# nalinbhardwaj/curdleproofs.pie

Hardware: AMD Instinct MI355X
Metric: BLS12-381 G1 scalar-muls/sec at MSM size 2^20 (higher is better)
Workload: dtype u32

## Files before the change

curdleproofs_pie_amd/build.py:

```python
from __future__ import annotations

import os
import shutil
import subprocess
import sys

HERE = os.path.dirname(os.path.abspath(__file__))
CSRC = os.path.join(HERE, "csrc")
LIB = os.path.join(HERE, "libcurdle_g1.so")
SOURCES = [os.path.join(CSRC, "msm_gpu.hip"), os.path.join(CSRC, "host_g1.cpp"), os.path.join(CSRC, "merlin.cpp"), os.path.join(CSRC, "shuffle_verify.cpp"), os.path.join(CSRC, "comm.cpp"), os.path.join(CSRC, "lazy_host.cpp")]
DEPS = SOURCES + [os.path.join(CSRC, f) for f in ("kernels_opening.h", "kernels_generator.h", "kernels_fixed.h", "fixed_digits.h", "capi_fixed.h", "kernels_light.h", "light_digits.h", "capi_light.h", "kernels_ipa.h", "ipa_rounds.h", "capi_ipa.h", "kernels_same_msm.h", "same_msm_rounds.h", "capi_same_msm.h", "fp28.h", "g1_xyzz.h", "g1_quad.h", "host_g1.h", "fe_mul_x86.h", "fr.h", "merlin_group.h", "bls_consts.h", "kernels_records.h", "kernels_prepare_digits.h",
                                                    "kernels_sort.h", "kernels_accumulate.h", "kernels_reduce.h", "kernels_small.h", "kernels_batch.h", "kernels_rows.h", "kernels_merlin.h", "kernels_frontend.h", "pool.h", "lazy_host.h", "fp_row.h", "glv.h", "host_context.h", "host_chains.h", "capi_core_msm.h", "capi_vec_batched.h", "capi_lincomb.h",
                                                    "capi_timing_batchmul.h", "capi_codec_transcripts.h", "capi_frontend.h", "capi_rows_probes.h")] + [
    os.path.join(HERE, "..", "include", "curdle_g1.h")
]


def _source_hash() -> str:
    import hashlib

    h = hashlib.sha256()
    for d in sorted(DEPS):
        if os.path.exists(d):
            h.update(os.path.basename(d).encode())
            with open(d, "rb") as f:
                h.update(f.read())
    h.update(os.environ.get("CURDLE_G1_PIPELINE", "staged").encode())
    with open(os.path.abspath(__file__), "rb") as f:
        h.update(f.read())
    return h.hexdigest()


HASH_FILE = LIB + ".srchash"
HOST_ONLY = ("host_g1.cpp", "merlin.cpp", "shuffle_verify.cpp", "comm.cpp", "lazy_host.cpp", "merlin_group.h", "fe_mul_x86.h")


def _hip_unit_hash(extra_flags=()) -> str:
    import hashlib

    h = hashlib.sha256()
    for d in sorted(DEPS):
        if os.path.basename(d) in HOST_ONLY or not os.path.exists(d):
            continue
        h.update(os.path.basename(d).encode())
        with open(d, "rb") as f:
            h.update(f.read())
    h.update(repr(tuple(extra_flags)).encode())
    with open(os.path.abspath(__file__), "rb") as f:
        h.update(f.read())
    return h.hexdigest()[:24]


def needs_build() -> bool:
    if not os.path.exists(LIB) or not os.path.exists(HASH_FILE):
        return True
    try:
        return open(HASH_FILE).read().strip() != _source_hash()
    except OSError:
        return True


LLVM_BIN = "/opt/rocm/lib/llvm/bin"
INFO_FILE = LIB + ".buildinfo"
DROPPED_PASSES = ("reassociate",)


def default_pipeline() -> str:
    p = os.environ.get("CURDLE_G1_PIPELINE", "staged")
    if p not in ("staged", "plain"):
        raise ValueError(f"CURDLE_G1_PIPELINE must be 'staged' or 'plain', not {p!r}")
    return p


def _run(cmd, verbose, **kw):
    if verbose:
        print("[curdleproofs_pie_amd.build]", " ".join(a if len(a) < 160 else a[:157] + "..." for a in cmd), flush=True)
    return subprocess.run(cmd, check=True, **kw)


def _device_pipeline(raw_bc: str, verbose: bool) -> str:
    import re

    tool = lambda t: os.path.join(LLVM_BIN, t)
    out = _run([tool("opt"), "-mtriple=amdgcn-amd-amdhsa", "-mcpu=gfx950", "-amdgpu-internalize-symbols", "-passes=default<O3>", "-print-pipeline-passes",
                "-disable-output", raw_bc], verbose, capture_output=True, text=True).stdout.strip()
    pipe = out.replace(",BitcodeWriterPass", "")
    for dropped in DROPPED_PASSES:
        if f"{dropped}," not in pipe:
            raise RuntimeError(f"pass {dropped!r} not found in the O3 pipeline: the toolchain changed, re-check DESIGN.md section 9")
        pipe = pipe.replace(f"{dropped},", "")
    ll = _run([tool("llvm-dis"), raw_bc, "-o", "-"], False, capture_output=True, text=True).stdout
    keep = re.findall(r"^define [^@\n]*amdgpu_kernel [^@\n]*@([\w.$]+)\(", ll, re.M)
    keep += re.findall(r"^@([\w.$]+) = (?!internal|private)", ll, re.M)
    if not keep or pipe.count(",internalize,") != 1:
# ... 165 lines not shown
```

curdleproofs_pie_amd/csrc/capi_core_msm.h:

```cpp
#pragma once

using cg1::Ctx;
struct cg1_ctx : public cg1::Ctx {};

namespace cg1 {
static Ctx* child_of(Ctx* ctx) { return static_cast<Ctx*>(ctx->child); }

static int ensure_child(Ctx* ctx) {
  if (!ctx->child) {
    cg1_ctx* made = ctx->cu_mask.empty() ? cg1_ctx_create(ctx->device) : cg1_ctx_create_cu_mask(ctx->device, ctx->cu_mask.data(), ctx->cu_mask.size());
    if (!made) { snprintf(ctx->err, sizeof ctx->err, "could not create the second launch chain's context"); return CG1_ERR_HIP; }
    made->split = 0;
    made->batched_split = 0;
    ctx->child = made;
  }
  if (!ctx->ev_prep) HIPCHK(hipEventCreateWithFlags(&ctx->ev_prep, hipEventDisableTiming));
  if (!ctx->ev_acc) HIPCHK(hipEventCreateWithFlags(&ctx->ev_acc, hipEventDisableTiming));
  return CG1_OK;
}

static int msm_begin_split(Ctx* ctx, const PtSrc& src, const void* d_scalars32, size_t n, const WinPlan& plan, int rank, int world) {
  HIPCHK(hipSetDevice(ctx->device));
  { int crc = ensure_child(ctx); if (crc) return crc; }
  Ctx* ch = child_of(ctx);
// ... 191 lines not shown
int cg1_h2d_async(cg1_ctx* ctx, void* dst, const void* src, size_t bytes) {
  if (!ctx) return CG1_ERR_HIP;
  if (bytes == 0) return CG1_OK;
  HIPCHK(hipSetDevice(ctx->device));
  std::call_once(ctx->copy_once, [ctx]() { hipStream_t s = nullptr; if (hipStreamCreateWithFlags(&s, hipStreamNonBlocking) == hipSuccess) ctx->copy_stream.store(s); });
  hipStream_t cs = ctx->copy_stream.load();
  if (!cs) { snprintf(ctx->err, sizeof ctx->err, "could not create the copy stream"); return CG1_ERR_HIP; }
  HIPCHK(hipMemcpyAsync(dst, src, bytes, hipMemcpyHostToDevice, cs));
  return CG1_OK;
}
int cg1_stream_sync(cg1_ctx* ctx) {
  if (!ctx) return CG1_ERR_HIP;
  HIPCHK(hipSetDevice(ctx->device));
  return cg1::wait_stream(ctx);
}
int cg1_copy_fence(cg1_ctx* ctx) {
  if (!ctx) return CG1_ERR_HIP;
  HIPCHK(hipSetDevice(ctx->device));
  hipStream_t cs = ctx->copy_stream.load();
  if (!cs) return CG1_OK;
  HIPCHK(hipEventRecord(ctx->copy_ev, cs));
  HIPCHK(hipStreamWaitEvent(ctx->stream, ctx->copy_ev, 0));
  return CG1_OK;
}
void* cg1_host_alloc(cg1_ctx* ctx, size_t bytes) {
  if (!ctx) return nullptr;
  void* p = nullptr;
  if (hipSetDevice(ctx->device) != hipSuccess) return nullptr;
  if (hipHostMalloc(&p, bytes ? bytes : 1) != hipSuccess) return nullptr;
  return p;
}
void cg1_host_free(cg1_ctx* ctx, void* p) {
  if (!ctx || !p) return;
  (void)hipSetDevice(ctx->device);
  (void)hipHostFree(p);
}
int cg1_d2h_2d(cg1_ctx* ctx, void* dst, size_t dst_pitch, const void* src, size_t src_pitch, size_t width, size_t rows) {
  if (!ctx) return CG1_ERR_HIP;
  if (rows == 0 || width == 0) return CG1_OK;
  if (width > dst_pitch || width > src_pitch) return CG1_ERR_ARG;
  HIPCHK(hipSetDevice(ctx->device));
  HIPCHK(hipMemcpy2D(dst, dst_pitch, src, src_pitch, width, rows, hipMemcpyDeviceToHost));
  return CG1_OK;
}
int cg1_ctx_sync(cg1_ctx* ctx) {
  if (!ctx) return CG1_ERR_HIP;
  HIPCHK(hipSetDevice(ctx->device));
  HIPCHK(hipDeviceSynchronize());
  return CG1_OK;
}
int cg1_merlin_last_passes(const cg1_ctx* ctx) { return ctx ? (int)ctx->merlin_passes : -1; }
int cg1_merlin_last_kernel(const cg1_ctx* ctx) { return ctx ? ctx->merlin_last_kernel : -1; }
int cg1_ctx_device(const cg1_ctx* ctx) { return ctx ? ctx->device : -1; }
void* cg1_ctx_stream(cg1_ctx* ctx) { return ctx ? (void*)ctx->stream : nullptr; }
int cg1_ctx_set_param(cg1_ctx* ctx, const char* name, int value) {
  if (!ctx || !name) return CG1_ERR_ARG;
  if (!strcmp(name, "chunk_rule")) { ctx->chunk_rule = value != 0; return CG1_OK; }
  if (!strcmp(name, "chunk_len")) { if (value < 1 || value > 65536) return CG1_ERR_ARG; ctx->L0 = (uint32_t)value; cg1::free_bufs(ctx); return CG1_OK; }
  if (!strcmp(name, "stage_sort")) { ctx->stage_sort = value ? 1 : 0; return CG1_OK; }
  if (!strcmp(name, "quad")) { ctx->quad = value ? 1 : 0; return CG1_OK; }
  if (!strcmp(name, "glv")) { if (value < 0 || value > 2) return CG1_ERR_ARG; ctx->glv = value; return CG1_OK; }
  if (!strcmp(name, "glv_max_n")) { if (value < 0) return CG1_ERR_ARG; ctx->glv_max_n = value; return CG1_OK; }
  if (!strcmp(name, "batched_split")) { ctx->batched_split = value ? 1 : 0; return CG1_OK; }
  if (!strcmp(name, "batched_split_min_m")) { if (value < 2) return CG1_ERR_ARG; ctx->batched_split_min_m = value; return CG1_OK; }
  if (!strcmp(name, "lincomb_zero_copy")) { ctx->lincomb_zero_copy = value ? 1 : 0; return CG1_OK; }
  if (!strcmp(name, "fold_quad")) { ctx->fold_quad = value ? 1 : 0; return CG1_OK; }
  if (!strcmp(name, "rowcol_row")) { ctx->rowcol_row = value ? 1 : 0; return CG1_OK; }
  if (!strcmp(name, "tree_row")) { ctx->tree_row = value ? 1 : 0; return CG1_OK; }
  if (!strcmp(name, "horner_row")) { ctx->horner_row = value ? 1 : 0; return CG1_OK; }
  if (!strcmp(name, "batch_mul_row")) { ctx->batch_mul_row = value ? 1 : 0; return CG1_OK; }
  if (!strcmp(name, "small_msm")) { ctx->small_msm = value ? 1 : 0; return CG1_OK; }
  if (!strcmp(name, "fixed_slice")) { if (value < 0 || value > 128) return CG1_ERR_ARG; ctx->fixed_slice = value; return CG1_OK; }
  if (!strcmp(name, "fixed_waves")) { if (value != 0 && value != 4 && value != 8 && value != 16) return CG1_ERR_ARG; ctx->fixed_waves = value; return CG1_OK; }
  if (!strcmp(name, "ipa_inv")) { if (value != 0 && value != 1) return CG1_ERR_ARG; ctx->ipa_inv = value; return CG1_OK; }
  if (!strcmp(name, "small_row_tail")) { ctx->small_row_tail = value ? 1 : 0; return CG1_OK; }
  if (!strcmp(name, "split")) { ctx->split = value ? 1 : 0; return CG1_OK; }
  if (!strcmp(name, "split_min_log2n")) { if (value < 10 || value > 31) return CG1_ERR_ARG; ctx->split_min_n = (size_t)1 << value; return CG1_OK; }
  if (!strcmp(name, "reduce_2d")) { ctx->reduce_2d = value ? 1 : 0; return CG1_OK; }
  if (!strcmp(name, "partition_sort")) { ctx->use_partition_sort = value ? 1 : 0; cg1::free_bufs(ctx); return CG1_OK; }
  if (!strcmp(name, "blocking_sync")) { ctx->blocking_sync = value != 0; return CG1_OK; }
  if (!strcmp(name, "big_bins")) { ctx->big_bins = value != 0; return CG1_OK; }
  if (!strcmp(name, "host_split")) { ctx->host_split = value != 0; return CG1_OK; }
  if (!strcmp(name, "arm_helpers")) { ctx->arm_helpers = value != 0; return CG1_OK; }
  if (!strcmp(name, "horner_threads")) { if (value != 1 && value != 2 && value != 4) return CG1_ERR_ARG; ctx->horner_threads = value; return CG1_OK; }
  if (!strcmp(name, "zero_copy")) { ctx->zero_copy = value != 0; return CG1_OK; }
  if (!strcmp(name, "auto_plan")) { ctx->auto_plan = value != 0; return CG1_OK; }
  if (!strcmp(name, "rowcol_quad")) { ctx->rowcol_quad = value != 0; return CG1_OK; }
  if (!strcmp(name, "rowcol_quad_max")) { if (value < 0) return CG1_ERR_ARG; ctx->rowcol_quad_max = value; return CG1_OK; }
  if (!strcmp(name, "fold_pass")) { ctx->fold_pass = value != 0; return CG1_OK; }
  if (!strcmp(name, "scan_one")) { ctx->scan_one = value != 0; return CG1_OK; }
  if (!strcmp(name, "batched_host_horner_max")) { if (value < 0) return CG1_ERR_ARG; ctx->batched_host_horner_max = value; return CG1_OK; }
  if (!strcmp(name, "tree_shift")) { if (value < -1 || value > 4) return CG1_ERR_ARG; ctx->tree_shift = value; return CG1_OK; }
  if (!strcmp(name, "rowcol_lgq")) { if (value != 0 && (value < 2 || value > 4)) return CG1_ERR_ARG; ctx->rowcol_lgq = value; return CG1_OK; }
  if (!strcmp(name, "sort_sub_bits")) { if (value != 0 && (value < 4 || value > 8)) return CG1_ERR_ARG; ctx->sort_sub_bits = value; return CG1_OK; }
  if (!strcmp(name, "batch_mul_host_max")) { if (value < -1) return CG1_ERR_ARG; ctx->batch_mul_host_max = value; return CG1_OK; }
  if (!strcmp(name, "batch_mul_quad_max")) { if (value < 0) return CG1_ERR_ARG; ctx->batch_mul_quad_max = value; return CG1_OK; }
  if (!strcmp(name, "merlin_sync")) { ctx->merlin_sync = value != 0; return CG1_OK; }
  if (!strcmp(name, "fe_timed")) { ctx->fe_timed = value != 0; return CG1_OK; }
  if (!strcmp(name, "fe_rows")) { ctx->fe_rows = value != 0; return CG1_OK; }
  if (!strcmp(name, "fe_prio")) { if (value < 0 || value > 3) return CG1_ERR_ARG; ctx->fe_prio = value; return CG1_OK; }
  if (!strcmp(name, "decompress_waves")) { if (value != 2 && value != 3) return CG1_ERR_ARG; ctx->decompress_waves = value; return CG1_OK; }
  if (!strcmp(name, "merlin_rows")) { ctx->merlin_rows = value != 0; return CG1_OK; }
  if (!strcmp(name, "merlin_lanes")) { if (value < 1 || value > 64) return CG1_ERR_ARG; ctx->merlin_lanes = value; return CG1_OK; }
  if (!strcmp(name, "tree_half")) { ctx->tree_half = value != 0; return CG1_OK; }
  if (!strcmp(name, "wave_agg")) {
    int v = value ? 1 : 0;
    HIPCHK(hipSetDevice(ctx->device));
    HIPCHK(hipMemcpyToSymbol(HIP_SYMBOL(cg1::g_wave_agg), &v, sizeof v));
    return CG1_OK;
  }
  if (!strcmp(name, "profile")) { if (value < 0 || value > 2) return CG1_ERR_ARG; ctx->profile = value; return CG1_OK; }
  if (!strcmp(name, "seg_m")) { if (value != 1 && value != 2 && value != 4 && value != 8 && value != 16) return CG1_ERR_ARG; ctx->seg_m = (uint32_t)value; return CG1_OK; }
  return CG1_ERR_ARG;
}

int cg1_msm_device(cg1_ctx* ctx, const void* d_points, const void* d_scalars, size_t n, int window_c, int shard_rank,
                   int shard_world, uint8_t* out) {
  if (!ctx) return CG1_ERR_HIP;
  cg1h::jac r;
  int rc = cg1::msm_device(ctx, d_points, d_scalars, n, window_c, shard_rank, shard_world, r);
  if (rc == CG1_OK) blob_out(out, r);
  return rc;
}

int cg1_msm_device_begin(cg1_ctx* ctx, const void* d_points, const void* d_scalars, size_t n, int window_c, int shard_rank, int shard_world) {
  if (!ctx) return CG1_ERR_HIP;
  return cg1::msm_begin(ctx, d_points, d_scalars, n, window_c, shard_rank, shard_world);
}
int cg1_msm_device_end(cg1_ctx* ctx, uint8_t* out) {
  if (!ctx) return CG1_ERR_HIP;
  cg1h::jac r;
  int rc = cg1::msm_end(ctx, r);
  if (rc == CG1_OK) blob_out(out, r);
  return rc;
}

int cg1_msm_multi_device(cg1_ctx* const* ctxs, size_t n_ctx, const void* const* d_points, const void* const* d_scalars, const size_t* n,
                         int window_c, uint8_t* out) {
  if (!ctxs || !n_ctx || !d_points || !d_scalars || !n || !out) return CG1_ERR_ARG;
  for (size_t i = 0; i < n_ctx; ++i) {
    if (!ctxs[i]) return CG1_ERR_HIP;
    for (size_t j = 0; j < i; ++j) if (ctxs[j] == ctxs[i]) return CG1_ERR_ARG;
  }
  int rc = CG1_OK;
  size_t begun = 0;
  for (; begun < n_ctx && rc == CG1_OK; ++begun)
    rc = cg1::msm_begin(ctxs[begun], d_points[begun], d_scalars[begun], n[begun], window_c, 0, 1);
  cg1h::jac acc = cg1h::jac_identity();
  for (size_t i = 0; i < begun; ++i) {
    cg1h::jac part;
    int r2 = cg1::msm_end(ctxs[i], part);
    if (rc == CG1_OK) rc = r2;
    if (r2 == CG1_OK) acc = cg1h::jac_add(acc, part);
  }
  if (rc == CG1_OK) blob_out(out, acc);
  return rc;
}

static int ensure_stage(cg1_ctx* ctx, size_t pts_bytes, size_t sc_bytes) {
  if (pts_bytes > ctx->cap_stage_pts) {
    if (ctx->d_stage_pts) (void)hipFree(ctx->d_stage_pts);
    ctx->d_stage_pts = nullptr; ctx->cap_stage_pts = 0;
    const size_t want = pts_bytes + pts_bytes / 4 + 256;
    HIPCHK(hipMalloc(&ctx->d_stage_pts, want));
    ctx->cap_stage_pts = want;
  }
  if (sc_bytes > ctx->cap_stage_sc) {
// ... 73 lines not shown
```

curdleproofs_pie_amd/csrc/host_chains.h:

```cpp
#pragma once

namespace cg1 {

static WinPlan make_plan(int c, bool glv = false) {
  WinPlan pl;
  const int bits = glv ? 127 : 255;
  pl.glv = glv ? 1 : 0;
  if (c > 0) { pl.cmax = c; pl.nwin = bits / c + 1; pl.n_hi = pl.nwin; }
  else {
    const int cm = -c, nw = (bits + 1 + cm - 1) / cm;
    pl.cmax = cm; pl.nwin = nw; pl.n_hi = bits + 1 - nw * (cm - 1);
    if (pl.n_hi < 0) pl.n_hi = 0;
  }
  return pl;
}

static int pick_plan_c(size_t n, int auto_plan) {
  const int c = pick_window(n);
  if (!auto_plan || c != 16) return c;
  if (n <= (1u << 14)) return -12;
  if (n <= (3u << 15)) return -13;
  if (n <= (3u << 16)) return -15;
  return 16;
}
// ... 23 lines not shown
  PtSrc(const void* affine96) : p(affine96) {}
};

static uint32_t blob_points_per_lane(size_t n) {
  size_t K = (n + (1u << 17) - 1) >> 17;
  return (uint32_t)(K < 1 ? 1 : (K > 16 ? 16 : K));
}

static void launch_prepare(hipStream_t st, const PtSrc& src, PreparedPoint* out, uint8_t* flags_out, uint32_t n32, uint32_t* status_words) {
  if (src.kind == PtSrc::AFFINE96) {
    hipLaunchKernelGGL(k_prepare_points, dim3((n32 + 255) / 256), dim3(256), 0, st, (const uint32_t*)src.p, out, flags_out, n32, status_words);
  } else if (src.normalised) {
    hipLaunchKernelGGL((k_prepare_blobs<false>), dim3((n32 + 127) / 128), dim3(128), 0, st, (const uint32_t*)src.p, out, flags_out, n32, 1u, status_words);
  } else {
    const uint32_t K = blob_points_per_lane(n32);
    const uint32_t lanes = (n32 + K - 1) / K;
    hipLaunchKernelGGL((k_prepare_blobs<true>), dim3((lanes + 127) / 128), dim3(128), 0, st, (const uint32_t*)src.p, out, flags_out, n32, K, status_words);
  }
}

struct ChainHooks {
  hipEvent_t before_start = nullptr, after_prepare = nullptr, before_accumulate = nullptr, after_accumulate = nullptr;
};

static int msm_enqueue(Ctx* ctx, const PtSrc& src, const void* d_scalars32, size_t n, const WinPlan& plan, int rank, int world,
                       const ChainHooks& hooks = ChainHooks()) {
  ctx->pend.active = false;
  HIPCHK(hipSetDevice(ctx->device));
  const int c = plan.cmax, nwin = plan.nwin;
  const size_t n_real = n;
  if (plan.glv) n *= 2;
  const int nlw = win_count(nwin, rank, world);
  if (nlw <= 0) return CG1_OK;
  const uint32_t NB = 1u << (c - 1);
  const uint32_t m = std::min<uint32_t>(ctx->seg_m, NB);
  const uint32_t J = NB / m;
  int nbits = 0; while ((1u << nbits) < J) ++nbits;
  const uint32_t bb = (uint32_t)c - 1u, lb2 = (bb + 1u) / 2u, hb2 = bb - lb2;
  const bool use2d = ctx->reduce_2d != 0;
  const uint32_t nitems = use2d ? 1u + hb2 + lb2 : 1u + (uint32_t)nbits;
  const size_t nb_total = (size_t)nlw * NB;
  uint32_t L0 = ctx->L0;
  while (L0 < 65536u && ((uint64_t)n * (uint64_t)nlw >> 18) > (uint64_t)L0) L0 <<= 1;
  if (ctx->chunk_rule && world == 1) {
    const uint64_t entries = (uint64_t)n * (uint64_t)nlw;
    if (entries >= (1ull << 20) && entries < (1ull << 21) && L0 < 10u) L0 = 10u;
    if (entries >= (1ull << 21) && entries < (1ull << 24) && nb_total > (size_t)ctx->rowcol_quad_max) {
      const double mload = (double)n / (double)(1u << bb);
      uint32_t want = (uint32_t)(mload + 8.0 * std::sqrt(mload) + 1.0);
      if (entries < (1ull << 22) && want > 20u) want = 20u;
      if (want > L0) L0 = want;
    }
  }
  int rc = ensure(ctx, n, nb_total, nlw, nitems, L0, src.kind != PtSrc::PREPARED);
  if (rc) return rc;
  hipStream_t st = ctx->stream;
  const uint32_t n32 = (uint32_t)n;
  const uint32_t gn = (n32 + 255) / 256;
  const int profile = ctx->profile;
  auto h0 = std::chrono::steady_clock::now();
  const bool resident = src.kind == PtSrc::PREPARED;
  const PreparedPoint* pts = resident ? static_cast<const PreparedPoint*>(src.p) : ctx->d_pts;
  const uint8_t* flags = resident ? src.flags : ctx->d_flags;
  const size_t nout_words = (size_t)nlw * nitems;
  uint32_t* bad_flag = reinterpret_cast<uint32_t*>(ctx->d_out + nout_words);
  if (hooks.before_start) HIPCHK(hipStreamWaitEvent(st, hooks.before_start, 0));
  if (profile >= 2) HIPCHK(hipEventRecord(ctx->ev[0], st));
  const uint32_t n_real32 = (uint32_t)n_real;
  if (resident) HIPCHK(hipMemsetAsync(bad_flag, 0, 16, st));
  else {
    launch_prepare(st, src, ctx->d_pts, ctx->d_flags, n_real32, bad_flag);
    if (plan.glv) hipLaunchKernelGGL(k_phi_records, dim3((n_real32 + 255) / 256), dim3(256), 0, st, ctx->d_pts, ctx->d_flags, n_real32);
  }
  if (hooks.after_prepare) HIPCHK(hipEventRecord(hooks.after_prepare, st));
  if (profile >= 2) HIPCHK(hipEventRecord(ctx->ev[1], st));
  const uint32_t nblk = (uint32_t)((nb_total + SCAN_ITEMS - 1) / SCAN_ITEMS);
  if (ctx->use_partition_sort && n <= PART_MAX_N) {
    const uint32_t want_sub = ctx->sort_sub_bits ? (uint32_t)ctx->sort_sub_bits : (n <= ((size_t)1 << 16) ? 7u : 8u);
    uint32_t sub_bits = bb < want_sub ? bb : want_sub;
    while (bb - sub_bits > 7u) ++sub_bits;
    const uint32_t nbins = 1u << (bb - sub_bits);
    const uint32_t nslices = (n32 + PART_TILE - 1) / PART_TILE;
    const uint32_t nbc = (uint32_t)nlw * nbins * nslices;
    hipLaunchKernelGGL(k_digits, dim3((n_real32 + 255) / 256), dim3(256), 0, st, (const uint32_t*)d_scalars32, flags, ctx->d_digits, n_real32, plan, rank, world, bad_flag);
    hipLaunchKernelGGL(k_part_count, dim3(nslices, nlw), dim3(256), 0, st, ctx->d_digits, ctx->d_blockcnt, n32, nslices, nbins, sub_bits);
    const uint32_t ublk = (nbc + SCAN_ITEMS - 1) / SCAN_ITEMS;
    if (ctx->scan_one && nbc <= USCAN1_MAX) {
      hipLaunchKernelGGL(k_uscan_one, dim3(1), dim3(1024), 0, st, ctx->d_blockcnt, nbc);
    } else {
      hipLaunchKernelGGL(k_uscan1, dim3(ublk), dim3(256), 0, st, ctx->d_blockcnt, ctx->d_ublocktot, nbc);
      hipLaunchKernelGGL(k_uscan2, dim3(1), dim3(256), 0, st, ctx->d_ublocktot, ublk, ctx->d_blockcnt, nbc);
      hipLaunchKernelGGL(k_uscan3, dim3(ublk), dim3(256), 0, st, ctx->d_ublocktot, ctx->d_blockcnt, nbc);
    }
    if (profile >= 2) HIPCHK(hipEventRecord(ctx->ev[2], st));
    hipLaunchKernelGGL(k_part_scatter, dim3(nslices, nlw), dim3(256), 0, st, ctx->d_digits, ctx->d_blockcnt, ctx->d_part, n32, nslices, nbins, sub_bits, ctx->stage_sort);
    const uint32_t nbt = (uint32_t)nlw * nbins;
    const int big_bins = ctx->big_bins && n32 > 2u * BIN_STAGE;
    hipLaunchKernelGGL(k_slice_plan, dim3(1), dim3(256), 0, st, ctx->d_blockcnt, nbt, nslices, ctx->d_slice_base, ctx->d_bigflag, big_bins);
    hipLaunchKernelGGL(k_bin_sort, dim3(nbt), dim3(256), 0, st, ctx->d_part, ctx->d_blockcnt, ctx->d_hist, ctx->d_sorted, nbt, nslices, sub_bits, ctx->stage_sort, ctx->d_bigflag);
    if (big_bins) {
      const uint32_t max_slices = (uint32_t)(((size_t)n * (size_t)nlw) / SLICE + nbt + 1);
      hipLaunchKernelGGL(k_slice_count, dim3(max_slices), dim3(256), 0, st, ctx->d_part, ctx->d_blockcnt, nbt, nslices, ctx->d_slice_base, ctx->d_slicehist);
      hipLaunchKernelGGL(k_slice_prefix, dim3(nbt), dim3(256), 0, st, ctx->d_blockcnt, nslices, sub_bits, ctx->d_slice_base, ctx->d_bigflag, ctx->d_slicehist, ctx->d_subbase, ctx->d_hist);
      hipLaunchKernelGGL(k_slice_scatter, dim3(max_slices), dim3(256), 0, st, ctx->d_part, ctx->d_blockcnt, nbt, nslices, ctx->d_slice_base, ctx->d_slicehist, ctx->d_subbase, ctx->d_sorted);
    }
    if (profile >= 2) HIPCHK(hipEventRecord(ctx->ev[3], st));
    if (ctx->scan_one && nb_total <= SCAN1_MAX) {
      hipLaunchKernelGGL(k_scan_one, dim3(1), dim3(1024), 0, st, ctx->d_hist, ctx->d_off, ctx->d_choff, (uint32_t)nb_total, L0);
    } else {
      hipLaunchKernelGGL(k_scan1, dim3(nblk), dim3(256), 0, st, ctx->d_hist, ctx->d_off, ctx->d_choff, ctx->d_blocktot, (uint32_t)nb_total, L0);
      hipLaunchKernelGGL(k_scan2, dim3(1), dim3(256), 0, st, ctx->d_blocktot, nblk, ctx->d_off, ctx->d_choff, (uint32_t)nb_total);
      hipLaunchKernelGGL(k_scan3, dim3(nblk), dim3(256), 0, st, ctx->d_blocktot, ctx->d_off, ctx->d_choff, (uint32_t)nb_total);
    }
  } else {
    HIPCHK(hipMemsetAsync(ctx->d_hist, 0, nb_total * 4, st));
    hipLaunchKernelGGL(k_hist, dim3(gn), dim3(256), 0, st, (const uint32_t*)d_scalars32, flags, ctx->d_hist, n32, plan, rank, world, bad_flag);
    if (profile >= 2) HIPCHK(hipEventRecord(ctx->ev[2], st));
    hipLaunchKernelGGL(k_scan1, dim3(nblk), dim3(256), 0, st, ctx->d_hist, ctx->d_off, ctx->d_choff, ctx->d_blocktot, (uint32_t)nb_total, L0);
    hipLaunchKernelGGL(k_scan2, dim3(1), dim3(256), 0, st, ctx->d_blocktot, nblk, ctx->d_off, ctx->d_choff, (uint32_t)nb_total);
    hipLaunchKernelGGL(k_scan3, dim3(nblk), dim3(256), 0, st, ctx->d_blocktot, ctx->d_off, ctx->d_choff, (uint32_t)nb_total);
    if (profile >= 2) HIPCHK(hipEventRecord(ctx->ev[3], st));
    hipLaunchKernelGGL(k_scatter, dim3(gn), dim3(256), 0, st, (const uint32_t*)d_scalars32, flags, ctx->d_hist, ctx->d_off, ctx->d_sorted, n32, plan, rank, world);
  }
  HIPCHK(hipMemsetAsync(ctx->d_zblock, 0, zblock_clear_bytes(ctx), st));
  hipLaunchKernelGGL(k_chunk_desc, dim3((uint32_t)std::min<size_t>(CHUNK_DESC_BLOCKS, (nb_total + 255) / 256)), dim3(256), 0, st, ctx->d_off, ctx->d_choff, ctx->d_desc, ctx->d_lenhist, ctx->d_heavy, (uint32_t)ctx->cap_heavy, (uint32_t)nb_total, L0, ctx->d_any_multi);
  const size_t max_chunks = nb_total + (n * (size_t)nlw) / L0 + 1;
  const uint32_t gchunks = (uint32_t)((max_chunks + 255) / 256);
  hipLaunchKernelGGL(k_len_scan, dim3(1), dim3(256), 0, st, ctx->d_lenhist, ctx->d_lenhist + LEN_BINS, ctx->d_off + nb_total, ctx->d_choff + nb_total, bad_flag);
  hipLaunchKernelGGL(k_order, dim3((gchunks + ORDER_PER - 1) / ORDER_PER), dim3(256), 0, st, ctx->d_desc, ctx->d_choff + nb_total, ctx->d_lenhist + LEN_BINS, ctx->d_order);
  if (hooks.before_accumulate) HIPCHK(hipStreamWaitEvent(st, hooks.before_accumulate, 0));
  if (profile >= 1) HIPCHK(hipEventRecord(ctx->ev[4], st));
  hipLaunchKernelGGL(k_accumulate, dim3(gchunks), dim3(256), 0, st, ctx->d_desc, ctx->d_choff + nb_total, ctx->d_order, ctx->d_sorted, pts, ctx->d_sums);
  if (profile >= 1) HIPCHK(hipEventRecord(ctx->ev[5], st));
  if (hooks.after_accumulate) HIPCHK(hipEventRecord(hooks.after_accumulate, st));
  hipLaunchKernelGGL(k_heavy_combine, dim3(512), dim3(256), 0, st, ctx->d_heavy, (uint32_t)ctx->cap_heavy, ctx->d_choff, ctx->d_sums, ctx->d_combined);
  const bool small_quad = ctx->quad && ctx->rowcol_quad && nb_total <= (size_t)ctx->rowcol_quad_max;
  const bool rows_fold = small_quad && use2d && ctx->rowcol_row && ctx->tree_row && nb_total <= 8192;
  if (rows_fold) {}
  else if (small_quad && ctx->fold_quad)
    hipLaunchKernelGGL(k_bucket_fold_quad, dim3((uint32_t)((nb_total * 4 + 255) / 256)), dim3(256), 0, st, ctx->d_choff, ctx->d_sums, ctx->d_combined, (uint32_t)nb_total, ctx->d_any_multi);
  else if (ctx->fold_pass)
    hipLaunchKernelGGL(k_bucket_fold, dim3((uint32_t)((nb_total + 255) / 256)), dim3(256), 0, st, ctx->d_choff, ctx->d_sums, ctx->d_combined, (uint32_t)nb_total, ctx->d_any_multi);
  bool tree_exports = false;
  if (use2d) {
    const uint32_t R = 1u << hb2, Cn = 1u << lb2;
    const uint32_t lpr = Cn < 32u ? Cn : 32u, lpc = R < 16u ? R : 16u;
    const uint32_t nrow_blocks = ((uint32_t)nlw * R + (256u / lpr) - 1u) / (256u / lpr);
    const uint32_t ncol_blocks = ((uint32_t)nlw * Cn + (256u / lpc) - 1u) / (256u / lpc);
    PointSum* rowsum = ctx->d_segrun;
    PointSum* colsum = ctx->d_segtot;
    if (small_quad) {
      uint32_t lgq = (R == Cn) ? 2u : 3u;
      if (ctx->rowcol_lgq >= 2 && ctx->rowcol_lgq <= 4) lgq = (uint32_t)ctx->rowcol_lgq;
      const uint32_t rc_waves = ((uint32_t)nlw * (R + Cn) + (16u >> lgq) - 1u) / (16u >> lgq);
      if (ctx->rowcol_row && ctx->tree_row)
        hipLaunchKernelGGL(k_rowcol_quad_row, dim3(((uint32_t)nlw * (R + Cn) + 3u) / 4u), dim3(256), 0, st, ctx->d_choff, ctx->d_sums, ctx->d_combined,
                           rowsum, colsum, (uint32_t)nlw, hb2, lb2);
      else
      hipLaunchKernelGGL(k_rowcol_quad, dim3((rc_waves + 3u) / 4u), dim3(256), 0, st, ctx->d_choff, ctx->d_sums,
                         rowsum, colsum, (uint32_t)nlw, hb2, lb2, lgq);
    }
    else
      hipLaunchKernelGGL(k_rowcol, dim3(nrow_blocks + ncol_blocks), dim3(256), 0, st, ctx->d_choff, ctx->d_sums, ctx->d_combined,
                         rowsum, colsum, (uint32_t)nlw, hb2, lb2, nrow_blocks, ctx->quad);
    if (profile >= 2) HIPCHK(hipEventRecord(ctx->ev[6], st));
    const uint32_t tree_threads = std::min<uint32_t>(512u, std::max<uint32_t>(64u, 4u << std::max(hb2, lb2)) >> (ctx->tree_shift >= 0 ? ctx->tree_shift : (ctx->tree_half ? 1 : 0)));
    if (ctx->tree_row) {
      uint32_t W = (1u << std::max(hb2, lb2)) >> 3;
      W = W < 1u ? 1u : (W > 16u ? 16u : W);
      tree_exports = ctx->zero_copy != 0;
      if (tree_exports) ++ctx->seq;
      hipLaunchKernelGGL(k_small_tree_row, dim3(nitems, nlw), dim3(64u * W), 0, st, rowsum, colsum, ctx->d_out, hb2, lb2,
                         tree_exports ? ctx->h_out_dev : (PointWords*)nullptr, bad_flag, ctx->h_flag_dev, ctx->seq);
    }
    else if (ctx->quad) hipLaunchKernelGGL(k_small_tree_quad, dim3(nitems, nlw), dim3(std::max<uint32_t>(64u, tree_threads)), 0, st, rowsum, colsum, ctx->d_out, hb2, lb2);
    else hipLaunchKernelGGL(k_small_tree, dim3(nitems, nlw), dim3(256), 0, st, rowsum, colsum, ctx->d_out, hb2, lb2);
  } else {
    const uint32_t nseg_total = (uint32_t)(nb_total / m);
    hipLaunchKernelGGL(k_seg_reduce, dim3((nseg_total + 255) / 256), dim3(256), 0, st, ctx->d_choff, ctx->d_sums, ctx->d_combined, ctx->d_segrun, ctx->d_segtot, nseg_total, m);
    if (profile >= 2) HIPCHK(hipEventRecord(ctx->ev[6], st));
    uint32_t S = (J + BT_ELEMS - 1) / BT_ELEMS; if (S < 1) S = 1; if (S > 64) S = 64;
    hipLaunchKernelGGL(k_bit_tree, dim3(nitems, nlw, S), dim3(256), 0, st, ctx->d_segrun, ctx->d_segtot, ctx->d_partial, J);
    hipLaunchKernelGGL(k_bit_tree_final, dim3((uint32_t)(nitems * nlw)), dim3(64), 0, st, ctx->d_partial, ctx->d_out, S);
  }
  const bool zc = ctx->zero_copy != 0;
  if (zc && tree_exports) {
  } else if (zc) {
    ++ctx->seq;
    const uint32_t nvec = (uint32_t)((((size_t)nlw * nitems + 1) * sizeof(PointWords)) / 16);
    hipLaunchKernelGGL(k_export_host, dim3(1), dim3(1024), 0, st, reinterpret_cast<const uint4*>(ctx->d_out), reinterpret_cast<uint4*>(ctx->h_out_dev), nvec,
                       ctx->h_flag_dev, ctx->seq);
  } else {
    HIPCHK(hipMemcpyAsync(ctx->h_out, ctx->d_out, ((size_t)nlw * nitems + 1) * sizeof(PointWords), hipMemcpyDeviceToHost, st));
  }
  if (profile >= 2) HIPCHK(hipEventRecord(ctx->ev[7], st));
  auto h1 = std::chrono::steady_clock::now();
  Ctx::Pending& pd = ctx->pend;
  pd.zero_copy = zc; pd.seq = ctx->seq; pd.hout = ctx->h_out;
  pd.active = true; pd.c = c; pd.plan = plan; pd.rank = rank; pd.world = world; pd.nlw = nlw; pd.nbits = nbits; pd.m = m; pd.lb2 = lb2; pd.hb2 = hb2;
  pd.nitems = nitems; pd.use2d = use2d; pd.profile = profile; pd.nout_words = nout_words; pd.h0 = h0; pd.h1 = h1;
  pd.arm_helpers = ctx->arm_helpers && ctx->host_split && ctx->horner_threads > 1 && n <= ((size_t)1 << 18);
  return CG1_OK;
}

static int msm_finish(Ctx* ctx, cg1h::jac& result) {
  result = cg1h::jac_identity();
  if (!ctx->pend.active) return CG1_OK;
  const Ctx::Pending pd = ctx->pend;
  ctx->pend.active = false;
  const int c = pd.c, rank = pd.rank, world = pd.world, nlw = pd.nlw, nbits = pd.nbits;
  (void)c;
  const uint32_t m = pd.m, lb2 = pd.lb2, hb2 = pd.hb2, nitems = pd.nitems;
  const bool use2d = pd.use2d;
  const size_t nout_words = pd.nout_words;
  const auto h0 = pd.h0, h1 = pd.h1;
  HIPCHK(hipSetDevice(ctx->device));
  struct StandDown { Ctx* c; bool on; ~StandDown() { if (on) for (int j = 0; j < 3; ++j) c->helper[j].disarm(); } } stand_down{ctx, false};
  if (pd.zero_copy && !ctx->blocking_sync && pd.profile < 2) {
    if (pd.arm_helpers) for (int j = 0; j < 3 && j + 1 < ctx->horner_threads; ++j) ctx->helper[j].arm();
    stand_down.on = pd.arm_helpers;
    volatile uint32_t* flag = ctx->h_flag;
    for (uint32_t spins = 0; *flag != pd.seq; ++spins) {
      if ((spins & 0x3fffu) == 0x3fffu) {
        hipError_t q = hipStreamQuery(ctx->stream);
        if (q == hipSuccess) { if (*flag != pd.seq) { snprintf(ctx->err, sizeof ctx->err, "the stream drained without the export flag"); return CG1_ERR_HIP; } break; }
        if (q != hipErrorNotReady) { snprintf(ctx->err, sizeof ctx->err, "stream failed: %s", hipGetErrorString(q)); return CG1_ERR_HIP; }
      }
      __builtin_ia32_pause();
    }
    std::atomic_thread_fence(std::memory_order_acquire);
  } else {
    int wrc = wait_stream(ctx); if (wrc) return wrc;
  }
  HIPCHK(hipGetLastError());
  {
    const uint32_t* st_words = reinterpret_cast<const uint32_t*>(pd.hout + nout_words);
    ctx->last_entries = st_words[1]; ctx->last_chunks = st_words[2];
    if (st_words[0]) {
      snprintf(ctx->err, sizeof ctx->err, "a scalar is >= 2^255: scalar32 must be a canonical Fr element (< r)");
      return CG1_ERR_ENCODING;
    }
  }
  auto h2 = std::chrono::steady_clock::now();
  { int erc = read_phase_events(ctx, pd.profile); if (erc) return erc; }
  ctx->last_c = c;

  auto t0 = std::chrono::steady_clock::now();
  ctx->host_ms[0] = std::chrono::duration<float, std::milli>(h1 - h0).count();
  ctx->host_ms[1] = std::chrono::duration<float, std::milli>(h2 - h1).count();
  ctx->host_ms[2] = std::chrono::duration<float, std::milli>(t0 - h2).count();
  int lm = 0; while ((1u << lm) < m) ++lm;
  const WinPlan& plan = pd.plan;
  constexpr int EMAX = 2 * 256 + 64;
  std::vector<std::pair<int, const PointWords*>> items;
  items.reserve((size_t)nlw * nitems);
  int e_top = 0;
  for (int lw = 0; lw < nlw; ++lw) {
    const int w = win_global(lw, rank, world), base = plan.off(w);
    const PointWords* row = pd.hout + (size_t)lw * nitems;
    auto put = [&](int e, const PointWords* p) { if (!p->inf && e >= 0 && e < EMAX) { items.emplace_back(e, p); if (e > e_top) e_top = e; } };
    put(base, &row[0]);
    if (use2d) {
      for (uint32_t k = 0; k < hb2; ++k) put(base + (int)lb2 + (int)k, &row[1 + k]);
      for (uint32_t k = 0; k < lb2; ++k) put(base + (int)k, &row[1 + hb2 + k]);
    } else {
      for (int b2 = 0; b2 < nbits; ++b2) put(base + lm + b2, &row[1 + b2]);
    }
  }
  uint16_t first[EMAX + 1];
  memset(first, 0, sizeof first);
  for (const auto& it : items) ++first[it.first + 1];
  for (int e = 0; e < EMAX; ++e) first[e + 1] = (uint16_t)(first[e + 1] + first[e]);
  std::vector<const PointWords*> byexp(items.size());
  {
    uint16_t cur[EMAX];
    memcpy(cur, first, sizeof cur);
    for (const auto& it : items) byexp[cur[it.first]++] = it.second;
  }
  auto horner = [&](int lo, int hi) {
    cg1h::jac a = cg1h::jac_identity();
    for (int e = hi; e >= lo; --e) {
      a = cg1h::jac_dbl(a);
      for (uint16_t k = first[e]; k < first[e + 1]; ++k) a = cg1h::jac_add(a, jac_from_words(*byexp[k]));
    }
    return a;
  };
  cg1h::jac acc;
  const int nth = (!ctx->host_split || e_top < 96) ? 1 : (ctx->horner_threads >= 4 && e_top >= 112 ? 4 : 2);
  if (nth > 1) {
    cg1h::jac part[4];
    int lo[5];
    {
      constexpr long DBL = 7, ADD = 16;
      auto fill = [&](long C, int* cut) {
        int e = 0;
        for (int j = 0; j < nth; ++j) {
          cut[j] = e;
          long adds = 0;
          while (e <= e_top && DBL * (e + 1) + ADD * (adds + (first[e + 1] - first[e])) <= C) { adds += first[e + 1] - first[e]; ++e; }
        }
        cut[nth] = e_top + 1;
        return e > e_top;
      };
      long lo_c = DBL * (e_top + 1), hi_c = DBL * (e_top + 1) + ADD * (long)items.size();
      int cut[5];
      while (lo_c < hi_c) {
        const long mid = (lo_c + hi_c) / 2;
        if (fill(mid, cut)) hi_c = mid; else lo_c = mid + 1;
      }
      fill(hi_c, cut);
      for (int j = 0; j <= nth; ++j) lo[j] = cut[j];
    }
    auto run_part = [&](int j) {
      cg1h::jac a = horner(lo[j], lo[j + 1] - 1);
      for (int k = 0; k < lo[j]; ++k) a = cg1h::jac_dbl(a);
      part[j] = a;
    };
    for (int j = 0; j + 1 < nth; ++j) ctx->helper[j].run([&, j]() { run_part(j); });
    if (pd.arm_helpers) for (int j = nth - 1 < 0 ? 0 : nth - 1; j < 3; ++j) ctx->helper[j].disarm();
    run_part(nth - 1);
    acc = part[nth - 1];
    for (int j = 0; j + 1 < nth; ++j) { ctx->helper[j].wait(); acc = cg1h::jac_add(acc, part[j]); }
  } else {
    if (pd.arm_helpers) for (int j = 0; j < 3; ++j) ctx->helper[j].disarm();
    acc = horner(0, e_top);
  }
  result = acc;
  ctx->host_tail_ms = std::chrono::duration<float, std::milli>(std::chrono::steady_clock::now() - t0).count();
  ctx->host_ms[3] = ctx->host_tail_ms;
  return CG1_OK;
}

static int pick_small_c(size_t n) {
  if (n <= 24) return 4;
  if (n <= 96) return 6;
  if (n <= 6 * SM_SLICE) return 7;
  return 8;
}

static int msm_enqueue_small(Ctx* ctx, const PtSrc& src, const void* d_scalars32, size_t n, int c, uint32_t M = 1, const uint32_t* d_offs = nullptr, size_t max_n = 0,
                             bool glv = false) {
  ctx->pend.active = false;
  HIPCHK(hipSetDevice(ctx->device));
  const WinPlan plan = make_plan(c, glv);
  const uint32_t nwin = (uint32_t)plan.nwin, bb = (uint32_t)c - 1u, lb2 = (bb + 1u) / 2u, hb2 = bb - lb2, nitems = 1u + hb2 + lb2;
  if (M == 1) max_n = n;
  const uint32_t S = (uint32_t)(((glv ? 2 * max_n : max_n) + SM_SLICE - 1) / SM_SLICE);
  auto h0 = std::chrono::steady_clock::now();
  if (!ctx->h_small_out) {
    HIPCHK(hipHostMalloc((void**)&ctx->h_small_out, ((size_t)SM_MAX_MSMS * 64 * 9 + 1) * sizeof(PointWords), hipHostMallocMapped | hipHostMallocCoherent));
    HIPCHK(hipHostGetDevicePointer((void**)&ctx->h_small_out_dev, ctx->h_small_out, 0));
    HIPCHK(hipMalloc(&ctx->d_small_ctr, (SM_MAX_MSMS * 64 + 8) * 4));
    HIPCHK(hipMemsetAsync(ctx->d_small_ctr, 0, (SM_MAX_MSMS * 64 + 8) * 4, ctx->stream));
  }
  const size_t need_partial = (size_t)M * nwin * S * nitems;
  if (S > 1 && need_partial > ctx->cap_small_partial) {
    if (ctx->d_small_partial) (void)hipFree(ctx->d_small_partial);
    ctx->d_small_partial = nullptr; ctx->cap_small_partial = 0;
    HIPCHK(hipMalloc(&ctx->d_small_partial, need_partial * sizeof(PointSum)));
    ctx->cap_small_partial = need_partial;
  }
  hipStream_t st = ctx->stream;
  SmallArgs a;
  a.src = src.p; a.flags = src.flags; a.scalars = static_cast<const uint32_t*>(d_scalars32); a.offs = d_offs;
  a.n = (uint32_t)n; a.M = M; a.S = S; a.c = (uint32_t)c; a.nwin = nwin; a.hb = hb2; a.lb = lb2; a.nitems = nitems;
  a.partial = ctx->d_small_partial; a.counters = ctx->d_small_ctr;
  a.out_host = ctx->h_small_out_dev; a.flag_host = ctx->h_flag_dev; a.seq = ++ctx->seq;
  a.row_tail = ctx->small_row_tail ? 1u : 0u;
  a.glv = glv ? 1u : 0u;
  int kind = (int)src.kind;
  if (src.kind == PtSrc::BLOBS && !src.normalised) {
    if (n > ctx->cap_small_pts) {
      if (ctx->d_small_pts) (void)hipFree(ctx->d_small_pts);
      if (ctx->d_small_flags) (void)hipFree(ctx->d_small_flags);
      ctx->d_small_pts = nullptr; ctx->d_small_flags = nullptr; ctx->cap_small_pts = 0;
      const size_t cap = n < SM_MAX_N ? SM_MAX_N : n;
      HIPCHK(hipMalloc(&ctx->d_small_pts, cap * sizeof(PreparedPoint)));
      HIPCHK(hipMalloc(&ctx->d_small_flags, cap + 16));
      ctx->cap_small_pts = cap;
    }
    launch_prepare(st, src, ctx->d_small_pts, ctx->d_small_flags, (uint32_t)n, nullptr);
    a.src = ctx->d_small_pts; a.flags = ctx->d_small_flags;
    kind = (int)PtSrc::PREPARED;
  }
  const dim3 grid(nwin, S, M), block(512);
  if (kind == (int)PtSrc::AFFINE96) hipLaunchKernelGGL((k_msm_small<0>), grid, block, 0, st, a);
  else if (kind == (int)PtSrc::BLOBS) hipLaunchKernelGGL((k_msm_small<1>), grid, block, 0, st, a);
  else hipLaunchKernelGGL((k_msm_small<2>), grid, block, 0, st, a);
  auto h1 = std::chrono::steady_clock::now();
  Ctx::Pending& pd = ctx->pend;
  pd.zero_copy = true; pd.seq = ctx->seq; pd.hout = ctx->h_small_out;
  pd.active = true; pd.c = c; pd.plan = plan; pd.rank = 0; pd.world = 1; pd.nlw = (int)nwin; pd.nbits = 0; pd.m = 1; pd.lb2 = lb2; pd.hb2 = hb2;
  pd.nitems = nitems; pd.use2d = true; pd.profile = 0; pd.nout_words = (size_t)M * nwin * nitems; pd.h0 = h0; pd.h1 = h1;
  pd.arm_helpers = ctx->arm_helpers && ctx->host_split && ctx->horner_threads > 1 && M == 1;
  return CG1_OK;
}

static cg1h::jac horner_2d_items(const PointWords* rows, const WinPlan& plan, uint32_t nitems, uint32_t hb2, uint32_t lb2) {
  constexpr int EMAX = 2 * 256 + 64;
  std::vector<std::pair<int, const PointWords*>> items;
  items.reserve((size_t)plan.nwin * nitems);
  int e_top = 0;
  for (int w = 0; w < plan.nwin; ++w) {
    const int base = plan.off(w);
    const PointWords* row = rows + (size_t)w * nitems;
    auto put = [&](int e, const PointWords* p) { if (!p->inf) { items.emplace_back(e, p); if (e > e_top) e_top = e; } };
    put(base, &row[0]);
    for (uint32_t k = 0; k < hb2; ++k) put(base + (int)lb2 + (int)k, &row[1 + k]);
    for (uint32_t k = 0; k < lb2; ++k) put(base + (int)k, &row[1 + hb2 + k]);
  }
  uint16_t first[EMAX + 1];
  memset(first, 0, sizeof first);
  for (const auto& it : items) ++first[it.first + 1];
  for (int e = 0; e < EMAX; ++e) first[e + 1] = (uint16_t)(first[e + 1] + first[e]);
  std::vector<const PointWords*> byexp(items.size());
  {
    uint16_t cur[EMAX];
    memcpy(cur, first, sizeof cur);
    for (const auto& it : items) byexp[cur[it.first]++] = it.second;
  }
  cg1h::jac a = cg1h::jac_identity();
  for (int e = e_top; e >= 0; --e) {
    a = cg1h::jac_dbl(a);
    for (uint16_t k = first[e]; k < first[e + 1]; ++k) a = cg1h::jac_add(a, jac_from_words(*byexp[k]));
  }
  return a;
}

static int msm_small_batched_finish(Ctx* ctx, uint32_t M, std::vector<cg1h::jac>& results) {
  const Ctx::Pending pd = ctx->pend;
  ctx->pend.active = false;
  HIPCHK(hipSetDevice(ctx->device));
  if (!ctx->blocking_sync) {
    volatile uint32_t* flag = ctx->h_flag;
    for (uint32_t spins = 0; *flag != pd.seq; ++spins) {
      if ((spins & 0x3fffu) == 0x3fffu) {
        hipError_t q = hipStreamQuery(ctx->stream);
        if (q == hipSuccess) { if (*flag != pd.seq) { snprintf(ctx->err, sizeof ctx->err, "the stream drained without the export flag"); return CG1_ERR_HIP; } break; }
        if (q != hipErrorNotReady) { snprintf(ctx->err, sizeof ctx->err, "stream failed: %s", hipGetErrorString(q)); return CG1_ERR_HIP; }
      }
      __builtin_ia32_pause();
    }
    std::atomic_thread_fence(std::memory_order_acquire);
  } else {
    int wrc = wait_stream(ctx); if (wrc) return wrc;
  }
  HIPCHK(hipGetLastError());
  const uint32_t* st_words = reinterpret_cast<const uint32_t*>(pd.hout + pd.nout_words);
  ctx->last_entries = st_words[1]; ctx->last_chunks = 0;
  if (st_words[0]) {
    snprintf(ctx->err, sizeof ctx->err, "a scalar is >= 2^255: scalar32 must be a canonical Fr element (< r)");
    return CG1_ERR_ENCODING;
  }
  auto t0 = std::chrono::steady_clock::now();
  const size_t per = (size_t)pd.plan.nwin * pd.nitems;
  auto one = [&](size_t j) { results[j] = horner_2d_items(pd.hout + j * per, pd.plan, pd.nitems, pd.hb2, pd.lb2); };
  if (M <= 4) {
    const size_t nth = std::min<size_t>(4, M);
    for (size_t t = 1; t < nth; ++t) ctx->helper[t - 1].run([&, t]() { for (size_t j = t; j < M; j += nth) one(j); });
    for (size_t j = 0; j < M; j += nth) one(j);
    for (size_t t = 1; t < nth; ++t) ctx->helper[t - 1].wait();
  } else {
    std::atomic<size_t> next{0};
    std::function<void()> work = [&]() { for (;;) { const size_t j = next.fetch_add(1); if (j >= M) return; one(j); } };
    Pool& pool = Pool::get();
    pool.run(work, std::min<size_t>(M, pool.size() + 1));
  }
  auto t1 = std::chrono::steady_clock::now();
  ctx->host_ms[0] = std::chrono::duration<float, std::milli>(pd.h1 - pd.h0).count();
  ctx->host_ms[1] = std::chrono::duration<float, std::milli>(t0 - pd.h1).count();
  ctx->host_ms[2] = 0;
  ctx->host_ms[3] = ctx->host_tail_ms = std::chrono::duration<float, std::milli>(t1 - t0).count();
  for (int i = 0; i < CG1_NPHASE; ++i) ctx->phase_ms[i] = 0.f;
  ctx->last_c = pd.c;
  ctx->last_acc_launches = 0;
  return CG1_OK;
}

static Ctx* child_of(Ctx* ctx);
static int msm_begin_split(Ctx* ctx, const PtSrc& src, const void* d_scalars32, size_t n, const WinPlan& plan, int rank, int world);

int msm_begin(Ctx* ctx, const PtSrc& src, const void* d_scalars32, size_t n, int c, int rank, int world) {
  ctx->pend.active = false;
  ctx->pend_c = 0;
  if (n == 0) return CG1_OK;
  if (n >= (1ull << 31)) { snprintf(ctx->err, sizeof ctx->err, "n too large"); return CG1_ERR_ARG; }
  if (world < 1 || world > 255 || rank < 0 || rank >= world) { snprintf(ctx->err, sizeof ctx->err, "bad window shard %d/%d", rank, world); return CG1_ERR_ARG; }
  for (int pass = (ctx->glv && 2 * n <= SM_MAX_N) ? 1 : 0; pass >= 0; --pass) {
    const bool sglv = pass == 1;
    const size_t nn = sglv ? 2 * n : n;
    const int bits = sglv ? 127 : 255;
    if (ctx->small_msm && nn <= SM_MAX_N && world == 1 && (c == 0 || (c >= 4 && c <= 9 && c != 5)) &&
        (size_t)(bits / (c ? c : pick_small_c(nn)) + 1) * ((nn + SM_SLICE - 1) / SM_SLICE) <= SM_ONE_ROUND) {
      if (c == 0) c = pick_small_c(nn);
      ctx->pend_c = c;
      return msm_enqueue_small(ctx, src, d_scalars32, n, c, 1, nullptr, 0, sglv);
    }
  }
  const bool glv = src.kind != PtSrc::PREPARED && ctx->use_partition_sort && 2 * n <= PART_MAX_N &&
                   (ctx->glv == 2 || (ctx->glv == 1 && n <= (size_t)ctx->glv_max_n));
  if (c == 0) c = pick_plan_c(glv ? 2 * n : n, ctx->auto_plan);
  const int cabs = c < 0 ? -c : c;
  if (cabs < 4 || cabs > 16) { snprintf(ctx->err, sizeof ctx->err, "window width %d out of range [4,16]", c); return CG1_ERR_ARG; }
  const WinPlan plan = make_plan(c, glv);
  ctx->pend_c = c;
  ctx->pend_split = false;
  if (ctx->split && n >= ctx->split_min_n && win_count(plan.nwin, rank, world) >= 2) return msm_begin_split(ctx, src, d_scalars32, n, plan, rank, world);
  return msm_enqueue(ctx, src, d_scalars32, n, plan, rank, world);
}
// ... 16 lines not shown
    ctx->last_entries = e_hi + ch->last_entries; ctx->last_chunks = c_hi + ch->last_chunks;
    ctx->host_ms[0] = enq + ch->host_ms[0]; ctx->host_ms[1] = wait_hi + ch->host_ms[1]; ctx->host_ms[3] = tail_hi + ch->host_ms[3];
    ctx->host_tail_ms = ch->host_ms[3];
  }
  if (ctx->pend_c) ctx->last_c = ctx->pend_c;
  return rc;
}
int msm_device(Ctx* ctx, const PtSrc& src, const void* d_scalars32, size_t n, int c, int rank, int world, cg1h::jac& result) {
  result = cg1h::jac_identity();
  int rc = msm_begin(ctx, src, d_scalars32, n, c, rank, world);
  if (rc) return rc;
  return msm_end(ctx, result);
}


int pick_window_batched(size_t n_avg, bool glv) {
  const int bits = glv ? 127 : 255;
  if (glv) n_avg *= 2;
  int best = 4; double best_cost = 1e300;
  for (int c = 4; c <= 9; ++c) {
    if (bits % c == 0) continue;
    int nwin = bits / c + 1;
    double NB = (double)(1u << (c - 1));
    double cost = (double)nwin * ((double)n_avg + 1.4 * (2.0 * NB + 3.0 * NB / 8.0)) + 1.4 * (double)bits;
    if (cost < best_cost) { best_cost = cost; best = c; }
  }
  return best;
}
int pick_window_batched(size_t n_avg) { return pick_window_batched(n_avg, false); }

static int ensure_child(Ctx* ctx);

struct BatchedChain {
  size_t M = 0; int c = 0; uint32_t nwin = 0; bool host_horner = false;
  std::chrono::steady_clock::time_point h0, h1;
};
static int batched_chain_enqueue(Ctx* ctx, const void* d_points96, const void* d_scalars32, const uint32_t* h_offsets, size_t M, int c, bool glv,
                                 hipEvent_t wait_before_accumulate, hipEvent_t record_after_accumulate, BatchedChain& bc) {
  const size_t N = h_offsets[M], N_real = N;
  HIPCHK(hipSetDevice(ctx->device));
  const WinPlan bplan = make_plan(c, glv);
  const uint32_t nwin = (uint32_t)bplan.nwin, NB = 1u << (c - 1);
  const size_t G = M * nwin, nb_total = G * NB;
  const size_t Nv = glv ? 2 * N : N;
  if (nb_total >= (1ull << 31) || Nv * nwin >= (1ull << 31)) { snprintf(ctx->err, sizeof ctx->err, "batch too large"); return CG1_ERR_ARG; }
  const uint32_t m = 8 < NB ? 8 : NB;
  uint32_t log2m = 0; while ((1u << log2m) < m) ++log2m;
  const uint32_t J = NB / m;
  uint32_t L0 = ctx->L0;
  while (L0 < 65536u && ((uint64_t)Nv * (uint64_t)nwin >> 18) > (uint64_t)L0) L0 <<= 1;
  int rc = ensure(ctx, Nv, nb_total, nwin, 1, L0);
  if (rc) return rc;
  if ((M + 1) > ctx->cap_boffs) {
    if (ctx->d_boffs) (void)hipFree(ctx->d_boffs);
    HIPCHK(hipMalloc(&ctx->d_boffs, (M + 1) * 4));
    ctx->cap_boffs = M + 1;
  }
  if (G > ctx->cap_gsum) {
    if (ctx->d_gsum) (void)hipFree(ctx->d_gsum);
    HIPCHK(hipMalloc(&ctx->d_gsum, G * sizeof(PointSum)));
    ctx->cap_gsum = G;
  }
  if (M > ctx->cap_bout) {
    if (ctx->d_bout) (void)hipFree(ctx->d_bout);
    if (ctx->h_bout) (void)hipHostFree(ctx->h_bout);
    HIPCHK(hipMalloc(&ctx->d_bout, (M + 1) * sizeof(PointWords)));
    HIPCHK(hipHostMalloc(&ctx->h_bout, (M + 1) * sizeof(PointWords)));
    ctx->cap_bout = M;
  }
  if (Nv * nwin > ctx->cap_digits) {
    if (ctx->d_digits) (void)hipFree(ctx->d_digits);
    HIPCHK(hipMalloc(&ctx->d_digits, Nv * nwin * 2 + 16));
    ctx->cap_digits = Nv * nwin;
  }
  hipStream_t st = ctx->stream;
  const uint32_t N32 = (uint32_t)N_real, gn = (N32 + 255) / 256, Nv32 = (uint32_t)Nv, split = glv ? N32 : 0u;
  auto h0 = std::chrono::steady_clock::now();
  HIPCHK(hipMemcpyAsync(ctx->d_boffs, h_offsets, (M + 1) * 4, hipMemcpyHostToDevice, st));
  if (ctx->profile >= 2) HIPCHK(hipEventRecord(ctx->ev[0], st));
  uint32_t* bad_flag = reinterpret_cast<uint32_t*>(ctx->d_bout + M);
  hipLaunchKernelGGL(k_prepare_points, dim3(gn), dim3(256), 0, st, (const uint32_t*)d_points96, ctx->d_pts, ctx->d_flags, N32, bad_flag);
  if (glv) hipLaunchKernelGGL(k_phi_records, dim3(gn), dim3(256), 0, st, ctx->d_pts, ctx->d_flags, N32);
  if (ctx->profile >= 2) HIPCHK(hipEventRecord(ctx->ev[1], st));
  hipLaunchKernelGGL(k_digits, dim3(gn), dim3(256), 0, st, (const uint32_t*)d_scalars32, ctx->d_flags, ctx->d_digits, N32, bplan, 0, 1, bad_flag);
  hipLaunchKernelGGL(k_group_count, dim3((uint32_t)M, nwin), dim3(256), 0, st, ctx->d_digits, ctx->d_boffs, ctx->d_hist, Nv32, NB, nwin, split);
  if (ctx->profile >= 2) HIPCHK(hipEventRecord(ctx->ev[2], st));
  const uint32_t nblk = (uint32_t)((nb_total + SCAN_ITEMS - 1) / SCAN_ITEMS);
  hipLaunchKernelGGL(k_scan1, dim3(nblk), dim3(256), 0, st, ctx->d_hist, ctx->d_off, ctx->d_choff, ctx->d_blocktot, (uint32_t)nb_total, L0);
  hipLaunchKernelGGL(k_scan2, dim3(1), dim3(256), 0, st, ctx->d_blocktot, nblk, ctx->d_off, ctx->d_choff, (uint32_t)nb_total);
  hipLaunchKernelGGL(k_scan3, dim3(nblk), dim3(256), 0, st, ctx->d_blocktot, ctx->d_off, ctx->d_choff, (uint32_t)nb_total);
  hipLaunchKernelGGL(k_group_scatter, dim3((uint32_t)M, nwin), dim3(256), 0, st, ctx->d_digits, ctx->d_boffs, ctx->d_off, ctx->d_sorted, Nv32, NB, nwin, split);
  if (ctx->profile >= 2) HIPCHK(hipEventRecord(ctx->ev[3], st));
  HIPCHK(hipMemsetAsync(ctx->d_zblock, 0, zblock_clear_bytes(ctx), st));
  hipLaunchKernelGGL(k_chunk_desc, dim3((uint32_t)std::min<size_t>(CHUNK_DESC_BLOCKS, (nb_total + 255) / 256)), dim3(256), 0, st, ctx->d_off, ctx->d_choff, ctx->d_desc, ctx->d_lenhist, ctx->d_heavy, (uint32_t)ctx->cap_heavy, (uint32_t)nb_total, L0, ctx->d_any_multi);
  const size_t max_chunks = nb_total + (Nv * (size_t)nwin) / L0 + 1;
  const uint32_t gchunks = (uint32_t)((max_chunks + 255) / 256);
  hipLaunchKernelGGL(k_len_scan, dim3(1), dim3(256), 0, st, ctx->d_lenhist, ctx->d_lenhist + LEN_BINS, ctx->d_off + nb_total, ctx->d_choff + nb_total, bad_flag);
  hipLaunchKernelGGL(k_order, dim3((gchunks + ORDER_PER - 1) / ORDER_PER), dim3(256), 0, st, ctx->d_desc, ctx->d_choff + nb_total, ctx->d_lenhist + LEN_BINS, ctx->d_order);
  if (wait_before_accumulate) HIPCHK(hipStreamWaitEvent(st, wait_before_accumulate, 0));
  if (ctx->profile >= 1) HIPCHK(hipEventRecord(ctx->ev[4], st));
  hipLaunchKernelGGL(k_accumulate, dim3(gchunks), dim3(256), 0, st, ctx->d_desc, ctx->d_choff + nb_total, ctx->d_order, ctx->d_sorted, ctx->d_pts, ctx->d_sums);
  if (ctx->profile >= 1) HIPCHK(hipEventRecord(ctx->ev[5], st));
  if (record_after_accumulate) HIPCHK(hipEventRecord(record_after_accumulate, st));
  const uint32_t nseg_total = (uint32_t)(nb_total / m);
  hipLaunchKernelGGL(k_heavy_combine, dim3(512), dim3(256), 0, st, ctx->d_heavy, (uint32_t)ctx->cap_heavy, ctx->d_choff, ctx->d_sums, ctx->d_combined);
  hipLaunchKernelGGL(k_seg_reduce, dim3((nseg_total + 255) / 256), dim3(256), 0, st, ctx->d_choff, ctx->d_sums, ctx->d_combined, ctx->d_segrun, ctx->d_segtot, nseg_total, m);
  hipLaunchKernelGGL(k_group_reduce, dim3((uint32_t)((G + 255) / 256)), dim3(256), 0, st, ctx->d_segrun, ctx->d_segtot, ctx->d_gsum, (uint32_t)G, J, log2m);
  if (ctx->profile >= 2) HIPCHK(hipEventRecord(ctx->ev[6], st));
  const bool host_horner = M <= (size_t)ctx->batched_host_horner_max;
  if (host_horner) {
    if (G > ctx->cap_gout) {
      if (ctx->d_gout) (void)hipFree(ctx->d_gout);
      if (ctx->h_gout) (void)hipHostFree(ctx->h_gout);
      ctx->d_gout = nullptr; ctx->h_gout = nullptr; ctx->cap_gout = 0;
      HIPCHK(hipMalloc(&ctx->d_gout, G * sizeof(PointWords)));
      HIPCHK(hipHostMalloc(&ctx->h_gout, G * sizeof(PointWords)));
      ctx->cap_gout = G;
    }
    hipLaunchKernelGGL(k_export_sums, dim3((uint32_t)((G + 63) / 64)), dim3(64), 0, st, ctx->d_gsum, ctx->d_gout, (uint32_t)G);
    HIPCHK(hipMemcpyAsync(ctx->h_gout, ctx->d_gout, G * sizeof(PointWords), hipMemcpyDeviceToHost, st));
    HIPCHK(hipMemcpyAsync(ctx->h_bout + M, ctx->d_bout + M, sizeof(PointWords), hipMemcpyDeviceToHost, st));
  } else {
    if (ctx->horner_row && M <= 2048) hipLaunchKernelGGL(k_msm_horner_row, dim3((uint32_t)M), dim3(64), 0, st, ctx->d_gsum, ctx->d_bout, (uint32_t)M, nwin, (uint32_t)c);
    else if (ctx->quad) hipLaunchKernelGGL(k_msm_horner_quad, dim3((uint32_t)((M * 4 + 63) / 64)), dim3(64), 0, st, ctx->d_gsum, ctx->d_bout, (uint32_t)M, nwin, (uint32_t)c);
    else hipLaunchKernelGGL(k_msm_horner, dim3((uint32_t)((M + 63) / 64)), dim3(64), 0, st, ctx->d_gsum, ctx->d_bout, (uint32_t)M, nwin, (uint32_t)c);
    HIPCHK(hipMemcpyAsync(ctx->h_bout, ctx->d_bout, (M + 1) * sizeof(PointWords), hipMemcpyDeviceToHost, st));
  }
  if (ctx->profile >= 2) HIPCHK(hipEventRecord(ctx->ev[7], st));
  bc.M = M; bc.c = c; bc.nwin = nwin; bc.host_horner = host_horner; bc.h0 = h0; bc.h1 = std::chrono::steady_clock::now();
  return CG1_OK;
}

static int batched_chain_finish(Ctx* ctx, const BatchedChain& bc, cg1h::jac* results) {
  const size_t M = bc.M; const int c = bc.c; const uint32_t nwin = bc.nwin; const bool host_horner = bc.host_horner;
  const auto h0 = bc.h0, h1 = bc.h1;
  HIPCHK(hipSetDevice(ctx->device));
  { int wrc = wait_stream(ctx); if (wrc) return wrc; }
  HIPCHK(hipGetLastError());
  {
    const uint32_t* st_words = reinterpret_cast<const uint32_t*>(ctx->h_bout + M);
    ctx->last_entries = st_words[1]; ctx->last_chunks = st_words[2];
    if (st_words[0]) {
      snprintf(ctx->err, sizeof ctx->err, "a scalar is >= 2^255: scalar32 must be a canonical Fr element (< r)");
      return CG1_ERR_ENCODING;
    }
  }
  auto h2 = std::chrono::steady_clock::now();
  { int erc = read_phase_events(ctx, ctx->profile); if (erc) return erc; }
  ctx->last_c = c;
  if (host_horner) {
    auto one = [&](size_t j) {
      cg1h::jac a = cg1h::jac_identity();
      for (int w = (int)nwin - 1; w >= 0; --w) {
        for (int k = 0; k < c; ++k) a = cg1h::jac_dbl(a);
        a = cg1h::jac_add(a, jac_from_words(ctx->h_gout[j * nwin + (size_t)w]));
      }
      results[j] = a;
    };
    const size_t nth = std::min<size_t>(4, M);
    for (size_t t = 1; t < nth; ++t) ctx->helper[t - 1].run([&, t]() { for (size_t j = t; j < M; j += nth) one(j); });
    for (size_t j = 0; j < M; j += nth) one(j);
    for (size_t t = 1; t < nth; ++t) ctx->helper[t - 1].wait();
  } else {
    for (size_t j = 0; j < M; ++j) results[j] = jac_from_words(ctx->h_bout[j]);
  }
  auto h3 = std::chrono::steady_clock::now();
  ctx->host_ms[0] = std::chrono::duration<float, std::milli>(h1 - h0).count();
  ctx->host_ms[1] = std::chrono::duration<float, std::milli>(h2 - h1).count();
  ctx->host_ms[2] = 0;
  ctx->host_ms[3] = ctx->host_tail_ms = std::chrono::duration<float, std::milli>(h3 - h2).count();
  return CG1_OK;
}

static int msm_batched_small_end(Ctx* ctx, size_t M, std::vector<cg1h::jac>& results) {
  if (M == 1) { cg1h::jac r; int rc = msm_finish(ctx, r); ctx->last_acc_launches = 0; if (rc == CG1_OK) results[0] = r; return rc; }
  return msm_small_batched_finish(ctx, (uint32_t)M, results);
}
int msm_batched_device(Ctx* ctx, const void* d_points96, const void* d_scalars32, const uint32_t* h_offsets, size_t M,
                       int c, std::vector<cg1h::jac>& results, bool* async_small = nullptr, const uint32_t* d_offsets_ready = nullptr) {
  if (async_small) *async_small = false;
  results.assign(M, cg1h::jac_identity());
  if (M == 0) return CG1_OK;
  const size_t N = h_offsets[M];
  for (size_t j = 0; j < M; ++j) if (h_offsets[j] > h_offsets[j + 1]) { snprintf(ctx->err, sizeof ctx->err, "offsets not monotone"); return CG1_ERR_ARG; }
  if (h_offsets[0] != 0) { snprintf(ctx->err, sizeof ctx->err, "offsets[0] must be 0"); return CG1_ERR_ARG; }
  if (N == 0) return CG1_OK;
  if (N >= (1ull << 31) || M > 65535) { snprintf(ctx->err, sizeof ctx->err, "batch too large"); return CG1_ERR_ARG; }
  {
// ... 62 lines not shown
```

curdleproofs_pie_amd/csrc/host_context.h:

```cpp
#pragma once

namespace cg1 {

#define HIPCHK(x) do { hipError_t e_ = (x); if (e_ != hipSuccess) { \
  snprintf(ctx->err, sizeof ctx->err, "%s failed: %s (%s:%d)", #x, hipGetErrorString(e_), __FILE__, __LINE__); return CG1_ERR_HIP; } } while (0)

struct Helper {
  std::thread th;
  std::mutex mu;
  std::condition_variable cv;
  std::function<void()> job;
  bool has = false, done = true, quit = false, armed = false;
  std::atomic<bool> posted{false};
  std::atomic<bool> stand_down{false};
  void start_locked() { if (!th.joinable()) th = std::thread([this]() { loop(); }); }
  void run(std::function<void()> f) {
    std::unique_lock<std::mutex> lk(mu);
    start_locked();
    job = std::move(f); has = true; done = false;
    posted.store(true, std::memory_order_release);
    cv.notify_all();
  }
  void arm() {
    std::unique_lock<std::mutex> lk(mu);
    start_locked();
    if (!has && done) { stand_down.store(false, std::memory_order_relaxed); armed = true; cv.notify_all(); }
  }
  void disarm() { stand_down.store(true, std::memory_order_release); }
  void wait() {
    std::unique_lock<std::mutex> lk(mu);
    cv.wait(lk, [this]() { return done; });
  }
  void loop() {
    std::unique_lock<std::mutex> lk(mu);
    for (;;) {
      cv.wait(lk, [this]() { return has || quit || armed; });
      if (quit) return;
      if (!has) {
        armed = false;
        lk.unlock();
        const auto until = std::chrono::steady_clock::now() + std::chrono::milliseconds(2);
        for (uint32_t k = 0; !posted.load(std::memory_order_acquire); ++k) {
          if (stand_down.load(std::memory_order_acquire)) break;
          if ((k & 0xffu) == 0xffu && std::chrono::steady_clock::now() > until) break;
          __builtin_ia32_pause();
        }
        lk.lock();
        if (!has) continue;
      }
      armed = false;
      std::function<void()> f = std::move(job);
      has = false;
      posted.store(false, std::memory_order_relaxed);
      lk.unlock();
      f();
      lk.lock();
      done = true;
      cv.notify_all();
    }
  }
  ~Helper() {
    { std::unique_lock<std::mutex> lk(mu); quit = true; cv.notify_all(); }
    if (th.joinable()) th.join();
  }
};

struct Ctx {
  int device = 0;
  Helper helper[3];
  hipStream_t stream = nullptr;
  std::atomic<hipStream_t> copy_stream{nullptr};
  std::once_flag copy_once;
  hipEvent_t copy_ev = nullptr;
  std::vector<uint32_t> cu_mask;
  hipStream_t side_stream = nullptr;
  hipEvent_t side_ev = nullptr;
  hipEvent_t sync_ev = nullptr;
  int blocking_sync = 0;
  char err[256] = {0};
  size_t cap_n = 0, cap_nb = 0, cap_chunks = 0, cap_entries = 0, cap_out = 0;
  PreparedPoint* d_pts = nullptr;
  uint8_t* d_flags = nullptr;
  uint32_t *d_hist = nullptr, *d_off = nullptr, *d_choff = nullptr, *d_sorted = nullptr;
  uint2 *d_blocktot = nullptr, *d_desc = nullptr;
  uint32_t *d_order = nullptr, *d_lenhist = nullptr;
  uint32_t* d_zblock = nullptr; size_t cap_zblock = 0;
  uint32_t* d_any_multi = nullptr;
  PointSum* d_partial = nullptr; size_t cap_partial = 0;
  uint16_t* d_digits = nullptr; uint32_t* d_part = nullptr; uint32_t* d_blockcnt = nullptr; uint32_t* d_ublocktot = nullptr;
  size_t cap_digits = 0, cap_part = 0, cap_blockcnt = 0;
  uint32_t *d_slice_base = nullptr, *d_slicehist = nullptr, *d_subbase = nullptr; uint8_t* d_bigflag = nullptr;
  size_t cap_bigflag = 0, cap_slices = 0;
  int big_bins = 1;
  int use_partition_sort = 1;
  int stage_sort = 1;
  int host_split = 1;
  int rowcol_quad = 1;
  int rowcol_lgq = 0;
  int rowcol_quad_max = 1 << 18;
  int tree_shift = 2;
  int tree_half = 1;
  int merlin_sync = 1;
  uint32_t merlin_clk[2] = {0, 0};
  int fe_timed = 0;
  int fe_rows = 1;
  int fe_prio = 0;
  int decompress_waves = 3;
  void* d_opening = nullptr; size_t cap_opening = 0;
  void* d_prover = nullptr; size_t cap_prover = 0;
  PreparedPoint* d_gen_tab = nullptr;
  int fixed_slice = 0;
  int fixed_waves = 0;
  int ipa_inv = 0;
  int merlin_last_kernel = 0;
  int merlin_rows = 1;
  void* d_merlin_rows = nullptr; size_t merlin_rows_cap = 0;
  int merlin_lanes = 64;
  uint32_t merlin_passes = 0;
  int sort_sub_bits = 0;
  int batch_mul_host_max = -1;
  int last_batch_mul_on_host = 0;
  int batch_mul_quad_max = 8192;
  int scan_one = 1;
  int fold_pass = 1;
  int auto_plan = 1;
  struct Pending {
    bool active = false;
    int c = 0, rank = 0, world = 1, nlw = 0, nbits = 0;
    WinPlan plan;
    uint32_t m = 1, lb2 = 0, hb2 = 0, nitems = 0;
    bool use2d = true;
    int profile = 0;
    bool zero_copy = false; uint32_t seq = 0;
    bool arm_helpers = false;
    size_t nout_words = 0;
    const PointWords* hout = nullptr;
    std::chrono::steady_clock::time_point h0, h1;
  } pend;
  int split = 0;
  size_t split_min_n = (size_t)1 << 17;
  cg1_ctx* child = nullptr;
  hipEvent_t ev_prep = nullptr, ev_acc = nullptr;
  bool pend_split = false;
  int last_acc_launches = 0;
  int small_row_tail = 1;
  int small_msm = 1;
  PointSum* d_small_partial = nullptr; size_t cap_small_partial = 0;
  uint32_t* d_small_ctr = nullptr;
  PreparedPoint* d_small_pts = nullptr; uint8_t* d_small_flags = nullptr; size_t cap_small_pts = 0;
  PointWords* h_small_out = nullptr; PointWords* h_small_out_dev = nullptr;
  int quad = 1;
  int reduce_2d = 1;
  uint32_t* d_heavy = nullptr; size_t cap_heavy = 0;
  uint8_t* d_combined = nullptr; size_t cap_combined = 0;
  uint32_t* d_boffs = nullptr; size_t cap_boffs = 0;
  PointSum* d_gsum = nullptr; size_t cap_gsum = 0;
  PointWords* d_bout = nullptr; PointWords* h_bout = nullptr; size_t cap_bout = 0;
  PointWords* d_gout = nullptr; PointWords* h_gout = nullptr; size_t cap_gout = 0;
  int glv = 0;
  int glv_max_n = 1 << 14;
  int lincomb_zero_copy = 1;
  int fold_quad = 1;
  int rowcol_row = 1;
  int tree_row = 1;
  int horner_row = 1;
  int batch_mul_row = 1;
  int batched_split = 0;
  int batched_split_min_m = 256;
  int batched_host_horner_max = 24;
  PointSum *d_sums = nullptr, *d_segrun = nullptr, *d_segtot = nullptr;
  PointWords* d_out = nullptr;
  PointWords* h_out = nullptr;
  PointWords* h_out_dev = nullptr;
  uint32_t* h_flag = nullptr;
  uint32_t* h_flag_dev = nullptr;
  uint32_t seq = 0;
  int zero_copy = 1;
  int arm_helpers = 1;
  int horner_threads = 4;
  void* d_stage_pts = nullptr; void* d_stage_sc = nullptr; size_t cap_stage_pts = 0, cap_stage_sc = 0;
  uint8_t* h_lin = nullptr; uint8_t* h_lin_dev = nullptr; size_t cap_h_lin = 0;
  hipEvent_t ev[CG1_NPHASE + 1];
  float phase_ms[CG1_NPHASE] = {0};
  float host_tail_ms = 0;
  float host_ms[4] = {0, 0, 0, 0};
  int profile = 1;
  uint32_t last_chunks = 0, last_entries = 0;
  hipEvent_t tm_ev[2] = {nullptr, nullptr};
  int last_c = 0, pend_c = 0;
  int chunk_rule = 1;
  uint32_t L0 = 8;
  uint32_t seg_m = 4;
};

static void free_bufs(Ctx* c) {
  auto F = [](auto*& p) { if (p) { (void)hipFree(p); p = nullptr; } };
  F(c->d_pts); F(c->d_flags); F(c->d_hist); F(c->d_off); F(c->d_choff); F(c->d_sorted); F(c->d_blocktot); F(c->d_desc);
  F(c->d_sums); F(c->d_segrun); F(c->d_segtot); F(c->d_out); F(c->d_order); F(c->d_zblock); F(c->d_partial);
  c->d_lenhist = c->d_heavy = c->d_any_multi = nullptr; c->d_combined = nullptr; c->cap_zblock = 0; c->cap_heavy = 0; c->cap_combined = 0;
  c->cap_partial = 0;
  F(c->d_digits); F(c->d_part); F(c->d_blockcnt); F(c->d_ublocktot); F(c->d_boffs); F(c->d_gsum); F(c->d_bout);
  F(c->d_slice_base); F(c->d_slicehist); F(c->d_subbase); F(c->d_bigflag); c->cap_bigflag = 0; c->cap_slices = 0;
  if (c->h_bout) { (void)hipHostFree(c->h_bout); c->h_bout = nullptr; }
  if (c->h_lin) { (void)hipHostFree(c->h_lin); c->h_lin = nullptr; c->h_lin_dev = nullptr; c->cap_h_lin = 0; }
  if (c->d_gout) { (void)hipFree(c->d_gout); c->d_gout = nullptr; }
  if (c->h_gout) { (void)hipHostFree(c->h_gout); c->h_gout = nullptr; }
  c->cap_gout = 0;
  c->cap_boffs = c->cap_gsum = c->cap_bout = 0;
  c->cap_digits = c->cap_part = c->cap_blockcnt = 0;
  if (c->h_out) { (void)hipHostFree(c->h_out); c->h_out = nullptr; }
  c->cap_n = c->cap_nb = c->cap_chunks = c->cap_entries = c->cap_out = 0;
}

static int ensure(Ctx* ctx, size_t n, size_t nb_total, size_t nlw, size_t nitems, uint32_t L, bool need_points = true) {
  size_t entries = n * nlw;
  size_t chunks = nb_total + entries / L + 1;
  if (need_points && n > ctx->cap_n) {
    if (ctx->d_pts) (void)hipFree(ctx->d_pts);
    if (ctx->d_flags) (void)hipFree(ctx->d_flags);
    HIPCHK(hipMalloc(&ctx->d_pts, n * sizeof(PreparedPoint)));
    HIPCHK(hipMalloc(&ctx->d_flags, n + 16));
    ctx->cap_n = n;
  }
  if (nb_total > ctx->cap_nb) {
    auto F = [](auto*& p) { if (p) { (void)hipFree(p); p = nullptr; } };
    F(ctx->d_hist); F(ctx->d_off); F(ctx->d_choff); F(ctx->d_blocktot); F(ctx->d_segrun); F(ctx->d_segtot);
    HIPCHK(hipMalloc(&ctx->d_hist, nb_total * 4));
    HIPCHK(hipMalloc(&ctx->d_off, (nb_total + 1) * 4));
    HIPCHK(hipMalloc(&ctx->d_choff, (nb_total + 1) * 4));
    HIPCHK(hipMalloc(&ctx->d_blocktot, (nb_total / SCAN_ITEMS + 2) * sizeof(uint2)));
    HIPCHK(hipMalloc(&ctx->d_segrun, nb_total * sizeof(PointSum)));
    HIPCHK(hipMalloc(&ctx->d_segtot, nb_total * sizeof(PointSum)));
    ctx->cap_nb = nb_total;
  }
  if (entries > ctx->cap_entries) {
    if (ctx->d_sorted) (void)hipFree(ctx->d_sorted);
    HIPCHK(hipMalloc(&ctx->d_sorted, (entries + 1) * 4));
    ctx->cap_entries = entries;
  }
  if (chunks > ctx->cap_chunks) {
    if (ctx->d_desc) (void)hipFree(ctx->d_desc);
    if (ctx->d_sums) (void)hipFree(ctx->d_sums);
    if (ctx->d_order) (void)hipFree(ctx->d_order);
    HIPCHK(hipMalloc(&ctx->d_order, chunks * 4));
    HIPCHK(hipMalloc(&ctx->d_desc, chunks * sizeof(uint2)));
    HIPCHK(hipMalloc(&ctx->d_sums, chunks * sizeof(PointSum)));
    ctx->cap_chunks = chunks;
  }
  {
    const size_t hcap = entries / ((size_t)L * (HEAVY_MIN_CHUNKS - 1)) + 2;
    const size_t z0 = 2 * LEN_BINS + 1, h0 = z0 + (nb_total + 3) / 4, words = h0 + 1 + hcap + 64;
    if (words > ctx->cap_zblock) {
      if (ctx->d_zblock) (void)hipFree(ctx->d_zblock);
      ctx->d_zblock = nullptr; ctx->cap_zblock = 0;
      HIPCHK(hipMalloc(&ctx->d_zblock, words * 4));
      ctx->cap_zblock = words;
    }
    ctx->d_lenhist = ctx->d_zblock;
    ctx->d_any_multi = ctx->d_zblock + 2 * LEN_BINS;
    ctx->d_combined = reinterpret_cast<uint8_t*>(ctx->d_zblock + z0);
    ctx->d_heavy = ctx->d_zblock + h0;
    ctx->cap_heavy = hcap;
    ctx->cap_combined = nb_total;
  }
  if (ctx->use_partition_sort && n <= PART_MAX_N) {
    const size_t nslices = (n + PART_TILE - 1) / PART_TILE;
    const size_t nbc = nlw * 128 * nslices + 1;
    if (entries > ctx->cap_digits) {
      if (ctx->d_digits) (void)hipFree(ctx->d_digits);
      HIPCHK(hipMalloc(&ctx->d_digits, entries * 2 + 16));
      ctx->cap_digits = entries;
    }
    if (entries > ctx->cap_part) {
      if (ctx->d_part) (void)hipFree(ctx->d_part);
      HIPCHK(hipMalloc(&ctx->d_part, (entries + 1) * 4));
      ctx->cap_part = entries;
    }
    if (nlw * 128 > ctx->cap_bigflag) {
      auto F = [](auto*& p) { if (p) { (void)hipFree(p); p = nullptr; } };
      F(ctx->d_bigflag); F(ctx->d_slice_base); F(ctx->d_subbase);
      HIPCHK(hipMalloc(&ctx->d_bigflag, nlw * 128 + 16));
      HIPCHK(hipMalloc(&ctx->d_slice_base, (nlw * 128 + 1) * 4));
      HIPCHK(hipMalloc(&ctx->d_subbase, nlw * 128 * 256 * 4));
      ctx->cap_bigflag = nlw * 128;
    }
    {
      const size_t max_slices = entries / SLICE + nlw * 128 + 1;
      if (max_slices > ctx->cap_slices) {
        if (ctx->d_slicehist) (void)hipFree(ctx->d_slicehist);
        HIPCHK(hipMalloc(&ctx->d_slicehist, max_slices * 256 * 4));
        ctx->cap_slices = max_slices;
      }
    }
    if (nbc > ctx->cap_blockcnt) {
      if (ctx->d_blockcnt) (void)hipFree(ctx->d_blockcnt);
      if (ctx->d_ublocktot) (void)hipFree(ctx->d_ublocktot);
      HIPCHK(hipMalloc(&ctx->d_blockcnt, nbc * 4));
      HIPCHK(hipMalloc(&ctx->d_ublocktot, (nbc / SCAN_ITEMS + 2) * 4));
      ctx->cap_blockcnt = nbc;
    }
  }
  size_t nout = nlw * nitems;
  if (nout * 64 > ctx->cap_partial) {
    if (ctx->d_partial) (void)hipFree(ctx->d_partial);
    HIPCHK(hipMalloc(&ctx->d_partial, nout * 64 * sizeof(PointSum)));
    ctx->cap_partial = nout * 64;
  }
  if (nout > ctx->cap_out) {
    if (ctx->d_out) (void)hipFree(ctx->d_out);
    if (ctx->h_out) (void)hipHostFree(ctx->h_out);
    HIPCHK(hipMalloc(&ctx->d_out, (nout + 1) * sizeof(PointWords)));
    HIPCHK(hipHostMalloc(&ctx->h_out, (nout + 1) * sizeof(PointWords), hipHostMallocMapped | hipHostMallocCoherent));
    HIPCHK(hipHostGetDevicePointer((void**)&ctx->h_out_dev, ctx->h_out, 0));
    ctx->cap_out = nout;
  }
  return CG1_OK;
}

static size_t zblock_clear_bytes(const Ctx* ctx) {
  size_t bytes = (size_t)((ctx->d_heavy + 1) - ctx->d_zblock) * 4;
  bytes = (bytes + 255) & ~(size_t)255;
  const size_t cap = ctx->cap_zblock * 4;
  return bytes < cap ? bytes : cap;
}

static int read_phase_events(Ctx* ctx, int profile) {
  for (int i = 0; i < CG1_NPHASE; ++i) ctx->phase_ms[i] = 0.f;
  if (profile >= 2) {
    for (int i = 0; i < CG1_NPHASE; ++i) HIPCHK(hipEventElapsedTime(&ctx->phase_ms[i], ctx->ev[i], ctx->ev[i + 1]));
  } else if (profile == 1) {
    HIPCHK(hipEventElapsedTime(&ctx->phase_ms[4], ctx->ev[4], ctx->ev[5]));
  }
  return CG1_OK;
}

static cg1h::fe fe_from_words12(const uint32_t w[12]) {
  cg1h::fe r;
  for (int i = 0; i < 6; ++i) r.l[i] = (uint64_t)w[2 * i] | ((uint64_t)w[2 * i + 1] << 32);
  return r;
}
static cg1h::jac jac_from_words(const PointWords& p) {
  if (p.inf) return cg1h::jac_identity();
  return cg1h::jac_from_xyzz(fe_from_words12(p.w[0]), fe_from_words12(p.w[1]), fe_from_words12(p.w[2]), fe_from_words12(p.w[3]));
}

}
```

curdleproofs_pie_amd/csrc/host_g1.cpp:

```cpp
#include "host_g1.h"
#include "bls_consts.h"
#include "fe_mul_x86.h"
#include <cstring>
#include <vector>

namespace cg1h {

typedef unsigned __int128 u128;
using cg1::H_P; using cg1::H_PINV; using cg1::H_R1; using cg1::H_R2;

static inline fe mk(const uint64_t* w) { fe r; for (int i = 0; i < 6; ++i) r.l[i] = w[i]; return r; }

fe fe_zero() { fe r; memset(&r, 0, sizeof r); return r; }
fe fe_one() { return mk(H_R1); }
bool fe_is_zero(const fe& a) { uint64_t o = 0; for (int i = 0; i < 6; ++i) o |= a.l[i]; return o == 0; }
bool fe_eq(const fe& a, const fe& b) { uint64_t o = 0; for (int i = 0; i < 6; ++i) o |= a.l[i] ^ b.l[i]; return o == 0; }

static inline bool geq_p(const uint64_t* a) {
  for (int i = 5; i >= 0; --i) { if (a[i] > H_P[i]) return true; if (a[i] < H_P[i]) return false; }
  return true;
}
static inline void sub_p(uint64_t* a) {
  u128 br = 0;
  for (int i = 0; i < 6; ++i) { u128 t = (u128)a[i] - H_P[i] - br; a[i] = (uint64_t)t; br = (t >> 64) & 1; }
}

bool fe_is_canonical(const fe& a) { return !geq_p(a.l); }

fe fe_add(const fe& a, const fe& b) {
  fe r; u128 c = 0;
  for (int i = 0; i < 6; ++i) { c += (u128)a.l[i] + b.l[i]; r.l[i] = (uint64_t)c; c >>= 64; }
  if (geq_p(r.l)) sub_p(r.l);
  return r;
}
fe fe_sub(const fe& a, const fe& b) {
  fe r; u128 br = 0;
  for (int i = 0; i < 6; ++i) { u128 t = (u128)a.l[i] - b.l[i] - br; r.l[i] = (uint64_t)t; br = (t >> 64) & 1; }
  if (br) { u128 c = 0; for (int i = 0; i < 6; ++i) { c += (u128)r.l[i] + H_P[i]; r.l[i] = (uint64_t)c; c >>= 64; } }
  return r;
}
fe fe_neg(const fe& a) { return fe_is_zero(a) ? a : fe_sub(fe_zero(), a); }

#if defined(__x86_64__)
static const bool g_has_adx = __builtin_cpu_supports("bmi2") && __builtin_cpu_supports("adx");
#endif

fe fe_mul(const fe& a, const fe& b) {
#if defined(__x86_64__)
  if (g_has_adx) {
    fe r;
    fe_mul_adx(r.l, a.l, b.l, H_P, H_PINV);
    if (geq_p(r.l)) sub_p(r.l);
    return r;
  }
#endif
  uint64_t t0 = 0, t1 = 0, t2 = 0, t3 = 0, t4 = 0, t5 = 0;
#pragma GCC unroll 6
  for (int i = 0; i < 6; ++i) {
    const uint64_t bi = b.l[i];
    u128 c = (u128)a.l[0] * bi + t0;
    const uint64_t m = (uint64_t)c * H_PINV;
    u128 d = (u128)m * H_P[0] + (uint64_t)c;
    c >>= 64; d >>= 64;
    c += (u128)a.l[1] * bi + t1; d += (u128)m * H_P[1] + (uint64_t)c; t0 = (uint64_t)d; c >>= 64; d >>= 64;
    c += (u128)a.l[2] * bi + t2; d += (u128)m * H_P[2] + (uint64_t)c; t1 = (uint64_t)d; c >>= 64; d >>= 64;
    c += (u128)a.l[3] * bi + t3; d += (u128)m * H_P[3] + (uint64_t)c; t2 = (uint64_t)d; c >>= 64; d >>= 64;
    c += (u128)a.l[4] * bi + t4; d += (u128)m * H_P[4] + (uint64_t)c; t3 = (uint64_t)d; c >>= 64; d >>= 64;
    c += (u128)a.l[5] * bi + t5; d += (u128)m * H_P[5] + (uint64_t)c; t4 = (uint64_t)d; c >>= 64; d >>= 64;
    t5 = (uint64_t)c + (uint64_t)d;
  }
  fe r; r.l[0] = t0; r.l[1] = t1; r.l[2] = t2; r.l[3] = t3; r.l[4] = t4; r.l[5] = t5;
  if (geq_p(r.l)) sub_p(r.l);
  return r;
}
fe fe_sqr(const fe& a) {
#if defined(__x86_64__)
  if (g_has_adx) {
    fe r;
    fe_sqr_adx(r.l, a.l, H_P, H_PINV);
    if (geq_p(r.l)) sub_p(r.l);
    return r;
  }
#endif
  return fe_mul(a, a);
}

static fe fe_pow(const fe& a, const uint64_t e[6]) {
  fe tab[16];
  tab[1] = a;
  for (int i = 2; i < 16; ++i) tab[i] = (i & 1) ? fe_mul(tab[i - 1], a) : fe_sqr(tab[i / 2]);
  fe r = fe_one();
  bool started = false;
  for (int nib = 95; nib >= 0; --nib) {
    const unsigned d = (unsigned)(e[nib >> 4] >> ((nib & 15) * 4)) & 15u;
    if (started) { r = fe_sqr(r); r = fe_sqr(r); r = fe_sqr(r); r = fe_sqr(r); }
    if (d) { r = started ? fe_mul(r, tab[d]) : tab[d]; started = true; }
  }
  return started ? r : fe_one();
}
fe fe_inv(const fe& a) { return fe_pow(a, cg1::H_INV_EXP); }
bool fe_sqrt(const fe& a, fe& out) {
  fe s = fe_pow(a, cg1::H_SQRT_EXP);
  if (!fe_eq(fe_sqr(s), a)) return false;
  out = s;
  return true;
}

fe fe_from_std(const uint64_t w[6]) { return fe_mul(mk(w), mk(H_R2)); }
void fe_to_std(const fe& a, uint64_t w[6]) {
  fe one = fe_zero(); one.l[0] = 1;
  fe r = fe_mul(a, one);
  for (int i = 0; i < 6; ++i) w[i] = r.l[i];
}
bool fe_from_le48(const uint8_t* b, fe& out) {
  uint64_t w[6];
  for (int i = 0; i < 6; ++i) { uint64_t v = 0; for (int j = 7; j >= 0; --j) v = (v << 8) | b[8 * i + j]; w[i] = v; }
  if (geq_p(w)) return false;
  out = fe_from_std(w);
  return true;
}
void fe_to_le48(const fe& a, uint8_t* b) {
  uint64_t w[6]; fe_to_std(a, w);
  for (int i = 0; i < 6; ++i) for (int j = 0; j < 8; ++j) b[8 * i + j] = (uint8_t)(w[i] >> (8 * j));
}
bool fe_from_be48(const uint8_t* b, fe& out) {
  uint8_t le[48];
  for (int i = 0; i < 48; ++i) le[i] = b[47 - i];
// ... 199 lines not shown
```

curdleproofs_pie_amd/csrc/kernels_accumulate.h:

```cpp
#pragma once

__global__ void __launch_bounds__(256) k_accumulate(const uint2* __restrict__ desc, const uint32_t* __restrict__ total_chunks,
                                                    const uint32_t* __restrict__ order, const uint32_t* __restrict__ sorted,
                                                    const PreparedPoint* __restrict__ pts, PointSum* __restrict__ sums) {
  uint32_t g = blockIdx.x * 256 + threadIdx.x;
  if (g >= *total_chunks) return;
  const uint32_t t = order[g];
  const uint2 d = desc[t];
  const uint32_t* ent = sorted + d.x;
  if (d.y == 0u) { store_sum(sums + t, xyzz_identity()); return; }
  uint32_t e = ent[0];
  fp x, y; uint32_t flags;
  load_affine(pts + (e & 0x7fffffffu), x, y, flags);
  xyzz acc;
  uint32_t j = 1;
  if (e >> 31) y = fp_neg<3>(y);
  if (d.y >= 2u) {
    const uint32_t e1 = ent[1];
    fp x1, y1;
    load_affine(pts + (e1 & 0x7fffffffu), x1, y1, flags);
    if (e1 >> 31) y1 = fp_neg<3>(y1);
    e = ent[d.y > 2u ? 2 : 1];
    fp xn, yn;
    load_affine(pts + (e & 0x7fffffffu), xn, yn, flags);
    acc = xyzz_mmadd(x, y, x1, y1);
    x = xn; y = yn;
    j = 2;
  } else {
    acc = xyzz_from_affine(x, y);
  }
  for (; j < d.y; ++j) {
    const uint32_t en = ent[(j + 1 < d.y) ? j + 1 : j];
    fp xn, yn;
    load_affine(pts + (en & 0x7fffffffu), xn, yn, flags);
    if (e >> 31) y = fp_neg<3>(y);
    if (!xyzz_madd_fast(acc, x, y)) break;
    e = en; x = xn; y = yn;
  }
  for (; j < d.y; ++j) {
    acc = xyzz_madd(acc, x, y);
    if (j + 1 < d.y) {
      e = ent[j + 1];
      load_affine(pts + (e & 0x7fffffffu), x, y, flags);
      if (e >> 31) y = fp_neg<3>(y);
    }
  }
  store_sum(sums + t, acc);
}

__global__ void __launch_bounds__(256) k_heavy_combine(const uint32_t* __restrict__ heavy, uint32_t heavy_cap,
                                                       const uint32_t* __restrict__ choff, PointSum* __restrict__ sums,
                                                       uint8_t* __restrict__ combined) {
  __shared__ PointSum sh[4];
  uint32_t nheavy = heavy[0];
  if (nheavy > heavy_cap) nheavy = heavy_cap;
  for (uint32_t h = blockIdx.x; h < nheavy; h += gridDim.x) {
    const uint32_t b = heavy[1 + h];
    const uint32_t c0 = choff[b], c1 = choff[b + 1];
    xyzz acc = xyzz_identity();
    for (uint32_t k = c0 + threadIdx.x; k < c1; k += 256) acc = xyzz_add(acc, load_sum(sums + k));
    __syncthreads();
    for (int delta = 32; delta >= 1; delta >>= 1) {
      xyzz o = shfl_down_xyzz(acc, delta);
      if ((threadIdx.x & 63) < (uint32_t)delta) acc = xyzz_add(acc, o);
    }
    if ((threadIdx.x & 63) == 0) store_sum(&sh[threadIdx.x >> 6], acc);
    __syncthreads();
    if (threadIdx.x == 0) {
      for (int k = 1; k < 4; ++k) acc = xyzz_add(acc, load_sum(&sh[k]));
      store_sum(sums + c0, acc);
      combined[b] = 1;
    }
    __syncthreads();
  }
}

__global__ void __launch_bounds__(256) k_bucket_fold(const uint32_t* __restrict__ choff, PointSum* __restrict__ sums,
                                                     uint8_t* __restrict__ combined, uint32_t nb_total, const uint32_t* __restrict__ any_multi = nullptr) {
  if (any_multi && *any_multi == 0u) return;
  uint32_t b = blockIdx.x * 256 + threadIdx.x;
  if (b >= nb_total) return;
  const uint32_t c0 = choff[b], c1 = choff[b + 1];
  if (c1 - c0 < 2u || c1 - c0 >= HEAVY_MIN_CHUNKS) return;
  xyzz acc = load_sum(sums + c0);
  for (uint32_t k = c0 + 1; k < c1; ++k) acc = xyzz_add(acc, load_sum(sums + k));
  store_sum(sums + c0, acc);
  combined[b] = 1;
}
```

curdleproofs_pie_amd/csrc/kernels_prepare_digits.h:

```cpp
#pragma once

__global__ void __launch_bounds__(256) k_prepare_points(const uint32_t* __restrict__ raw, PreparedPoint* __restrict__ out,
                                                        uint8_t* __restrict__ inf_flag, uint32_t n, uint32_t* __restrict__ status_words = nullptr) {
  if (status_words && blockIdx.x == 0 && threadIdx.x < 4) status_words[threadIdx.x] = 0;
  __shared__ uint4 stage[256 * 8];
  const uint32_t base = blockIdx.x * 256u, t = threadIdx.x;
  const uint32_t cnt = (n - base < 256u) ? n - base : 256u;
  const uint4* src = reinterpret_cast<const uint4*>(raw + 24ull * base);
  for (uint32_t j = t; j < cnt * 6u; j += 256u) stage[j] = src[j];
  __syncthreads();
  uint32_t o[32];
  if (t < cnt) {
    uint32_t w[24];
#pragma unroll
    for (int k = 0; k < 6; ++k) { uint4 v = stage[t * 6u + k]; w[4 * k] = v.x; w[4 * k + 1] = v.y; w[4 * k + 2] = v.z; w[4 * k + 3] = v.w; }
    uint32_t any = 0;
#pragma unroll
    for (int k = 0; k < 24; ++k) any |= w[k];
    fp x = fp_to_mont(fp_from_words(w));
    fp y = fp_to_mont(fp_from_words(w + 12));
#pragma unroll
    for (int k = 0; k < NL; ++k) { o[k] = x.l[k]; o[NL + k] = y.l[k]; }
    o[28] = any ? 0u : 1u;
    inf_flag[base + t] = any ? 0 : 1;
// ... 93 lines not shown
    store_fp14(o, x);
    store_fp14(o + NL, y);
    reinterpret_cast<uint4*>(o)[7] = make_uint4(0u, 0u, 0u, 0u);
  }
}

struct WinPlan {
  int nwin, cmax, n_hi;
  int glv;
  CG1_HD int width(int w) const { return w < n_hi ? cmax : cmax - 1; }
  CG1_HD int off(int w) const { return w < n_hi ? w * cmax : n_hi * cmax + (w - n_hi) * (cmax - 1); }
};
CG1_HD int win_local(int w, int rank, int sel) {
  const int world = sel & 0xff, lw0 = (sel >> 8) & 0xff, cnt = (sel >> 16) & 0xff;
  if ((w % world) != rank) return -1;
  const int lw = w / world - lw0;
  return (lw >= 0 && (cnt == 0 || lw < cnt)) ? lw : -1;
}
CG1_HD int win_global(int lw, int rank, int sel) { return rank + (lw + ((sel >> 8) & 0xff)) * (sel & 0xff); }
CG1_HD int win_count(int nwin, int rank, int sel) {
  const int world = sel & 0xff, lw0 = (sel >> 8) & 0xff, cnt = (sel >> 16) & 0xff;
  return cnt ? cnt : (nwin - rank + world - 1) / world - lw0;
}
CG1_HD int win_sel(int world, int lw0, int cnt) { return world | (lw0 << 8) | (cnt << 16); }
struct WinWalk {
  int own, lw, world, cnt;
  CG1_HD WinWalk(int rank, int sel) : own(rank), lw(-((sel >> 8) & 0xff)), world(sel & 0xff), cnt((sel >> 16) & 0xff) {}
  CG1_HD int step(int w) {
    if (w != own) return -1;
    const int l = lw;
    own += world; ++lw;
    return (l >= 0 && (cnt == 0 || l < cnt)) ? l : -1;
  }
};

struct DigitIter {
  uint32_t s[8];
  uint32_t carry;
  uint32_t flip;
  __device__ __forceinline__ int next(const WinPlan& pl, int w) {
    const int c = pl.width(w);
    const uint32_t raw = s[0] & ((1u << c) - 1u);
#pragma unroll
    for (int k = 0; k < 7; ++k) s[k] = __builtin_amdgcn_alignbit(s[k + 1], s[k], (uint32_t)c);
    s[7] >>= c;
    uint32_t d = raw + carry;
    int r;
    if (d > (1u << (c - 1)) - flip) { carry = 1; r = (int)d - (1 << c); }
    else { carry = 0; r = (int)d; }
    return flip ? -r : r;
  }
};
__device__ __forceinline__ void load_scalar(const uint32_t* scalars, uint32_t i, DigitIter& it) {
  const uint4* q = reinterpret_cast<const uint4*>(scalars + 8ull * i);
  uint4 a = q[0], b = q[1];
  it.s[0] = a.x; it.s[1] = a.y; it.s[2] = a.z; it.s[3] = a.w;
  it.s[4] = b.x; it.s[5] = b.y; it.s[6] = b.z; it.s[7] = b.w;
  it.carry = 0; it.flip = 0;
}
__device__ __forceinline__ void load_half(const uint32_t (&mag)[4], uint32_t neg, DigitIter& it) {
  it.s[0] = mag[0]; it.s[1] = mag[1]; it.s[2] = mag[2]; it.s[3] = mag[3];
  it.s[4] = it.s[5] = it.s[6] = it.s[7] = 0;
  it.carry = 0; it.flip = neg;
}

__global__ void __launch_bounds__(256) k_phi_records(PreparedPoint* __restrict__ pts, uint8_t* __restrict__ inf_flag, uint32_t n) {
  const uint32_t i = blockIdx.x * 256 + threadIdx.x;
  if (i >= n) return;
  constexpr uint32_t bt[NL] = {D_BETA[0], D_BETA[1], D_BETA[2], D_BETA[3], D_BETA[4], D_BETA[5], D_BETA[6], D_BETA[7], D_BETA[8], D_BETA[9], D_BETA[10], D_BETA[11], D_BETA[12], D_BETA[13]};
  fp beta; for (int k = 0; k < NL; ++k) beta.l[k] = bt[k];
  const uint4* src = reinterpret_cast<const uint4*>(pts + i);
  uint32_t w[32];
#pragma unroll
  for (int k = 0; k < 8; ++k) { const uint4 v = src[k]; w[4 * k] = v.x; w[4 * k + 1] = v.y; w[4 * k + 2] = v.z; w[4 * k + 3] = v.w; }
  fp x; for (int k = 0; k < NL; ++k) x.l[k] = w[k];
  const fp bx = fp_norm(fp_mul(x, beta));
  for (int k = 0; k < NL; ++k) w[k] = bx.l[k];
  uint4* dst = reinterpret_cast<uint4*>(pts + n + i);
#pragma unroll
  for (int k = 0; k < 8; ++k) dst[k] = make_uint4(w[4 * k], w[4 * k + 1], w[4 * k + 2], w[4 * k + 3]);
  inf_flag[n + i] = inf_flag[i];
}

__global__ void __launch_bounds__(256) k_hist(const uint32_t* __restrict__ scalars, const uint8_t* __restrict__ inf_flag,
                                              uint32_t* __restrict__ hist, uint32_t n, WinPlan pl, int rank, int world,
                                              uint32_t* __restrict__ bad_flag) {
  uint32_t i = blockIdx.x * 256 + threadIdx.x;
  if (i >= n) return;
  if (inf_flag[i]) return;
  DigitIter it;
  load_scalar(scalars, i, it);
  if (it.s[7] >> 31) *bad_flag = 1u;
  const uint32_t NB = 1u << (pl.cmax - 1);
  WinWalk ww(rank, world);
  for (int w = 0; w < pl.nwin; ++w) {
    int d = it.next(pl, w);
    const int lw = ww.step(w);
    if (d == 0 || lw < 0) continue;
    uint32_t b = (uint32_t)(d < 0 ? -d : d) - 1u;
    atomicAdd(&hist[(uint32_t)lw * NB + b], 1u);
  }
}

__global__ void __launch_bounds__(256) k_scatter(const uint32_t* __restrict__ scalars, const uint8_t* __restrict__ inf_flag,
                                                 uint32_t* __restrict__ cursor, const uint32_t* __restrict__ off,
                                                 uint32_t* __restrict__ sorted, uint32_t n, WinPlan pl, int rank, int world) {
  uint32_t i = blockIdx.x * 256 + threadIdx.x;
  if (i >= n) return;
  if (inf_flag[i]) return;
  DigitIter it;
  load_scalar(scalars, i, it);
  const uint32_t NB = 1u << (pl.cmax - 1);
  WinWalk ww(rank, world);
  for (int w = 0; w < pl.nwin; ++w) {
    int d = it.next(pl, w);
    const int lw = ww.step(w);
    if (d == 0 || lw < 0) continue;
    uint32_t key = (uint32_t)lw * NB + (uint32_t)(d < 0 ? -d : d) - 1u;
    uint32_t slot = atomicSub(&cursor[key], 1u) - 1u;
    sorted[off[key] + slot] = i | (d < 0 ? 0x80000000u : 0u);
  }
}

constexpr int SCAN_ITEMS = 1024;
```

curdleproofs_pie_amd/csrc/kernels_records.h:

```cpp
#pragma once

struct alignas(16) PreparedPoint {
  uint32_t x[NL];
  uint32_t y[NL];
  uint32_t flags;
  uint32_t pad[3];
};
static_assert(sizeof(PreparedPoint) == 128, "one cache line per point");

struct alignas(16) PointSum {
  uint32_t c[4][NL];
  uint32_t inf;
  uint32_t pad[7];
};
static_assert(sizeof(PointSum) == 256, "");

struct alignas(16) PointWords {
  uint32_t w[4][12];
  uint32_t inf;
  uint32_t pad[3];
};
static_assert(sizeof(PointWords) == 208, "");

__device__ __forceinline__ void load_affine(const PreparedPoint* p, fp& x, fp& y, uint32_t& flags) {
  const uint4* q = reinterpret_cast<const uint4*>(p);
  uint4 v[8];
#pragma unroll
  for (int i = 0; i < 8; ++i) v[i] = q[i];
  const uint32_t* w = reinterpret_cast<const uint32_t*>(v);
#pragma unroll
  for (int i = 0; i < NL; ++i) { x.l[i] = w[i]; y.l[i] = w[NL + i]; }
  flags = w[2 * NL];
}

__device__ __forceinline__ void store_sum(PointSum* dst, const xyzz& a) {
  uint32_t w[64];
#pragma unroll
  for (int i = 0; i < NL; ++i) { w[i] = a.X.l[i]; w[NL + i] = a.Y.l[i]; w[2 * NL + i] = a.ZZ.l[i]; w[3 * NL + i] = a.ZZZ.l[i]; }
  w[4 * NL] = a.inf;
#pragma unroll
  for (int i = 4 * NL + 1; i < 64; ++i) w[i] = 0;
  uint4* q = reinterpret_cast<uint4*>(dst);
#pragma unroll
  for (int i = 0; i < 16; ++i) q[i] = make_uint4(w[4 * i], w[4 * i + 1], w[4 * i + 2], w[4 * i + 3]);
}

__device__ __forceinline__ xyzz load_sum(const PointSum* src) {
  const uint4* q = reinterpret_cast<const uint4*>(src);
  uint32_t w[60];
#pragma unroll
  for (int i = 0; i < 15; ++i) { uint4 v = q[i]; w[4 * i] = v.x; w[4 * i + 1] = v.y; w[4 * i + 2] = v.z; w[4 * i + 3] = v.w; }
  xyzz a;
#pragma unroll
  for (int i = 0; i < NL; ++i) { a.X.l[i] = w[i]; a.Y.l[i] = w[NL + i]; a.ZZ.l[i] = w[2 * NL + i]; a.ZZZ.l[i] = w[3 * NL + i]; }
  a.inf = w[4 * NL];
  return a;
}


__device__ __forceinline__ xyzz shfl_xyzz(const xyzz& a, int src_lane) {
  xyzz r;
#pragma unroll
  for (int i = 0; i < NL; ++i) {
    r.X.l[i] = __shfl(a.X.l[i], src_lane, 64);
    r.Y.l[i] = __shfl(a.Y.l[i], src_lane, 64);
    r.ZZ.l[i] = __shfl(a.ZZ.l[i], src_lane, 64);
    r.ZZZ.l[i] = __shfl(a.ZZZ.l[i], src_lane, 64);
  }
  r.inf = __shfl(a.inf, src_lane, 64);
  return r;
}

__device__ __forceinline__ xyzz shfl_down_xyzz(const xyzz& a, int delta) {
  xyzz r;
#pragma unroll
  for (int i = 0; i < NL; ++i) {
    r.X.l[i] = __shfl_down(a.X.l[i], delta, 64);
    r.Y.l[i] = __shfl_down(a.Y.l[i], delta, 64);
    r.ZZ.l[i] = __shfl_down(a.ZZ.l[i], delta, 64);
    r.ZZZ.l[i] = __shfl_down(a.ZZZ.l[i], delta, 64);
  }
  r.inf = __shfl_down(a.inf, delta, 64);
  return r;
}
```

curdleproofs_pie_amd/csrc/kernels_sort.h:

```cpp
#pragma once

constexpr uint32_t PART_TILE = 4096;
constexpr uint32_t PART_MAX_N = 1u << 23;

__device__ __forceinline__ uint32_t digit_mag(uint32_t e, uint32_t& neg) {
  if (e == 0x8000u) { neg = 0; return 0x8000u; }
  int d = (int)(int16_t)(uint16_t)e;
  neg = d < 0;
  return (uint32_t)(d < 0 ? -d : d);
}

__device__ int g_wave_agg = 1;
__device__ __forceinline__ uint32_t lds_ranked_inc(uint32_t* ctr, uint32_t key, bool active) {
  if (!g_wave_agg) return active ? atomicAdd(&ctr[key], 1u) : 0u;
  const unsigned long long amask = __ballot(active);
  if (amask == 0ull) return 0u;
  const int leader = __ffsll((long long)amask) - 1;
  const uint32_t k0 = __shfl(key, leader, 64);
  if (__ballot(active && key != k0) == 0ull) {
    const uint32_t lane = threadIdx.x & 63u;
    uint32_t base = 0;
    if ((int)lane == leader) base = atomicAdd(&ctr[k0], (uint32_t)__popcll(amask));
    base = __shfl(base, leader, 64);
    return base + (uint32_t)__popcll(amask & ((1ull << lane) - 1ull));
  }
  return active ? atomicAdd(&ctr[key], 1u) : 0u;
}

__global__ void __launch_bounds__(256) k_digits(const uint32_t* __restrict__ scalars, const uint8_t* __restrict__ inf_flag,
                                                uint16_t* __restrict__ digits, uint32_t n, WinPlan pl, int rank, int world,
                                                uint32_t* __restrict__ bad_flag) {
  uint32_t i = blockIdx.x * 256 + threadIdx.x;
  if (i >= n) return;
  const bool inf = inf_flag[i] != 0;
  DigitIter it;
  load_scalar(scalars, i, it);
  if (it.s[7] >> 31) *bad_flag = 1u;
  if (pl.glv) {
    GlvParts g;
    glv_split(it.s, g);
    DigitIter a, b;
    load_half(g.k1, g.neg1, a);
    load_half(g.k2, g.neg2, b);
    const size_t nv = 2 * (size_t)n;
    WinWalk ww(rank, world);
    for (int w = 0; w < pl.nwin; ++w) {
      const int d1 = a.next(pl, w), d2 = b.next(pl, w);
      const int lw = ww.step(w);
      if (lw < 0) continue;
      digits[(size_t)lw * nv + i] = inf ? (uint16_t)0 : (uint16_t)(d1 & 0xFFFF);
      digits[(size_t)lw * nv + n + i] = inf ? (uint16_t)0 : (uint16_t)(d2 & 0xFFFF);
    }
    return;
  }
  WinWalk ww(rank, world);
  for (int w = 0; w < pl.nwin; ++w) {
    int d = it.next(pl, w);
    const int lw = ww.step(w);
    if (lw < 0) continue;
    digits[(size_t)lw * n + i] = inf ? (uint16_t)0 : (uint16_t)(d & 0xFFFF);
  }
}

__global__ void __launch_bounds__(256) k_part_count(const uint16_t* __restrict__ digits, uint32_t* __restrict__ block_counts,
                                                    uint32_t n, uint32_t nslices, uint32_t nbins, uint32_t sub_bits) {
  __shared__ uint32_t cnt[128];
  if (threadIdx.x < 128) cnt[threadIdx.x] = 0;
  __syncthreads();
  const uint32_t slice = blockIdx.x, lw = blockIdx.y;
  const uint16_t* dg = digits + (size_t)lw * n;
  for (uint32_t k = 0; k < PART_TILE / 256; ++k) {
    uint32_t i = slice * PART_TILE + k * 256 + threadIdx.x;
    uint32_t e = (i < n) ? (uint32_t)dg[i] : 0u;
    uint32_t neg, key = e ? ((digit_mag(e, neg) - 1u) >> sub_bits) : 0u;
    lds_ranked_inc(cnt, key, e != 0u);
  }
  __syncthreads();
  if (threadIdx.x < nbins) block_counts[((size_t)lw * nbins + threadIdx.x) * nslices + slice] = cnt[threadIdx.x];
}

__global__ void __launch_bounds__(256) k_part_scatter(const uint16_t* __restrict__ digits, const uint32_t* __restrict__ block_base,
                                                      uint32_t* __restrict__ part, uint32_t n, uint32_t nslices, uint32_t nbins,
                                                      uint32_t sub_bits, int use_stage) {
  __shared__ uint32_t cur[128];
  __shared__ uint32_t gbase[128];
  __shared__ uint32_t lbase[128];
  __shared__ uint32_t stage[PART_TILE];
  __shared__ uint32_t gpos[PART_TILE];
  const uint32_t slice = blockIdx.x, lw = blockIdx.y;
  uint32_t mycnt = 0;
  if (threadIdx.x < nbins) {
    const size_t idx = ((size_t)lw * nbins + threadIdx.x) * nslices + slice;
    gbase[threadIdx.x] = block_base[idx];
    mycnt = block_base[idx + 1] - block_base[idx];
    lbase[threadIdx.x] = mycnt;
  } else if (threadIdx.x < 128) {
    lbase[threadIdx.x] = 0;
  }
  __syncthreads();
  if (use_stage) {
    for (int d = 1; d < 128; d <<= 1) {
      uint32_t u = (threadIdx.x < 128 && (int)threadIdx.x >= d) ? lbase[threadIdx.x - d] : 0u;
      __syncthreads();
      if (threadIdx.x < 128) lbase[threadIdx.x] += u;
      __syncthreads();
    }
    if (threadIdx.x < 128) { lbase[threadIdx.x] -= mycnt; cur[threadIdx.x] = lbase[threadIdx.x]; }
  } else if (threadIdx.x < nbins) {
    cur[threadIdx.x] = gbase[threadIdx.x];
  }
  __syncthreads();
  const uint16_t* dg = digits + (size_t)lw * n;
  const uint32_t sub_mask = (1u << sub_bits) - 1u;
  for (uint32_t k = 0; k < PART_TILE / 256; ++k) {
    uint32_t i = slice * PART_TILE + k * 256 + threadIdx.x;
    uint32_t e = (i < n) ? (uint32_t)dg[i] : 0u;
    uint32_t neg = 0, b = e ? (digit_mag(e, neg) - 1u) : 0u;
    const uint32_t bin = b >> sub_bits;
    uint32_t pos = lds_ranked_inc(cur, bin, e != 0u);
    const uint32_t val = i | (neg << 23) | ((b & sub_mask) << 24);
    if (e) {
      if (use_stage) { stage[pos] = val; gpos[pos] = gbase[bin] + (pos - lbase[bin]); }
      else part[pos] = val;
    }
  }
  if (use_stage) {
    __syncthreads();
    const uint32_t total = lbase[nbins - 1] + (block_base[((size_t)lw * nbins + nbins - 1) * nslices + slice + 1] - gbase[nbins - 1]);
    for (uint32_t o = threadIdx.x; o < total; o += 256) part[gpos[o]] = stage[o];
  }
}
constexpr uint32_t BIN_STAGE = 12288;
__global__ void __launch_bounds__(256) k_bin_sort(const uint32_t* __restrict__ part, const uint32_t* __restrict__ block_base,
                                                  uint32_t* __restrict__ hist, uint32_t* __restrict__ sorted,
                                                  uint32_t nbins_total, uint32_t nslices, uint32_t sub_bits, int use_stage,
                                                  const uint8_t* __restrict__ bigflag) {
  __shared__ uint32_t cnt[256];
  __shared__ uint32_t cur[256];
  __shared__ uint32_t stage[BIN_STAGE];
  const uint32_t g = blockIdx.x;
  if (bigflag[g]) return;
  const uint32_t start = block_base[(size_t)g * nslices];
  const uint32_t end = block_base[(size_t)(g + 1) * nslices];
  cnt[threadIdx.x] = 0;
  __syncthreads();
  const uint32_t span = ((end - start + 255u) / 256u) * 256u;
  for (uint32_t o = threadIdx.x; o < span; o += 256) {
    const bool live = start + o < end;
    lds_ranked_inc(cnt, live ? (part[start + o] >> 24) : 0u, live);
  }
  __syncthreads();
  const uint32_t mine = cnt[threadIdx.x];
  cur[threadIdx.x] = mine;
  __syncthreads();
  for (int d = 1; d < 256; d <<= 1) {
    uint32_t u = ((int)threadIdx.x >= d) ? cur[threadIdx.x - d] : 0u;
    __syncthreads();
    cur[threadIdx.x] += u;
    __syncthreads();
  }
  const uint32_t excl = cur[threadIdx.x] - mine;
  __syncthreads();
  const bool staged = use_stage && (end - start) <= BIN_STAGE;
  cur[threadIdx.x] = (staged ? 0u : start) + excl;
  if (threadIdx.x < (1u << sub_bits)) hist[((size_t)g << sub_bits) + threadIdx.x] = mine;
  __syncthreads();
  for (uint32_t o = threadIdx.x; o < span; o += 256) {
    const bool live = start + o < end;
    const uint32_t v = live ? part[start + o] : 0u;
    const uint32_t pos = lds_ranked_inc(cur, v >> 24, live);
    const uint32_t val = (v & 0x7fffffu) | ((v >> 23 & 1u) << 31);
    if (live) { if (staged) stage[pos] = val; else sorted[pos] = val; }
  }
  if (staged) {
    __syncthreads();
    for (uint32_t o = threadIdx.x; start + o < end; o += 256) sorted[start + o] = stage[o];
  }
}

constexpr uint32_t SLICE = BIN_STAGE;

__global__ void __launch_bounds__(256) k_slice_plan(const uint32_t* __restrict__ block_base, uint32_t nbins_total, uint32_t nslices,
                                                    uint32_t* __restrict__ slice_base ,
                                                    uint8_t* __restrict__ bigflag, int enable) {
  __shared__ uint32_t part_sum[256];
  const uint32_t per = (nbins_total + 255u) / 256u, g0 = threadIdx.x * per;
  uint32_t mine = 0;
  for (uint32_t g = g0; g < g0 + per && g < nbins_total; ++g) {
    const uint32_t size = block_base[(size_t)(g + 1) * nslices] - block_base[(size_t)g * nslices];
    mine += (enable && size > BIN_STAGE) ? (size + SLICE - 1u) / SLICE : 0u;
  }
  part_sum[threadIdx.x] = mine;
  __syncthreads();
  for (int d = 1; d < 256; d <<= 1) {
    uint32_t u = ((int)threadIdx.x >= d) ? part_sum[threadIdx.x - d] : 0u;
    __syncthreads();
    part_sum[threadIdx.x] += u;
    __syncthreads();
  }
  uint32_t run = part_sum[threadIdx.x] - mine;
  for (uint32_t g = g0; g < g0 + per && g < nbins_total; ++g) {
    const uint32_t size = block_base[(size_t)(g + 1) * nslices] - block_base[(size_t)g * nslices];
    const uint32_t ns = (enable && size > BIN_STAGE) ? (size + SLICE - 1u) / SLICE : 0u;
    slice_base[g] = run;
    bigflag[g] = ns ? 1 : 0;
    run += ns;
  }
  if (threadIdx.x == 255) slice_base[nbins_total] = part_sum[255];
}

__device__ __forceinline__ bool slice_of_block(const uint32_t* __restrict__ slice_base, uint32_t nbins_total, uint32_t b,
                                               uint32_t& g, uint32_t& s) {
  if (b >= slice_base[nbins_total]) return false;
  uint32_t lo = 0, hi = nbins_total;
  while (hi - lo > 1) {
    const uint32_t mid = (lo + hi) >> 1;
    if (slice_base[mid] <= b) lo = mid; else hi = mid;
  }
  g = lo;
  s = b - slice_base[lo];
  return true;
}

__global__ void __launch_bounds__(256) k_slice_count(const uint32_t* __restrict__ part, const uint32_t* __restrict__ block_base,
                                                     uint32_t nbins_total, uint32_t nslices, const uint32_t* __restrict__ slice_base,
                                                     uint32_t* __restrict__ slicehist) {
  __shared__ uint32_t cnt[256];
  uint32_t g, s;
  if (!slice_of_block(slice_base, nbins_total, blockIdx.x, g, s)) return;
  const uint32_t start = block_base[(size_t)g * nslices], end = block_base[(size_t)(g + 1) * nslices];
  const uint32_t lo = start + s * SLICE, hi = (lo + SLICE < end) ? lo + SLICE : end;
  cnt[threadIdx.x] = 0;
  __syncthreads();
  const uint32_t span = ((hi - lo + 255u) / 256u) * 256u;
  for (uint32_t o = threadIdx.x; o < span; o += 256) {
    const bool live = lo + o < hi;
    lds_ranked_inc(cnt, live ? (part[lo + o] >> 24) : 0u, live);
  }
  __syncthreads();
  slicehist[(size_t)blockIdx.x * 256u + threadIdx.x] = cnt[threadIdx.x];
}

__global__ void __launch_bounds__(256) k_slice_prefix(const uint32_t* __restrict__ block_base, uint32_t nslices, uint32_t sub_bits,
                                                      const uint32_t* __restrict__ slice_base, const uint8_t* __restrict__ bigflag,
                                                      uint32_t* __restrict__ slicehist, uint32_t* __restrict__ subbase,
                                                      uint32_t* __restrict__ hist) {
  __shared__ uint32_t tot[256];
  const uint32_t g = blockIdx.x;
  if (!bigflag[g]) return;
  const uint32_t b0 = slice_base[g], b1 = slice_base[g + 1];
  uint32_t run = 0;
  for (uint32_t b = b0; b < b1; ++b) {
    const size_t idx = (size_t)b * 256u + threadIdx.x;
    const uint32_t v = slicehist[idx];
    slicehist[idx] = run;
    run += v;
  }
  tot[threadIdx.x] = run;
  __syncthreads();
  for (int d = 1; d < 256; d <<= 1) {
    uint32_t u = ((int)threadIdx.x >= d) ? tot[threadIdx.x - d] : 0u;
    __syncthreads();
    tot[threadIdx.x] += u;
    __syncthreads();
  }
  subbase[(size_t)g * 256u + threadIdx.x] = block_base[(size_t)g * nslices] + tot[threadIdx.x] - run;
  if (threadIdx.x < (1u << sub_bits)) hist[((size_t)g << sub_bits) + threadIdx.x] = run;
}

__global__ void __launch_bounds__(256) k_slice_scatter(const uint32_t* __restrict__ part, const uint32_t* __restrict__ block_base,
                                                       uint32_t nbins_total, uint32_t nslices, const uint32_t* __restrict__ slice_base,
                                                       const uint32_t* __restrict__ slicehist, const uint32_t* __restrict__ subbase,
                                                       uint32_t* __restrict__ sorted) {
  __shared__ uint32_t cnt[256];
  __shared__ uint32_t cur[256];
  __shared__ uint32_t gdst[256];
  __shared__ uint32_t stage[SLICE];
  uint32_t g, s;
  if (!slice_of_block(slice_base, nbins_total, blockIdx.x, g, s)) return;
  const uint32_t start = block_base[(size_t)g * nslices], end = block_base[(size_t)(g + 1) * nslices];
  const uint32_t lo = start + s * SLICE, hi = (lo + SLICE < end) ? lo + SLICE : end;
  cnt[threadIdx.x] = 0;
  __syncthreads();
  const uint32_t span = ((hi - lo + 255u) / 256u) * 256u;
  for (uint32_t o = threadIdx.x; o < span; o += 256) {
    const bool live = lo + o < hi;
    lds_ranked_inc(cnt, live ? (part[lo + o] >> 24) : 0u, live);
  }
  __syncthreads();
  const uint32_t mine = cnt[threadIdx.x];
  __syncthreads();
  for (int d = 1; d < 256; d <<= 1) {
    uint32_t u = ((int)threadIdx.x >= d) ? cnt[threadIdx.x - d] : 0u;
    __syncthreads();
    cnt[threadIdx.x] += u;
    __syncthreads();
  }
  const uint32_t lbase = cnt[threadIdx.x] - mine;
  __syncthreads();
  cnt[threadIdx.x] = lbase;
  cur[threadIdx.x] = lbase;
  gdst[threadIdx.x] = subbase[(size_t)g * 256u + threadIdx.x] + slicehist[(size_t)blockIdx.x * 256u + threadIdx.x];
  __syncthreads();
  for (uint32_t o = threadIdx.x; o < span; o += 256) {
    const bool live = lo + o < hi;
    const uint32_t v = live ? part[lo + o] : 0u;
    const uint32_t pos = lds_ranked_inc(cur, v >> 24, live);
    if (live) stage[pos] = v;
  }
  __syncthreads();
  for (uint32_t o = threadIdx.x; o < hi - lo; o += 256) {
    const uint32_t v = stage[o], k = v >> 24;
    sorted[gdst[k] + (o - cnt[k])] = (v & 0x7fffffu) | ((v >> 23 & 1u) << 31);
  }
}

__global__ void __launch_bounds__(256) k_uscan1(uint32_t* __restrict__ a, uint32_t* __restrict__ block_tot, uint32_t n) {
  __shared__ uint32_t sh[256];
  uint32_t base = blockIdx.x * SCAN_ITEMS + threadIdx.x * 4;
  uint32_t v[4], local = 0;
#pragma unroll
  for (int k = 0; k < 4; ++k) { v[k] = (base + k < n) ? a[base + k] : 0u; local += v[k]; }
  sh[threadIdx.x] = local;
  __syncthreads();
  for (int d = 1; d < 256; d <<= 1) {
    uint32_t u = ((int)threadIdx.x >= d) ? sh[threadIdx.x - d] : 0u;
    __syncthreads();
    sh[threadIdx.x] += u;
    __syncthreads();
  }
  uint32_t excl = sh[threadIdx.x] - local;
#pragma unroll
  for (int k = 0; k < 4; ++k) { if (base + k < n) a[base + k] = excl; excl += v[k]; }
  if (threadIdx.x == 255) block_tot[blockIdx.x] = sh[255];
}
__global__ void __launch_bounds__(256) k_uscan2(uint32_t* __restrict__ block_tot, uint32_t nblocks, uint32_t* __restrict__ a, uint32_t n) {
  __shared__ uint32_t sh[256];
  uint32_t carry = 0;
  for (uint32_t tile = 0; tile < nblocks; tile += 256) {
    uint32_t i = tile + threadIdx.x;
    uint32_t v = (i < nblocks) ? block_tot[i] : 0u;
    sh[threadIdx.x] = v;
    __syncthreads();
    for (int d = 1; d < 256; d <<= 1) {
      uint32_t u = ((int)threadIdx.x >= d) ? sh[threadIdx.x - d] : 0u;
      __syncthreads();
      sh[threadIdx.x] += u;
      __syncthreads();
    }
    if (i < nblocks) block_tot[i] = carry + sh[threadIdx.x] - v;
    uint32_t tot = sh[255];
    __syncthreads();
    carry += tot;
  }
  if (threadIdx.x == 0) a[n] = carry;
}
__global__ void __launch_bounds__(256) k_uscan3(const uint32_t* __restrict__ block_tot, uint32_t* __restrict__ a, uint32_t n) {
  uint32_t base = blockIdx.x * SCAN_ITEMS + threadIdx.x * 4;
  uint32_t p = block_tot[blockIdx.x];
#pragma unroll
  for (int k = 0; k < 4; ++k) if (base + k < n) a[base + k] += p;
}

constexpr uint32_t USCAN1_MAX = 1u << 15;
__global__ void __launch_bounds__(1024) k_uscan_one(uint32_t* __restrict__ a, uint32_t n) {
  __shared__ uint32_t sh[1024];
  const uint32_t per = (n + 1023u) / 1024u, lo = threadIdx.x * per, hi = (lo + per < n) ? lo + per : n;
  uint32_t local = 0;
  for (uint32_t i = lo; i < hi; ++i) local += a[i];
  sh[threadIdx.x] = local;
  __syncthreads();
  for (int d = 1; d < 1024; d <<= 1) {
    uint32_t u = ((int)threadIdx.x >= d) ? sh[threadIdx.x - d] : 0u;
    __syncthreads();
    sh[threadIdx.x] += u;
    __syncthreads();
  }
  uint32_t excl = sh[threadIdx.x] - local;
  for (uint32_t i = lo; i < hi; ++i) { const uint32_t v = a[i]; a[i] = excl; excl += v; }
  if (threadIdx.x == 1023) a[n] = sh[1023];
}

__global__ void __launch_bounds__(256) k_group_count(const uint16_t* __restrict__ digits, const uint32_t* __restrict__ offs,
                                                     uint32_t* __restrict__ hist, uint32_t N, uint32_t NB, uint32_t nwin, uint32_t split) {
  __shared__ uint32_t cnt[256];
  cnt[threadIdx.x] = 0;
  __syncthreads();
  const uint32_t j = blockIdx.x, w = blockIdx.y;
  const uint32_t o0 = offs[j], o1 = offs[j + 1];
  const uint32_t span = ((o1 - o0 + 255u) / 256u) * 256u;
  for (uint32_t half = 0; half < (split ? 2u : 1u); ++half) {
    const uint16_t* dg = digits + (size_t)w * N + (size_t)half * split;
    for (uint32_t o = threadIdx.x; o < span; o += 256) {
      const uint32_t e = (o0 + o < o1) ? (uint32_t)dg[o0 + o] : 0u;
      uint32_t neg;
      lds_ranked_inc(cnt, e ? digit_mag(e, neg) - 1u : 0u, e != 0u);
    }
  }
  __syncthreads();
  if (threadIdx.x < NB) hist[((size_t)j * nwin + w) * NB + threadIdx.x] = cnt[threadIdx.x];
}

__global__ void __launch_bounds__(256) k_group_scatter(const uint16_t* __restrict__ digits, const uint32_t* __restrict__ offs,
                                                       const uint32_t* __restrict__ off, uint32_t* __restrict__ sorted,
                                                       uint32_t N, uint32_t NB, uint32_t nwin, uint32_t split) {
  __shared__ uint32_t cur[256];
  const uint32_t j = blockIdx.x, w = blockIdx.y;
  if (threadIdx.x < NB) cur[threadIdx.x] = off[((size_t)j * nwin + w) * NB + threadIdx.x];
  __syncthreads();
  const uint32_t o0 = offs[j], o1 = offs[j + 1];
  const uint16_t* dg = digits + (size_t)w * N;
  const uint32_t span = ((o1 - o0 + 255u) / 256u) * 256u;
  for (uint32_t half = 0; half < (split ? 2u : 1u); ++half) {
    for (uint32_t o = threadIdx.x; o < span; o += 256) {
      const uint32_t i = half * split + o0 + o;
      const uint32_t e = (o0 + o < o1) ? (uint32_t)dg[i] : 0u;
      uint32_t neg = 0;
      const uint32_t b = e ? digit_mag(e, neg) - 1u : 0u;
      const uint32_t pos = lds_ranked_inc(cur, b, e != 0u);
      if (e) sorted[pos] = i | (neg << 31);
    }
  }
}

__global__ void __launch_bounds__(256) k_group_reduce(const PointSum* __restrict__ seg_run, const PointSum* __restrict__ seg_tot,
                                                      PointSum* __restrict__ group_sum, uint32_t ngroups, uint32_t J, uint32_t log2m) {
  uint32_t g = blockIdx.x * 256 + threadIdx.x;
  if (g >= ngroups) return;
  const PointSum* run = seg_run + (size_t)g * J;
  const PointSum* tot = seg_tot + (size_t)g * J;
  xyzz r = xyzz_identity(), t = xyzz_identity();
  for (uint32_t s = J - 1; s >= 1; --s) { r = xyzz_add(r, load_sum(run + s)); t = xyzz_add(t, r); }
  for (uint32_t k = 0; k < log2m; ++k) t = xyzz_dbl(t);
  for (uint32_t s = 0; s < J; ++s) t = xyzz_add(t, load_sum(tot + s));
  store_sum(group_sum + g, t);
}

__global__ void __launch_bounds__(64) k_msm_horner(const PointSum* __restrict__ group_sum, PointWords* __restrict__ out,
                                                   uint32_t M, uint32_t nwin, uint32_t c) {
  uint32_t j = blockIdx.x * 64 + threadIdx.x;
  if (j >= M) return;
  xyzz acc = xyzz_identity();
  for (int w = (int)nwin - 1; w >= 0; --w) {
    for (uint32_t k = 0; k < c; ++k) acc = xyzz_dbl(acc);
    acc = xyzz_add(acc, load_sum(group_sum + (size_t)j * nwin + w));
  }
  xyzz_words o;
  xyzz_export(acc, o);
  PointWords* dst = out + j;
  for (int cidx = 0; cidx < 4; ++cidx) for (int k = 0; k < 12; ++k) dst->w[cidx][k] = o.w[cidx][k];
  dst->inf = o.inf;
}

constexpr uint32_t MAX_CHUNKS_PER_BUCKET = 4096;
constexpr uint32_t HEAVY_MIN_CHUNKS = 17;
__device__ __forceinline__ uint32_t chunk_len(uint32_t cnt, uint32_t L0) {
  uint32_t s = (cnt + MAX_CHUNKS_PER_BUCKET - 1) / MAX_CHUNKS_PER_BUCKET;
  return s > L0 ? s : L0;
}
__device__ __forceinline__ uint32_t chunk_count(uint32_t cnt, uint32_t L0) {
  if (cnt == 0) return 0;
  uint32_t L = chunk_len(cnt, L0);
  return (cnt + L - 1) / L;
}

__global__ void __launch_bounds__(256) k_scan1(const uint32_t* __restrict__ hist, uint32_t* __restrict__ off, uint32_t* __restrict__ choff,
                                               uint2* __restrict__ block_tot, uint32_t nb_total, uint32_t L0) {
  __shared__ uint2 sh[256];
  uint32_t base = blockIdx.x * SCAN_ITEMS + threadIdx.x * 4;
  uint32_t cnt[4], ch[4];
  uint2 local = make_uint2(0, 0);
#pragma unroll
  for (int k = 0; k < 4; ++k) {
    cnt[k] = (base + k < nb_total) ? hist[base + k] : 0u;
    ch[k] = chunk_count(cnt[k], L0);
    local.x += cnt[k]; local.y += ch[k];
  }
  sh[threadIdx.x] = local;
  __syncthreads();
  for (int d = 1; d < 256; d <<= 1) {
    uint2 v = make_uint2(0, 0);
    if ((int)threadIdx.x >= d) v = sh[threadIdx.x - d];
    __syncthreads();
    sh[threadIdx.x].x += v.x; sh[threadIdx.x].y += v.y;
    __syncthreads();
  }
  uint2 excl = make_uint2(sh[threadIdx.x].x - local.x, sh[threadIdx.x].y - local.y);
#pragma unroll
  for (int k = 0; k < 4; ++k) {
    if (base + k < nb_total) { off[base + k] = excl.x; choff[base + k] = excl.y; }
    excl.x += cnt[k]; excl.y += ch[k];
  }
  if (threadIdx.x == 255) block_tot[blockIdx.x] = sh[255];
}
__global__ void __launch_bounds__(256) k_scan2(uint2* __restrict__ block_tot, uint32_t nblocks, uint32_t* __restrict__ off,
                                               uint32_t* __restrict__ choff, uint32_t nb_total) {
  __shared__ uint2 sh[256];
  uint2 carry = make_uint2(0, 0);
  for (uint32_t tile = 0; tile < nblocks; tile += 256) {
    uint32_t i = tile + threadIdx.x;
    uint2 v = (i < nblocks) ? block_tot[i] : make_uint2(0, 0);
    sh[threadIdx.x] = v;
    __syncthreads();
    for (int d = 1; d < 256; d <<= 1) {
      uint2 u = make_uint2(0, 0);
      if ((int)threadIdx.x >= d) u = sh[threadIdx.x - d];
      __syncthreads();
      sh[threadIdx.x].x += u.x; sh[threadIdx.x].y += u.y;
      __syncthreads();
    }
    if (i < nblocks) block_tot[i] = make_uint2(carry.x + sh[threadIdx.x].x - v.x, carry.y + sh[threadIdx.x].y - v.y);
    uint2 tot = sh[255];
    __syncthreads();
    carry.x += tot.x; carry.y += tot.y;
  }
  if (threadIdx.x == 0) { off[nb_total] = carry.x; choff[nb_total] = carry.y; }
}
__global__ void __launch_bounds__(256) k_scan3(const uint2* __restrict__ block_tot, uint32_t* __restrict__ off,
                                               uint32_t* __restrict__ choff, uint32_t nb_total) {
  uint32_t base = blockIdx.x * SCAN_ITEMS + threadIdx.x * 4;
  uint2 p = block_tot[blockIdx.x];
#pragma unroll
  for (int k = 0; k < 4; ++k) if (base + k < nb_total) { off[base + k] += p.x; choff[base + k] += p.y; }
}

constexpr uint32_t LEN_BINS = 256;
__device__ __forceinline__ uint32_t len_key(uint32_t len) { return len < LEN_BINS - 1 ? len : LEN_BINS - 1; }

constexpr uint32_t SCAN1_MAX = 1u << 13;
__global__ void __launch_bounds__(1024) k_scan_one(const uint32_t* __restrict__ hist, uint32_t* __restrict__ off, uint32_t* __restrict__ choff,
                                                    uint32_t nb_total, uint32_t L0) {
  __shared__ uint2 sh[1024];
  const uint32_t per = (nb_total + 1023u) / 1024u, lo = threadIdx.x * per, hi = (lo + per < nb_total) ? lo + per : nb_total;
  uint2 local = make_uint2(0, 0);
  for (uint32_t i = lo; i < hi; ++i) { const uint32_t c = hist[i]; local.x += c; local.y += chunk_count(c, L0); }
  sh[threadIdx.x] = local;
  __syncthreads();
  for (int d = 1; d < 1024; d <<= 1) {
    uint2 v = make_uint2(0, 0);
    if ((int)threadIdx.x >= d) v = sh[threadIdx.x - d];
    __syncthreads();
    sh[threadIdx.x].x += v.x; sh[threadIdx.x].y += v.y;
    __syncthreads();
  }
  uint2 excl = make_uint2(sh[threadIdx.x].x - local.x, sh[threadIdx.x].y - local.y);
  for (uint32_t i = lo; i < hi; ++i) {
    const uint32_t c = hist[i];
    off[i] = excl.x; choff[i] = excl.y;
    excl.x += c; excl.y += chunk_count(c, L0);
  }
  if (threadIdx.x == 1023) { off[nb_total] = sh[1023].x; choff[nb_total] = sh[1023].y; }
}

constexpr uint32_t CHUNK_DESC_BLOCKS = 320;
__global__ void __launch_bounds__(256) k_chunk_desc(const uint32_t* __restrict__ off, const uint32_t* __restrict__ choff,
                                                    uint2* __restrict__ desc, uint32_t* __restrict__ len_hist,
                                                    uint32_t* __restrict__ heavy ,
                                                    uint32_t heavy_cap, uint32_t nb_total, uint32_t L0, uint32_t* __restrict__ any_multi = nullptr) {
  __shared__ uint32_t sh[LEN_BINS];
  sh[threadIdx.x] = 0;
  __syncthreads();
#pragma unroll 1
  for (uint32_t b = blockIdx.x * 256 + threadIdx.x; b - threadIdx.x < nb_total; b += gridDim.x * 256) {
  if (b < nb_total) {
    uint32_t start = off[b], cnt = off[b + 1] - start;
    if (cnt) {
      uint32_t L = chunk_len(cnt, L0), nch = (cnt + L - 1) / L, o = choff[b];
      for (uint32_t k = 0; k < nch; ++k) {
        uint32_t s = k * L, len = (cnt - s < L) ? (cnt - s) : L;
        desc[o + k] = make_uint2(start + s, len);
      }
      if (nch > 1u) atomicAdd(&sh[len_key(L)], nch - 1u);
      atomicAdd(&sh[len_key(cnt - (nch - 1u) * L)], 1u);
      if (nch >= HEAVY_MIN_CHUNKS) {
        uint32_t slot = atomicAdd(&heavy[0], 1u);
        if (slot < heavy_cap) heavy[1 + slot] = b;
      } else if (nch >= 2u && any_multi) {
        *any_multi = 1u;
      }
    }
  }
  }
  __syncthreads();
  uint32_t v = sh[threadIdx.x];
  if (v) atomicAdd(&len_hist[threadIdx.x], v);
}

__global__ void __launch_bounds__(256) k_len_scan(const uint32_t* __restrict__ len_hist, uint32_t* __restrict__ len_cursor,
                                                  const uint32_t* __restrict__ total_entries, const uint32_t* __restrict__ total_chunks,
                                                  uint32_t* __restrict__ stats) {
  __shared__ uint32_t sh[LEN_BINS];
  if (threadIdx.x == 0) { stats[1] = *total_entries; stats[2] = *total_chunks; }
  uint32_t rev = LEN_BINS - 1 - threadIdx.x;
  uint32_t v = len_hist[rev];
  sh[threadIdx.x] = v;
  __syncthreads();
  for (int d = 1; d < 256; d <<= 1) {
    uint32_t u = ((int)threadIdx.x >= d) ? sh[threadIdx.x - d] : 0u;
    __syncthreads();
    sh[threadIdx.x] += u;
    __syncthreads();
  }
  len_cursor[rev] = sh[threadIdx.x] - v;
}

constexpr uint32_t ORDER_PER = 8;
__global__ void __launch_bounds__(256) k_order(const uint2* __restrict__ desc, const uint32_t* __restrict__ total_chunks,
                                               uint32_t* __restrict__ len_cursor, uint32_t* __restrict__ order) {
  __shared__ uint32_t cnt[LEN_BINS];
  __shared__ uint32_t base[LEN_BINS];
  cnt[threadIdx.x] = 0;
  __syncthreads();
  const uint32_t total = *total_chunks;
  uint32_t key[ORDER_PER], local[ORDER_PER];
#pragma unroll
  for (uint32_t rep = 0; rep < ORDER_PER; ++rep) {
    const uint32_t t = (blockIdx.x * ORDER_PER + rep) * 256 + threadIdx.x;
    const bool live = t < total;
    key[rep] = live ? len_key(desc[t].y) : 0u;
    local[rep] = 0;
    const unsigned long long amask = __ballot(live);
    if (amask) {
      const int leader = __ffsll((long long)amask) - 1;
      const uint32_t k0 = __shfl(key[rep], leader, 64);
      const unsigned long long same = __ballot(live && key[rep] == k0);
      const uint32_t lane = threadIdx.x & 63u;
      uint32_t b0 = 0;
      if ((int)lane == leader) b0 = atomicAdd(&cnt[k0], (uint32_t)__popcll(same));
      b0 = __shfl(b0, leader, 64);
      if (live) local[rep] = (key[rep] == k0) ? b0 + (uint32_t)__popcll(same & ((1ull << lane) - 1ull)) : atomicAdd(&cnt[key[rep]], 1u);
    }
  }
  __syncthreads();
  const uint32_t c = cnt[threadIdx.x];
  if (c) base[threadIdx.x] = atomicAdd(&len_cursor[threadIdx.x], c);
  __syncthreads();
#pragma unroll
  for (uint32_t rep = 0; rep < ORDER_PER; ++rep) {
    const uint32_t t = (blockIdx.x * ORDER_PER + rep) * 256 + threadIdx.x;
    if (t < total) order[base[key[rep]] + local[rep]] = t;
  }
}
```

curdleproofs_pie_amd/csrc/msm_gpu.hip:

```cpp
#include <hip/hip_runtime.h>
#include <cstdint>
#include <cstdio>
#include <cstring>
#include <cmath>
#include <vector>
#include <string>
#include <algorithm>
#include <atomic>
#include <chrono>
#include <condition_variable>
#include <functional>
#include <mutex>
#include <thread>
#include "g1_xyzz.h"
#include "g1_quad.h"
#include "host_g1.h"
#include "lazy_host.h"
#include "pool.h"
#include "../../include/curdle_g1.h"

namespace cg1 {

int pick_window(size_t n);

#include "kernels_records.h"
#include "fp_row.h"
#include "glv.h"
#include "kernels_prepare_digits.h"
#include "kernels_sort.h"
#include "kernels_accumulate.h"
#include "kernels_reduce.h"
#include "kernels_small.h"
#include "kernels_batch.h"
#include "kernels_generator.h"
#include "fixed_digits.h"
#include "kernels_fixed.h"
#include "light_digits.h"
#include "kernels_light.h"
}
#include "kernels_rows.h"
#include "kernels_merlin.h"
#include "kernels_frontend.h"
#include "kernels_opening.h"
#include "kernels_ipa.h"
#include "kernels_same_msm.h"
#include "host_context.h"
#include "host_chains.h"
#include "capi_core_msm.h"
#include "capi_vec_batched.h"
#include "capi_lincomb.h"
#include "capi_timing_batchmul.h"
#include "capi_codec_transcripts.h"
#include "capi_frontend.h"
#include "capi_rows_probes.h"
#include "capi_fixed.h"
#include "capi_ipa.h"
#include "capi_light.h"
#include "capi_same_msm.h"
```

Measured before the change: 371.2 million.

## Fuse MSM sort-pipeline kernels and widen host Horner split to eight threads

Several small launches in the bucket-sort pipeline are folded away. The scan second pass moves into a last-block-ticket tail of the first pass, the length histogram and its scan move into the scan kernels, k_order is merged into k_chunk_desc, slice planning moves into part_scatter, zblock clearing moves into the digit kernel, and heavy combine is joined with the bucket fold. The aim is to cut kernel-launch and serialization overhead on the critical path. The host Horner tail is factored into a shared helper that can use up to eight threads. The trade-offs are the extra atomics and ticket synchronization the fusions need, and possible ordering subtleties.

```diff
diff --git a/curdleproofs_pie_amd/build.py b/curdleproofs_pie_amd/build.py
--- a/curdleproofs_pie_amd/build.py
+++ b/curdleproofs_pie_amd/build.py
@@ -9,7 +9,7 @@
 CSRC = os.path.join(HERE, "csrc")
 LIB = os.path.join(HERE, "libcurdle_g1.so")
 SOURCES = [os.path.join(CSRC, "msm_gpu.hip"), os.path.join(CSRC, "host_g1.cpp"), os.path.join(CSRC, "merlin.cpp"), os.path.join(CSRC, "shuffle_verify.cpp"), os.path.join(CSRC, "comm.cpp"), os.path.join(CSRC, "lazy_host.cpp")]
-DEPS = SOURCES + [os.path.join(CSRC, f) for f in ("kernels_opening.h", "kernels_generator.h", "kernels_fixed.h", "fixed_digits.h", "capi_fixed.h", "kernels_light.h", "light_digits.h", "capi_light.h", "kernels_ipa.h", "ipa_rounds.h", "capi_ipa.h", "kernels_same_msm.h", "same_msm_rounds.h", "capi_same_msm.h", "fp28.h", "g1_xyzz.h", "g1_quad.h", "host_g1.h", "fe_mul_x86.h", "fr.h", "merlin_group.h", "bls_consts.h", "kernels_records.h", "kernels_prepare_digits.h",
+DEPS = SOURCES + [os.path.join(CSRC, f) for f in ("kernels_opening.h", "kernels_generator.h", "kernels_fixed.h", "fixed_digits.h", "capi_fixed.h", "kernels_light.h", "light_digits.h", "capi_light.h", "kernels_ipa.h", "ipa_rounds.h", "capi_ipa.h", "kernels_same_msm.h", "same_msm_rounds.h", "capi_same_msm.h", "fp28.h", "g1_xyzz.h", "g1_quad.h", "host_g1.h", "host_horner.h", "fe_mul_x86.h", "fr.h", "merlin_group.h", "bls_consts.h", "kernels_records.h", "kernels_prepare_digits.h",
                                                     "kernels_sort.h", "kernels_accumulate.h", "kernels_reduce.h", "kernels_small.h", "kernels_batch.h", "kernels_rows.h", "kernels_merlin.h", "kernels_frontend.h", "pool.h", "lazy_host.h", "fp_row.h", "glv.h", "host_context.h", "host_chains.h", "capi_core_msm.h", "capi_vec_batched.h", "capi_lincomb.h",
                                                     "capi_timing_batchmul.h", "capi_codec_transcripts.h", "capi_frontend.h", "capi_rows_probes.h")] + [
     os.path.join(HERE, "..", "include", "curdle_g1.h")
diff --git a/curdleproofs_pie_amd/csrc/capi_core_msm.h b/curdleproofs_pie_amd/csrc/capi_core_msm.h
--- a/curdleproofs_pie_amd/csrc/capi_core_msm.h
+++ b/curdleproofs_pie_amd/csrc/capi_core_msm.h
@@ -297,7 +297,7 @@
   if (!strcmp(name, "big_bins")) { ctx->big_bins = value != 0; return CG1_OK; }
   if (!strcmp(name, "host_split")) { ctx->host_split = value != 0; return CG1_OK; }
   if (!strcmp(name, "arm_helpers")) { ctx->arm_helpers = value != 0; return CG1_OK; }
-  if (!strcmp(name, "horner_threads")) { if (value != 1 && value != 2 && value != 4) return CG1_ERR_ARG; ctx->horner_threads = value; return CG1_OK; }
+  if (!strcmp(name, "horner_threads")) { if (value != 1 && value != 2 && value != 4 && value != 8) return CG1_ERR_ARG; ctx->horner_threads = value; return CG1_OK; }
   if (!strcmp(name, "zero_copy")) { ctx->zero_copy = value != 0; return CG1_OK; }
   if (!strcmp(name, "auto_plan")) { ctx->auto_plan = value != 0; return CG1_OK; }
   if (!strcmp(name, "rowcol_quad")) { ctx->rowcol_quad = value != 0; return CG1_OK; }
diff --git a/curdleproofs_pie_amd/csrc/host_chains.h b/curdleproofs_pie_amd/csrc/host_chains.h
--- a/curdleproofs_pie_amd/csrc/host_chains.h
+++ b/curdleproofs_pie_amd/csrc/host_chains.h
@@ -129,21 +129,20 @@
     const uint32_t nbins = 1u << (bb - sub_bits);
     const uint32_t nslices = (n32 + PART_TILE - 1) / PART_TILE;
     const uint32_t nbc = (uint32_t)nlw * nbins * nslices;
-    hipLaunchKernelGGL(k_digits, dim3((n_real32 + 255) / 256), dim3(256), 0, st, (const uint32_t*)d_scalars32, flags, ctx->d_digits, n_real32, plan, rank, world, bad_flag);
+    hipLaunchKernelGGL(k_digits, dim3((n_real32 + 255) / 256), dim3(256), 0, st, (const uint32_t*)d_scalars32, flags, ctx->d_digits, n_real32, plan, rank, world, bad_flag, ctx->d_zblock, zblock_clear_words(ctx));
     hipLaunchKernelGGL(k_part_count, dim3(nslices, nlw), dim3(256), 0, st, ctx->d_digits, ctx->d_blockcnt, n32, nslices, nbins, sub_bits);
     const uint32_t ublk = (nbc + SCAN_ITEMS - 1) / SCAN_ITEMS;
     if (ctx->scan_one && nbc <= USCAN1_MAX) {
       hipLaunchKernelGGL(k_uscan_one, dim3(1), dim3(1024), 0, st, ctx->d_blockcnt, nbc);
     } else {
-      hipLaunchKernelGGL(k_uscan1, dim3(ublk), dim3(256), 0, st, ctx->d_blockcnt, ctx->d_ublocktot, nbc);
-      hipLaunchKernelGGL(k_uscan2, dim3(1), dim3(256), 0, st, ctx->d_ublocktot, ublk, ctx->d_blockcnt, nbc);
+      hipLaunchKernelGGL(k_uscan1, dim3(ublk), dim3(256), 0, st, ctx->d_blockcnt, ctx->d_ublocktot, nbc, ctx->d_ticket);
       hipLaunchKernelGGL(k_uscan3, dim3(ublk), dim3(256), 0, st, ctx->d_ublocktot, ctx->d_blockcnt, nbc);
     }
     if (profile >= 2) HIPCHK(hipEventRecord(ctx->ev[2], st));
-    hipLaunchKernelGGL(k_part_scatter, dim3(nslices, nlw), dim3(256), 0, st, ctx->d_digits, ctx->d_blockcnt, ctx->d_part, n32, nslices, nbins, sub_bits, ctx->stage_sort);
     const uint32_t nbt = (uint32_t)nlw * nbins;
     const int big_bins = ctx->big_bins && n32 > 2u * BIN_STAGE;
-    hipLaunchKernelGGL(k_slice_plan, dim3(1), dim3(256), 0, st, ctx->d_blockcnt, nbt, nslices, ctx->d_slice_base, ctx->d_bigflag, big_bins);
+    hipLaunchKernelGGL(k_part_scatter, dim3(nslices, nlw), dim3(256), 0, st, ctx->d_digits, ctx->d_blockcnt, ctx->d_part, n32, nslices, nbins, sub_bits, ctx->stage_sort,
+                       ctx->d_slice_base, ctx->d_bigflag, big_bins);
     hipLaunchKernelGGL(k_bin_sort, dim3(nbt), dim3(256), 0, st, ctx->d_part, ctx->d_blockcnt, ctx->d_hist, ctx->d_sorted, nbt, nslices, sub_bits, ctx->stage_sort, ctx->d_bigflag);
     if (big_bins) {
       const uint32_t max_slices = (uint32_t)(((size_t)n * (size_t)nlw) / SLICE + nbt + 1);
@@ -153,41 +152,39 @@
     }
     if (profile >= 2) HIPCHK(hipEventRecord(ctx->ev[3], st));
     if (ctx->scan_one && nb_total <= SCAN1_MAX) {
-      hipLaunchKernelGGL(k_scan_one, dim3(1), dim3(1024), 0, st, ctx->d_hist, ctx->d_off, ctx->d_choff, (uint32_t)nb_total, L0);
+      hipLaunchKernelGGL(k_scan_one, dim3(1), dim3(1024), 0, st, ctx->d_hist, ctx->d_off, ctx->d_choff, (uint32_t)nb_total, L0, ctx->d_lenhist + LEN_BINS, bad_flag);
     } else {
-      hipLaunchKernelGGL(k_scan1, dim3(nblk), dim3(256), 0, st, ctx->d_hist, ctx->d_off, ctx->d_choff, ctx->d_blocktot, (uint32_t)nb_total, L0);
-      hipLaunchKernelGGL(k_scan2, dim3(1), dim3(256), 0, st, ctx->d_blocktot, nblk, ctx->d_off, ctx->d_choff, (uint32_t)nb_total);
+      hipLaunchKernelGGL(k_scan1, dim3(nblk), dim3(256), 0, st, ctx->d_hist, ctx->d_off, ctx->d_choff, ctx->d_blocktot, (uint32_t)nb_total, L0,
+                         ctx->d_lenhist, ctx->d_lenhist + LEN_BINS, ctx->d_ticket + 1, bad_flag);
       hipLaunchKernelGGL(k_scan3, dim3(nblk), dim3(256), 0, st, ctx->d_blocktot, ctx->d_off, ctx->d_choff, (uint32_t)nb_total);
     }
   } else {
     HIPCHK(hipMemsetAsync(ctx->d_hist, 0, nb_total * 4, st));
-    hipLaunchKernelGGL(k_hist, dim3(gn), dim3(256), 0, st, (const uint32_t*)d_scalars32, flags, ctx->d_hist, n32, plan, rank, world, bad_flag);
+    hipLaunchKernelGGL(k_hist, dim3(gn), dim3(256), 0, st, (const uint32_t*)d_scalars32, flags, ctx->d_hist, n32, plan, rank, world, bad_flag, ctx->d_zblock, zblock_clear_words(ctx));
     if (profile >= 2) HIPCHK(hipEventRecord(ctx->ev[2], st));
-    hipLaunchKernelGGL(k_scan1, dim3(nblk), dim3(256), 0, st, ctx->d_hist, ctx->d_off, ctx->d_choff, ctx->d_blocktot, (uint32_t)nb_total, L0);
-    hipLaunchKernelGGL(k_scan2, dim3(1), dim3(256), 0, st, ctx->d_blocktot, nblk, ctx->d_off, ctx->d_choff, (uint32_t)nb_total);
+    hipLaunchKernelGGL(k_scan1, dim3(nblk), dim3(256), 0, st, ctx->d_hist, ctx->d_off, ctx->d_choff, ctx->d_blocktot, (uint32_t)nb_total, L0,
+                       ctx->d_lenhist, ctx->d_lenhist + LEN_BINS, ctx->d_ticket + 1, bad_flag);
     hipLaunchKernelGGL(k_scan3, dim3(nblk), dim3(256), 0, st, ctx->d_blocktot, ctx->d_off, ctx->d_choff, (uint32_t)nb_total);
     if (profile >= 2) HIPCHK(hipEventRecord(ctx->ev[3], st));
     hipLaunchKernelGGL(k_scatter, dim3(gn), dim3(256), 0, st, (const uint32_t*)d_scalars32, flags, ctx->d_hist, ctx->d_off, ctx->d_sorted, n32, plan, rank, world);
   }
-  HIPCHK(hipMemsetAsync(ctx->d_zblock, 0, zblock_clear_bytes(ctx), st));
-  hipLaunchKernelGGL(k_chunk_desc, dim3((uint32_t)std::min<size_t>(CHUNK_DESC_BLOCKS, (nb_total + 255) / 256)), dim3(256), 0, st, ctx->d_off, ctx->d_choff, ctx->d_desc, ctx->d_lenhist, ctx->d_heavy, (uint32_t)ctx->cap_heavy, (uint32_t)nb_total, L0, ctx->d_any_multi);
+  hipLaunchKernelGGL(k_chunk_desc, dim3((uint32_t)std::min<size_t>(CHUNK_DESC_BLOCKS, (nb_total + 255) / 256)), dim3(256), 0, st, ctx->d_off, ctx->d_choff, ctx->d_desc,
+                     ctx->d_lenhist + LEN_BINS, ctx->d_order, ctx->d_heavy, (uint32_t)ctx->cap_heavy, (uint32_t)nb_total, L0, ctx->d_any_multi);
   const size_t max_chunks = nb_total + (n * (size_t)nlw) / L0 + 1;
   const uint32_t gchunks = (uint32_t)((max_chunks + 255) / 256);
-  hipLaunchKernelGGL(k_len_scan, dim3(1), dim3(256), 0, st, ctx->d_lenhist, ctx->d_lenhist + LEN_BINS, ctx->d_off + nb_total, ctx->d_choff + nb_total, bad_flag);
-  hipLaunchKernelGGL(k_order, dim3((gchunks + ORDER_PER - 1) / ORDER_PER), dim3(256), 0, st, ctx->d_desc, ctx->d_choff + nb_total, ctx->d_lenhist + LEN_BINS, ctx->d_order);
   if (hooks.before_accumulate) HIPCHK(hipStreamWaitEvent(st, hooks.before_accumulate, 0));
   if (profile >= 1) HIPCHK(hipEventRecord(ctx->ev[4], st));
   hipLaunchKernelGGL(k_accumulate, dim3(gchunks), dim3(256), 0, st, ctx->d_desc, ctx->d_choff + nb_total, ctx->d_order, ctx->d_sorted, pts, ctx->d_sums);
   if (profile >= 1) HIPCHK(hipEventRecord(ctx->ev[5], st));
   if (hooks.after_accumulate) HIPCHK(hipEventRecord(hooks.after_accumulate, st));
-  hipLaunchKernelGGL(k_heavy_combine, dim3(512), dim3(256), 0, st, ctx->d_heavy, (uint32_t)ctx->cap_heavy, ctx->d_choff, ctx->d_sums, ctx->d_combined);
   const bool small_quad = ctx->quad && ctx->rowcol_quad && nb_total <= (size_t)ctx->rowcol_quad_max;
   const bool rows_fold = small_quad && use2d && ctx->rowcol_row && ctx->tree_row && nb_total <= 8192;
-  if (rows_fold) {}
-  else if (small_quad && ctx->fold_quad)
+  const bool quad_fold = !rows_fold && small_quad && ctx->fold_quad;
+  const int lane_fold = (!rows_fold && !quad_fold && ctx->fold_pass) ? 1 : 0;
+  hipLaunchKernelGGL(k_chunk_join, dim3(lane_fold ? std::max<uint32_t>(512u, (uint32_t)((nb_total + 255) / 256)) : 512u), dim3(256), 0, st, ctx->d_heavy, (uint32_t)ctx->cap_heavy,
+                     ctx->d_choff, ctx->d_sums, ctx->d_combined, (uint32_t)nb_total, ctx->d_any_multi, lane_fold);
+  if (quad_fold)
     hipLaunchKernelGGL(k_bucket_fold_quad, dim3((uint32_t)((nb_total * 4 + 255) / 256)), dim3(256), 0, st, ctx->d_choff, ctx->d_sums, ctx->d_combined, (uint32_t)nb_total, ctx->d_any_multi);
-  else if (ctx->fold_pass)
-    hipLaunchKernelGGL(k_bucket_fold, dim3((uint32_t)((nb_total + 255) / 256)), dim3(256), 0, st, ctx->d_choff, ctx->d_sums, ctx->d_combined, (uint32_t)nb_total, ctx->d_any_multi);
   bool tree_exports = false;
   if (use2d) {
     const uint32_t R = 1u << hb2, Cn = 1u << lb2;
@@ -262,9 +259,9 @@
   const size_t nout_words = pd.nout_words;
   const auto h0 = pd.h0, h1 = pd.h1;
   HIPCHK(hipSetDevice(ctx->device));
-  struct StandDown { Ctx* c; bool on; ~StandDown() { if (on) for (int j = 0; j < 3; ++j) c->helper[j].disarm(); } } stand_down{ctx, false};
+  struct StandDown { Ctx* c; bool on; ~StandDown() { if (on) for (int j = 0; j < HORNER_MAX_PARTS - 1; ++j) c->helper[j].disarm(); } } stand_down{ctx, false};
   if (pd.zero_copy && !ctx->blocking_sync && pd.profile < 2) {
-    if (pd.arm_helpers) for (int j = 0; j < 3 && j + 1 < ctx->horner_threads; ++j) ctx->helper[j].arm();
+    if (pd.arm_helpers) for (int j = 0; j < HORNER_MAX_PARTS - 1 && j + 1 < ctx->horner_threads; ++j) ctx->helper[j].arm();
     stand_down.on = pd.arm_helpers;
     volatile uint32_t* flag = ctx->h_flag;
     for (uint32_t spins = 0; *flag != pd.seq; ++spins) {
@@ -298,14 +295,14 @@
   ctx->host_ms[2] = std::chrono::duration<float, std::milli>(t0 - h2).count();
   int lm = 0; while ((1u << lm) < m) ++lm;
   const WinPlan& plan = pd.plan;
-  constexpr int EMAX = 2 * 256 + 64;
-  std::vector<std::pair<int, const PointWords*>> items;
-  items.reserve((size_t)nlw * nitems);
+  std::vector<const PointWords*> pts;
+  std::vector<int> exps;
+  pts.reserve((size_t)nlw * nitems); exps.reserve((size_t)nlw * nitems);
   int e_top = 0;
   for (int lw = 0; lw < nlw; ++lw) {
     const int w = win_global(lw, rank, world), base = plan.off(w);
     const PointWords* row = pd.hout + (size_t)lw * nitems;
-    auto put = [&](int e, const PointWords* p) { if (!p->inf && e >= 0 && e < EMAX) { items.emplace_back(e, p); if (e > e_top) e_top = e; } };
+    auto put = [&](int e, const PointWords* p) { if (!p->inf && e >= 0 && e < HORNER_EMAX) { pts.push_back(p); exps.push_back(e); if (e > e_top) e_top = e; } };
     put(base, &row[0]);
     if (use2d) {
       for (uint32_t k = 0; k < hb2; ++k) put(base + (int)lb2 + (int)k, &row[1 + k]);
@@ -314,64 +311,10 @@
       for (int b2 = 0; b2 < nbits; ++b2) put(base + lm + b2, &row[1 + b2]);
     }
   }
-  uint16_t first[EMAX + 1];
-  memset(first, 0, sizeof first);
-  for (const auto& it : items) ++first[it.first + 1];
-  for (int e = 0; e < EMAX; ++e) first[e + 1] = (uint16_t)(first[e + 1] + first[e]);
-  std::vector<const PointWords*> byexp(items.size());
-  {
-    uint16_t cur[EMAX];
-    memcpy(cur, first, sizeof cur);
-    for (const auto& it : items) byexp[cur[it.first]++] = it.second;
-  }
-  auto horner = [&](int lo, int hi) {
-    cg1h::jac a = cg1h::jac_identity();
-    for (int e = hi; e >= lo; --e) {
-      a = cg1h::jac_dbl(a);
-      for (uint16_t k = first[e]; k < first[e + 1]; ++k) a = cg1h::jac_add(a, jac_from_words(*byexp[k]));
-    }
-    return a;
-  };
-  cg1h::jac acc;
-  const int nth = (!ctx->host_split || e_top < 96) ? 1 : (ctx->horner_threads >= 4 && e_top >= 112 ? 4 : 2);
-  if (nth > 1) {
-    cg1h::jac part[4];
-    int lo[5];
-    {
-      constexpr long DBL = 7, ADD = 16;
-      auto fill = [&](long C, int* cut) {
-        int e = 0;
-        for (int j = 0; j < nth; ++j) {
-          cut[j] = e;
-          long adds = 0;
-          while (e <= e_top && DBL * (e + 1) + ADD * (adds + (first[e + 1] - first[e])) <= C) { adds += first[e + 1] - first[e]; ++e; }
-        }
-        cut[nth] = e_top + 1;
-        return e > e_top;
-      };
-      long lo_c = DBL * (e_top + 1), hi_c = DBL * (e_top + 1) + ADD * (long)items.size();
-      int cut[5];
-      while (lo_c < hi_c) {
-        const long mid = (lo_c + hi_c) / 2;
-        if (fill(mid, cut)) hi_c = mid; else lo_c = mid + 1;
-      }
-      fill(hi_c, cut);
-      for (int j = 0; j <= nth; ++j) lo[j] = cut[j];
-    }
-    auto run_part = [&](int j) {
-      cg1h::jac a = horner(lo[j], lo[j + 1] - 1);
-      for (int k = 0; k < lo[j]; ++k) a = cg1h::jac_dbl(a);
-      part[j] = a;
-    };
-    for (int j = 0; j + 1 < nth; ++j) ctx->helper[j].run([&, j]() { run_part(j); });
-    if (pd.arm_helpers) for (int j = nth - 1 < 0 ? 0 : nth - 1; j < 3; ++j) ctx->helper[j].disarm();
-    run_part(nth - 1);
-    acc = part[nth - 1];
-    for (int j = 0; j + 1 < nth; ++j) { ctx->helper[j].wait(); acc = cg1h::jac_add(acc, part[j]); }
-  } else {
-    if (pd.arm_helpers) for (int j = 0; j < 3; ++j) ctx->helper[j].disarm();
-    acc = horner(0, e_top);
-  }
+  const int wide = ctx->horner_threads >= 8 ? 8 : 4;
+  const int nth = (!ctx->host_split || e_top < 96) ? 1 : (ctx->horner_threads >= 4 && e_top >= 112 ? wide : 2);
+  if (pd.arm_helpers) for (int j = nth - 1 < 0 ? 0 : nth - 1; j < HORNER_MAX_PARTS - 1; ++j) ctx->helper[j].disarm();
+  const cg1h::jac acc = horner_sum(pts.data(), exps.data(), pts.size(), nth, ctx->helper);
   result = acc;
   ctx->host_tail_ms = std::chrono::duration<float, std::milli>(std::chrono::steady_clock::now() - t0).count();
   ctx->host_ms[3] = ctx->host_tail_ms;
@@ -444,34 +387,18 @@
 }
 
 static cg1h::jac horner_2d_items(const PointWords* rows, const WinPlan& plan, uint32_t nitems, uint32_t hb2, uint32_t lb2) {
-  constexpr int EMAX = 2 * 256 + 64;
-  std::vector<std::pair<int, const PointWords*>> items;
-  items.reserve((size_t)plan.nwin * nitems);
-  int e_top = 0;
+  std::vector<const PointWords*> pts;
+  std::vector<int> exps;
+  pts.reserve((size_t)plan.nwin * nitems); exps.reserve((size_t)plan.nwin * nitems);
   for (int w = 0; w < plan.nwin; ++w) {
     const int base = plan.off(w);
     const PointWords* row = rows + (size_t)w * nitems;
-    auto put = [&](int e, const PointWords* p) { if (!p->inf) { items.emplace_back(e, p); if (e > e_top) e_top = e; } };
+    auto put = [&](int e, const PointWords* p) { if (!p->inf) { pts.push_back(p); exps.push_back(e); } };
     put(base, &row[0]);
     for (uint32_t k = 0; k < hb2; ++k) put(base + (int)lb2 + (int)k, &row[1 + k]);
     for (uint32_t k = 0; k < lb2; ++k) put(base + (int)k, &row[1 + hb2 + k]);
   }
-  uint16_t first[EMAX + 1];
-  memset(first, 0, sizeof first);
-  for (const auto& it : items) ++first[it.first + 1];
-  for (int e = 0; e < EMAX; ++e) first[e + 1] = (uint16_t)(first[e + 1] + first[e]);
-  std::vector<const PointWords*> byexp(items.size());
-  {
-    uint16_t cur[EMAX];
-    memcpy(cur, first, sizeof cur);
-    for (const auto& it : items) byexp[cur[it.first]++] = it.second;
-  }
-  cg1h::jac a = cg1h::jac_identity();
-  for (int e = e_top; e >= 0; --e) {
-    a = cg1h::jac_dbl(a);
-    for (uint16_t k = first[e]; k < first[e + 1]; ++k) a = cg1h::jac_add(a, jac_from_words(*byexp[k]));
-  }
-  return a;
+  return horner_sum(pts.data(), exps.data(), pts.size(), 1, nullptr);
 }
 
 static int msm_small_batched_finish(Ctx* ctx, uint32_t M, std::vector<cg1h::jac>& results) {
@@ -654,28 +581,26 @@
   hipLaunchKernelGGL(k_prepare_points, dim3(gn), dim3(256), 0, st, (const uint32_t*)d_points96, ctx->d_pts, ctx->d_flags, N32, bad_flag);
   if (glv) hipLaunchKernelGGL(k_phi_records, dim3(gn), dim3(256), 0, st, ctx->d_pts, ctx->d_flags, N32);
   if (ctx->profile >= 2) HIPCHK(hipEventRecord(ctx->ev[1], st));
-  hipLaunchKernelGGL(k_digits, dim3(gn), dim3(256), 0, st, (const uint32_t*)d_scalars32, ctx->d_flags, ctx->d_digits, N32, bplan, 0, 1, bad_flag);
+  hipLaunchKernelGGL(k_digits, dim3(gn), dim3(256), 0, st, (const uint32_t*)d_scalars32, ctx->d_flags, ctx->d_digits, N32, bplan, 0, 1, bad_flag, ctx->d_zblock, zblock_clear_words(ctx));
   hipLaunchKernelGGL(k_group_count, dim3((uint32_t)M, nwin), dim3(256), 0, st, ctx->d_digits, ctx->d_boffs, ctx->d_hist, Nv32, NB, nwin, split);
   if (ctx->profile >= 2) HIPCHK(hipEventRecord(ctx->ev[2], st));
   const uint32_t nblk = (uint32_t)((nb_total + SCAN_ITEMS - 1) / SCAN_ITEMS);
-  hipLaunchKernelGGL(k_scan1, dim3(nblk), dim3(256), 0, st, ctx->d_hist, ctx->d_off, ctx->d_choff, ctx->d_blocktot, (uint32_t)nb_total, L0);
-  hipLaunchKernelGGL(k_scan2, dim3(1), dim3(256), 0, st, ctx->d_blocktot, nblk, ctx->d_off, ctx->d_choff, (uint32_t)nb_total);
+  hipLaunchKernelGGL(k_scan1, dim3(nblk), dim3(256), 0, st, ctx->d_hist, ctx->d_off, ctx->d_choff, ctx->d_blocktot, (uint32_t)nb_total, L0,
+                     ctx->d_lenhist, ctx->d_lenhist + LEN_BINS, ctx->d_ticket + 1, bad_flag);
   hipLaunchKernelGGL(k_scan3, dim3(nblk), dim3(256), 0, st, ctx->d_blocktot, ctx->d_off, ctx->d_choff, (uint32_t)nb_total);
   hipLaunchKernelGGL(k_group_scatter, dim3((uint32_t)M, nwin), dim3(256), 0, st, ctx->d_digits, ctx->d_boffs, ctx->d_off, ctx->d_sorted, Nv32, NB, nwin, split);
   if (ctx->profile >= 2) HIPCHK(hipEventRecord(ctx->ev[3], st));
-  HIPCHK(hipMemsetAsync(ctx->d_zblock, 0, zblock_clear_bytes(ctx), st));
-  hipLaunchKernelGGL(k_chunk_desc, dim3((uint32_t)std::min<size_t>(CHUNK_DESC_BLOCKS, (nb_total + 255) / 256)), dim3(256), 0, st, ctx->d_off, ctx->d_choff, ctx->d_desc, ctx->d_lenhist, ctx->d_heavy, (uint32_t)ctx->cap_heavy, (uint32_t)nb_total, L0, ctx->d_any_multi);
+  hipLaunchKernelGGL(k_chunk_desc, dim3((uint32_t)std::min<size_t>(CHUNK_DESC_BLOCKS, (nb_total + 255) / 256)), dim3(256), 0, st, ctx->d_off, ctx->d_choff, ctx->d_desc,
+                     ctx->d_lenhist + LEN_BINS, ctx->d_order, ctx->d_heavy, (uint32_t)ctx->cap_heavy, (uint32_t)nb_total, L0, ctx->d_any_multi);
   const size_t max_chunks = nb_total + (Nv * (size_t)nwin) / L0 + 1;
   const uint32_t gchunks = (uint32_t)((max_chunks + 255) / 256);
-  hipLaunchKernelGGL(k_len_scan, dim3(1), dim3(256), 0, st, ctx->d_lenhist, ctx->d_lenhist + LEN_BINS, ctx->d_off + nb_total, ctx->d_choff + nb_total, bad_flag);
-  hipLaunchKernelGGL(k_order, dim3((gchunks + ORDER_PER - 1) / ORDER_PER), dim3(256), 0, st, ctx->d_desc, ctx->d_choff + nb_total, ctx->d_lenhist + LEN_BINS, ctx->d_order);
   if (wait_before_accumulate) HIPCHK(hipStreamWaitEvent(st, wait_before_accumulate, 0));
   if (ctx->profile >= 1) HIPCHK(hipEventRecord(ctx->ev[4], st));
   hipLaunchKernelGGL(k_accumulate, dim3(gchunks), dim3(256), 0, st, ctx->d_desc, ctx->d_choff + nb_total, ctx->d_order, ctx->d_sorted, ctx->d_pts, ctx->d_sums);
   if (ctx->profile >= 1) HIPCHK(hipEventRecord(ctx->ev[5], st));
   if (record_after_accumulate) HIPCHK(hipEventRecord(record_after_accumulate, st));
   const uint32_t nseg_total = (uint32_t)(nb_total / m);
-  hipLaunchKernelGGL(k_heavy_combine, dim3(512), dim3(256), 0, st, ctx->d_heavy, (uint32_t)ctx->cap_heavy, ctx->d_choff, ctx->d_sums, ctx->d_combined);
+  hipLaunchKernelGGL(k_chunk_join, dim3(512), dim3(256), 0, st, ctx->d_heavy, (uint32_t)ctx->cap_heavy, ctx->d_choff, ctx->d_sums, ctx->d_combined, (uint32_t)nb_total, ctx->d_any_multi, 0);
   hipLaunchKernelGGL(k_seg_reduce, dim3((nseg_total + 255) / 256), dim3(256), 0, st, ctx->d_choff, ctx->d_sums, ctx->d_combined, ctx->d_segrun, ctx->d_segtot, nseg_total, m);
   hipLaunchKernelGGL(k_group_reduce, dim3((uint32_t)((G + 255) / 256)), dim3(256), 0, st, ctx->d_segrun, ctx->d_segtot, ctx->d_gsum, (uint32_t)G, J, log2m);
   if (ctx->profile >= 2) HIPCHK(hipEventRecord(ctx->ev[6], st));
diff --git a/curdleproofs_pie_amd/csrc/host_context.h b/curdleproofs_pie_amd/csrc/host_context.h
--- a/curdleproofs_pie_amd/csrc/host_context.h
+++ b/curdleproofs_pie_amd/csrc/host_context.h
@@ -5,69 +5,9 @@
 #define HIPCHK(x) do { hipError_t e_ = (x); if (e_ != hipSuccess) { \
   snprintf(ctx->err, sizeof ctx->err, "%s failed: %s (%s:%d)", #x, hipGetErrorString(e_), __FILE__, __LINE__); return CG1_ERR_HIP; } } while (0)
 
-struct Helper {
-  std::thread th;
-  std::mutex mu;
-  std::condition_variable cv;
-  std::function<void()> job;
-  bool has = false, done = true, quit = false, armed = false;
-  std::atomic<bool> posted{false};
-  std::atomic<bool> stand_down{false};
-  void start_locked() { if (!th.joinable()) th = std::thread([this]() { loop(); }); }
-  void run(std::function<void()> f) {
-    std::unique_lock<std::mutex> lk(mu);
-    start_locked();
-    job = std::move(f); has = true; done = false;
-    posted.store(true, std::memory_order_release);
-    cv.notify_all();
-  }
-  void arm() {
-    std::unique_lock<std::mutex> lk(mu);
-    start_locked();
-    if (!has && done) { stand_down.store(false, std::memory_order_relaxed); armed = true; cv.notify_all(); }
-  }
-  void disarm() { stand_down.store(true, std::memory_order_release); }
-  void wait() {
-    std::unique_lock<std::mutex> lk(mu);
-    cv.wait(lk, [this]() { return done; });
-  }
-  void loop() {
-    std::unique_lock<std::mutex> lk(mu);
-    for (;;) {
-      cv.wait(lk, [this]() { return has || quit || armed; });
-      if (quit) return;
-      if (!has) {
-        armed = false;
-        lk.unlock();
-        const auto until = std::chrono::steady_clock::now() + std::chrono::milliseconds(2);
-        for (uint32_t k = 0; !posted.load(std::memory_order_acquire); ++k) {
-          if (stand_down.load(std::memory_order_acquire)) break;
-          if ((k & 0xffu) == 0xffu && std::chrono::steady_clock::now() > until) break;
-          __builtin_ia32_pause();
-        }
-        lk.lock();
-        if (!has) continue;
-      }
-      armed = false;
-      std::function<void()> f = std::move(job);
-      has = false;
-      posted.store(false, std::memory_order_relaxed);
-      lk.unlock();
-      f();
-      lk.lock();
-      done = true;
-      cv.notify_all();
-    }
-  }
-  ~Helper() {
-    { std::unique_lock<std::mutex> lk(mu); quit = true; cv.notify_all(); }
-    if (th.joinable()) th.join();
-  }
-};
-
 struct Ctx {
   int device = 0;
-  Helper helper[3];
+  Helper helper[HORNER_MAX_PARTS - 1];
   hipStream_t stream = nullptr;
   std::atomic<hipStream_t> copy_stream{nullptr};
   std::once_flag copy_once;
@@ -86,6 +26,7 @@
   uint32_t *d_order = nullptr, *d_lenhist = nullptr;
   uint32_t* d_zblock = nullptr; size_t cap_zblock = 0;
   uint32_t* d_any_multi = nullptr;
+  uint32_t* d_ticket = nullptr;
   PointSum* d_partial = nullptr; size_t cap_partial = 0;
   uint16_t* d_digits = nullptr; uint32_t* d_part = nullptr; uint32_t* d_blockcnt = nullptr; uint32_t* d_ublocktot = nullptr;
   size_t cap_digits = 0, cap_part = 0, cap_blockcnt = 0;
@@ -197,7 +138,7 @@
   auto F = [](auto*& p) { if (p) { (void)hipFree(p); p = nullptr; } };
   F(c->d_pts); F(c->d_flags); F(c->d_hist); F(c->d_off); F(c->d_choff); F(c->d_sorted); F(c->d_blocktot); F(c->d_desc);
   F(c->d_sums); F(c->d_segrun); F(c->d_segtot); F(c->d_out); F(c->d_order); F(c->d_zblock); F(c->d_partial);
-  c->d_lenhist = c->d_heavy = c->d_any_multi = nullptr; c->d_combined = nullptr; c->cap_zblock = 0; c->cap_heavy = 0; c->cap_combined = 0;
+  c->d_lenhist = c->d_heavy = c->d_any_multi = c->d_ticket = nullptr; c->d_combined = nullptr; c->cap_zblock = 0; c->cap_heavy = 0; c->cap_combined = 0;
   c->cap_partial = 0;
   F(c->d_digits); F(c->d_part); F(c->d_blockcnt); F(c->d_ublocktot); F(c->d_boffs); F(c->d_gsum); F(c->d_bout);
   F(c->d_slice_base); F(c->d_slicehist); F(c->d_subbase); F(c->d_bigflag); c->cap_bigflag = 0; c->cap_slices = 0;
@@ -249,7 +190,7 @@
   }
   {
     const size_t hcap = entries / ((size_t)L * (HEAVY_MIN_CHUNKS - 1)) + 2;
-    const size_t z0 = 2 * LEN_BINS + 1, h0 = z0 + (nb_total + 3) / 4, words = h0 + 1 + hcap + 64;
+    const size_t z0 = 2 * LEN_BINS + 4, h0 = z0 + (nb_total + 3) / 4, words = h0 + 1 + hcap;
     if (words > ctx->cap_zblock) {
       if (ctx->d_zblock) (void)hipFree(ctx->d_zblock);
       ctx->d_zblock = nullptr; ctx->cap_zblock = 0;
@@ -258,6 +199,7 @@
     }
     ctx->d_lenhist = ctx->d_zblock;
     ctx->d_any_multi = ctx->d_zblock + 2 * LEN_BINS;
+    ctx->d_ticket = ctx->d_zblock + 2 * LEN_BINS + 1;
     ctx->d_combined = reinterpret_cast<uint8_t*>(ctx->d_zblock + z0);
     ctx->d_heavy = ctx->d_zblock + h0;
     ctx->cap_heavy = hcap;
@@ -317,11 +259,8 @@
   return CG1_OK;
 }
 
-static size_t zblock_clear_bytes(const Ctx* ctx) {
-  size_t bytes = (size_t)((ctx->d_heavy + 1) - ctx->d_zblock) * 4;
-  bytes = (bytes + 255) & ~(size_t)255;
-  const size_t cap = ctx->cap_zblock * 4;
-  return bytes < cap ? bytes : cap;
+static uint32_t zblock_clear_words(const Ctx* ctx) {
+  return (uint32_t)((ctx->d_heavy + 1) - ctx->d_zblock);
 }
 
 static int read_phase_events(Ctx* ctx, int profile) {
@@ -334,14 +273,4 @@
   return CG1_OK;
 }
 
-static cg1h::fe fe_from_words12(const uint32_t w[12]) {
-  cg1h::fe r;
-  for (int i = 0; i < 6; ++i) r.l[i] = (uint64_t)w[2 * i] | ((uint64_t)w[2 * i + 1] << 32);
-  return r;
-}
-static cg1h::jac jac_from_words(const PointWords& p) {
-  if (p.inf) return cg1h::jac_identity();
-  return cg1h::jac_from_xyzz(fe_from_words12(p.w[0]), fe_from_words12(p.w[1]), fe_from_words12(p.w[2]), fe_from_words12(p.w[3]));
-}
-
-}
+}
diff --git a/curdleproofs_pie_amd/csrc/host_g1.cpp b/curdleproofs_pie_amd/csrc/host_g1.cpp
--- a/curdleproofs_pie_amd/csrc/host_g1.cpp
+++ b/curdleproofs_pie_amd/csrc/host_g1.cpp
@@ -42,7 +42,11 @@
 fe fe_neg(const fe& a) { return fe_is_zero(a) ? a : fe_sub(fe_zero(), a); }
 
 #if defined(__x86_64__)
+#if defined(__SANITIZE_THREAD__)
+static const bool g_has_adx = false;
+#else
 static const bool g_has_adx = __builtin_cpu_supports("bmi2") && __builtin_cpu_supports("adx");
+#endif
 #endif
 
 fe fe_mul(const fe& a, const fe& b) {
diff --git a/curdleproofs_pie_amd/csrc/host_horner.h b/curdleproofs_pie_amd/csrc/host_horner.h
--- /dev/null
+++ b/curdleproofs_pie_amd/csrc/host_horner.h
@@ -0,0 +1,155 @@
+#pragma once
+#include <atomic>
+#include <chrono>
+#include <condition_variable>
+#include <cstdint>
+#include <cstring>
+#include <functional>
+#include <mutex>
+#include <thread>
+#include <vector>
+#include "host_g1.h"
+
+namespace cg1 {
+
+struct alignas(16) PointWords {
+  uint32_t w[4][12];
+  uint32_t inf;
+  uint32_t pad[3];
+};
+static_assert(sizeof(PointWords) == 208, "");
+
+static cg1h::fe fe_from_words12(const uint32_t w[12]) {
+  cg1h::fe r;
+  for (int i = 0; i < 6; ++i) r.l[i] = (uint64_t)w[2 * i] | ((uint64_t)w[2 * i + 1] << 32);
+  return r;
+}
+static cg1h::jac jac_from_words(const PointWords& p) {
+  if (p.inf) return cg1h::jac_identity();
+  return cg1h::jac_from_xyzz(fe_from_words12(p.w[0]), fe_from_words12(p.w[1]), fe_from_words12(p.w[2]), fe_from_words12(p.w[3]));
+}
+
+struct Helper {
+  std::thread th;
+  std::mutex mu;
+  std::condition_variable cv;
+  std::function<void()> job;
+  bool has = false, done = true, quit = false, armed = false;
+  std::atomic<bool> posted{false};
+  std::atomic<bool> stand_down{false};
+  void start_locked() { if (!th.joinable()) th = std::thread([this]() { loop(); }); }
+  void run(std::function<void()> f) {
+    std::unique_lock<std::mutex> lk(mu);
+    start_locked();
+    job = std::move(f); has = true; done = false;
+    posted.store(true, std::memory_order_release);
+    cv.notify_all();
+  }
+  void arm() {
+    std::unique_lock<std::mutex> lk(mu);
+    start_locked();
+    if (!has && done) { stand_down.store(false, std::memory_order_relaxed); armed = true; cv.notify_all(); }
+  }
+  void disarm() { stand_down.store(true, std::memory_order_release); }
+  void wait() {
+    std::unique_lock<std::mutex> lk(mu);
+    cv.wait(lk, [this]() { return done; });
+  }
+  void loop() {
+    std::unique_lock<std::mutex> lk(mu);
+    for (;;) {
+      cv.wait(lk, [this]() { return has || quit || armed; });
+      if (quit) return;
+      if (!has) {
+        armed = false;
+        lk.unlock();
+        const auto until = std::chrono::steady_clock::now() + std::chrono::milliseconds(2);
+        for (uint32_t k = 0; !posted.load(std::memory_order_acquire); ++k) {
+          if (stand_down.load(std::memory_order_acquire)) break;
+          if ((k & 0xffu) == 0xffu && std::chrono::steady_clock::now() > until) break;
+          __builtin_ia32_pause();
+        }
+        lk.lock();
+        if (!has) continue;
+      }
+      armed = false;
+      std::function<void()> f = std::move(job);
+      has = false;
+      posted.store(false, std::memory_order_relaxed);
+      lk.unlock();
+      f();
+      lk.lock();
+      done = true;
+      cv.notify_all();
+    }
+  }
+  ~Helper() {
+    { std::unique_lock<std::mutex> lk(mu); quit = true; cv.notify_all(); }
+    if (th.joinable()) th.join();
+  }
+};
+
+constexpr int HORNER_EMAX = 2 * 256 + 64;
+constexpr int HORNER_MAX_PARTS = 8;
+
+static cg1h::jac horner_sum(const PointWords* const* pts, const int* exps, size_t count, int nth, Helper* helpers) {
+  constexpr int EMAX = HORNER_EMAX;
+  uint16_t first[EMAX + 1];
+  memset(first, 0, sizeof first);
+  int e_top = 0;
+  size_t live = 0;
+  auto keep = [&](size_t i) { return !pts[i]->inf && exps[i] >= 0 && exps[i] < EMAX; };
+  for (size_t i = 0; i < count; ++i) if (keep(i)) { ++first[exps[i] + 1]; ++live; if (exps[i] > e_top) e_top = exps[i]; }
+  for (int e = 0; e < EMAX; ++e) first[e + 1] = (uint16_t)(first[e + 1] + first[e]);
+  std::vector<const PointWords*> byexp(live);
+  {
+    uint16_t cur[EMAX];
+    memcpy(cur, first, sizeof cur);
+    for (size_t i = 0; i < count; ++i) if (keep(i)) byexp[cur[exps[i]]++] = pts[i];
+  }
+  auto horner = [&](int lo, int hi) {
+    cg1h::jac a = cg1h::jac_identity();
+    for (int e = hi; e >= lo; --e) {
+      a = cg1h::jac_dbl(a);
+      for (uint16_t k = first[e]; k < first[e + 1]; ++k) a = cg1h::jac_add(a, jac_from_words(*byexp[k]));
+    }
+    return a;
+  };
+  if (nth > HORNER_MAX_PARTS) nth = HORNER_MAX_PARTS;
+  if (nth <= 1 || !helpers) return horner(0, e_top);
+  cg1h::jac part[HORNER_MAX_PARTS];
+  int lo[HORNER_MAX_PARTS + 1];
+  {
+    constexpr long DBL = 7, ADD = 16;
+    auto fill = [&](long C, int* cut) {
+      int e = 0;
+      for (int j = 0; j < nth; ++j) {
+        cut[j] = e;
+        long adds = 0;
+        while (e <= e_top && DBL * (e + 1) + ADD * (adds + (first[e + 1] - first[e])) <= C) { adds += first[e + 1] - first[e]; ++e; }
+      }
+      cut[nth] = e_top + 1;
+      return e > e_top;
+    };
+    long lo_c = DBL * (e_top + 1), hi_c = DBL * (e_top + 1) + ADD * (long)live;
+    int cut[HORNER_MAX_PARTS + 1];
+    while (lo_c < hi_c) {
+      const long mid = (lo_c + hi_c) / 2;
+      if (fill(mid, cut)) hi_c = mid; else lo_c = mid + 1;
+    }
+    fill(hi_c, cut);
+    for (int j = 0; j <= nth; ++j) lo[j] = cut[j];
+  }
+  auto run_part = [&](int j) {
+    cg1h::jac a = horner(lo[j], lo[j + 1] - 1);
+    for (int k = 0; k < lo[j]; ++k) a = cg1h::jac_dbl(a);
+    part[j] = a;
+  };
+  for (int j = 0; j + 1 < nth; ++j) helpers[j].run([&, j]() { run_part(j); });
+  run_part(nth - 1);
+  cg1h::jac acc = part[nth - 1];
+  for (int j = 0; j + 1 < nth; ++j) { helpers[j].wait(); acc = cg1h::jac_add(acc, part[j]); }
+  return acc;
+}
+
+}
diff --git a/curdleproofs_pie_amd/csrc/kernels_accumulate.h b/curdleproofs_pie_amd/csrc/kernels_accumulate.h
--- a/curdleproofs_pie_amd/csrc/kernels_accumulate.h
+++ b/curdleproofs_pie_amd/csrc/kernels_accumulate.h
@@ -48,12 +48,15 @@
   store_sum(sums + t, acc);
 }
 
-__global__ void __launch_bounds__(256) k_heavy_combine(const uint32_t* __restrict__ heavy, uint32_t heavy_cap,
-                                                       const uint32_t* __restrict__ choff, PointSum* __restrict__ sums,
-                                                       uint8_t* __restrict__ combined) {
+__global__ void __launch_bounds__(256) k_chunk_join(const uint32_t* __restrict__ heavy, uint32_t heavy_cap,
+                                                    const uint32_t* __restrict__ choff, PointSum* __restrict__ sums,
+                                                    uint8_t* __restrict__ combined, uint32_t nb_total,
+                                                    const uint32_t* __restrict__ any_multi, int fold) {
   __shared__ PointSum sh[4];
   uint32_t nheavy = heavy[0];
   if (nheavy > heavy_cap) nheavy = heavy_cap;
+  const bool do_fold = fold && *any_multi != 0u;
+  if (nheavy == 0u && !do_fold) return;
   for (uint32_t h = blockIdx.x; h < nheavy; h += gridDim.x) {
     const uint32_t b = heavy[1 + h];
     const uint32_t c0 = choff[b], c1 = choff[b + 1];
@@ -73,17 +76,13 @@
     }
     __syncthreads();
   }
+  if (!do_fold) return;
+  for (uint32_t b = blockIdx.x * 256 + threadIdx.x; b < nb_total; b += gridDim.x * 256) {
+    const uint32_t c0 = choff[b], c1 = choff[b + 1];
+    if (c1 - c0 < 2u || c1 - c0 >= HEAVY_MIN_CHUNKS) continue;
+    xyzz acc = load_sum(sums + c0);
+    for (uint32_t k = c0 + 1; k < c1; ++k) acc = xyzz_add(acc, load_sum(sums + k));
+    store_sum(sums + c0, acc);
+    combined[b] = 1;
+  }
 }
-
-__global__ void __launch_bounds__(256) k_bucket_fold(const uint32_t* __restrict__ choff, PointSum* __restrict__ sums,
-                                                     uint8_t* __restrict__ combined, uint32_t nb_total, const uint32_t* __restrict__ any_multi = nullptr) {
-  if (any_multi && *any_multi == 0u) return;
-  uint32_t b = blockIdx.x * 256 + threadIdx.x;
-  if (b >= nb_total) return;
-  const uint32_t c0 = choff[b], c1 = choff[b + 1];
-  if (c1 - c0 < 2u || c1 - c0 >= HEAVY_MIN_CHUNKS) return;
-  xyzz acc = load_sum(sums + c0);
-  for (uint32_t k = c0 + 1; k < c1; ++k) acc = xyzz_add(acc, load_sum(sums + k));
-  store_sum(sums + c0, acc);
-  combined[b] = 1;
-}
diff --git a/curdleproofs_pie_amd/csrc/kernels_prepare_digits.h b/curdleproofs_pie_amd/csrc/kernels_prepare_digits.h
--- a/curdleproofs_pie_amd/csrc/kernels_prepare_digits.h
+++ b/curdleproofs_pie_amd/csrc/kernels_prepare_digits.h
@@ -199,9 +199,14 @@
   inf_flag[n + i] = inf_flag[i];
 }
 
+__device__ __forceinline__ void zero_words(uint32_t* __restrict__ z, uint32_t nwords) {
+  for (uint32_t k = blockIdx.x * blockDim.x + threadIdx.x; k < nwords; k += gridDim.x * blockDim.x) z[k] = 0u;
+}
+
 __global__ void __launch_bounds__(256) k_hist(const uint32_t* __restrict__ scalars, const uint8_t* __restrict__ inf_flag,
                                               uint32_t* __restrict__ hist, uint32_t n, WinPlan pl, int rank, int world,
-                                              uint32_t* __restrict__ bad_flag) {
+                                              uint32_t* __restrict__ bad_flag, uint32_t* __restrict__ zwords, uint32_t nzwords) {
+  zero_words(zwords, nzwords);
   uint32_t i = blockIdx.x * 256 + threadIdx.x;
   if (i >= n) return;
   if (inf_flag[i]) return;
diff --git a/curdleproofs_pie_amd/csrc/kernels_records.h b/curdleproofs_pie_amd/csrc/kernels_records.h
--- a/curdleproofs_pie_amd/csrc/kernels_records.h
+++ b/curdleproofs_pie_amd/csrc/kernels_records.h
@@ -15,12 +15,6 @@
 };
 static_assert(sizeof(PointSum) == 256, "");
 
-struct alignas(16) PointWords {
-  uint32_t w[4][12];
-  uint32_t inf;
-  uint32_t pad[3];
-};
-static_assert(sizeof(PointWords) == 208, "");
 
 __device__ __forceinline__ void load_affine(const PreparedPoint* p, fp& x, fp& y, uint32_t& flags) {
   const uint4* q = reinterpret_cast<const uint4*>(p);
diff --git a/curdleproofs_pie_amd/csrc/kernels_sort.h b/curdleproofs_pie_amd/csrc/kernels_sort.h
--- a/curdleproofs_pie_amd/csrc/kernels_sort.h
+++ b/curdleproofs_pie_amd/csrc/kernels_sort.h
@@ -29,7 +29,8 @@
 
 __global__ void __launch_bounds__(256) k_digits(const uint32_t* __restrict__ scalars, const uint8_t* __restrict__ inf_flag,
                                                 uint16_t* __restrict__ digits, uint32_t n, WinPlan pl, int rank, int world,
-                                                uint32_t* __restrict__ bad_flag) {
+                                                uint32_t* __restrict__ bad_flag, uint32_t* __restrict__ zwords, uint32_t nzwords) {
+  zero_words(zwords, nzwords);
   uint32_t i = blockIdx.x * 256 + threadIdx.x;
   if (i >= n) return;
   const bool inf = inf_flag[i] != 0;
@@ -79,15 +80,49 @@
   if (threadIdx.x < nbins) block_counts[((size_t)lw * nbins + threadIdx.x) * nslices + slice] = cnt[threadIdx.x];
 }
 
+constexpr uint32_t BIN_STAGE = 12288;
+constexpr uint32_t SLICE = BIN_STAGE;
+
+__device__ __forceinline__ void slice_plan(const uint32_t* __restrict__ block_base, uint32_t nbins_total, uint32_t nslices,
+                                           uint32_t* __restrict__ slice_base ,
+                                           uint8_t* __restrict__ bigflag, int enable, uint32_t* part_sum ) {
+  const uint32_t per = (nbins_total + 255u) / 256u, g0 = threadIdx.x * per;
+  uint32_t mine = 0;
+  for (uint32_t g = g0; g < g0 + per && g < nbins_total; ++g) {
+    const uint32_t size = block_base[(size_t)(g + 1) * nslices] - block_base[(size_t)g * nslices];
+    mine += (enable && size > BIN_STAGE) ? (size + SLICE - 1u) / SLICE : 0u;
+  }
+  part_sum[threadIdx.x] = mine;
+  __syncthreads();
+  for (int d = 1; d < 256; d <<= 1) {
+    uint32_t u = ((int)threadIdx.x >= d) ? part_sum[threadIdx.x - d] : 0u;
+    __syncthreads();
+    part_sum[threadIdx.x] += u;
+    __syncthreads();
+  }
+  uint32_t run = part_sum[threadIdx.x] - mine;
+  for (uint32_t g = g0; g < g0 + per && g < nbins_total; ++g) {
+    const uint32_t size = block_base[(size_t)(g + 1) * nslices] - block_base[(size_t)g * nslices];
+    const uint32_t ns = (enable && size > BIN_STAGE) ? (size + SLICE - 1u) / SLICE : 0u;
+    slice_base[g] = run;
+    bigflag[g] = ns ? 1 : 0;
+    run += ns;
+  }
+  if (threadIdx.x == 255) slice_base[nbins_total] = part_sum[255];
+  __syncthreads();
+}
+
 __global__ void __launch_bounds__(256) k_part_scatter(const uint16_t* __restrict__ digits, const uint32_t* __restrict__ block_base,
                                                       uint32_t* __restrict__ part, uint32_t n, uint32_t nslices, uint32_t nbins,
-                                                      uint32_t sub_bits, int use_stage) {
+                                                      uint32_t sub_bits, int use_stage,
+                                                      uint32_t* __restrict__ slice_base, uint8_t* __restrict__ bigflag, int big_bins) {
   __shared__ uint32_t cur[128];
   __shared__ uint32_t gbase[128];
   __shared__ uint32_t lbase[128];
   __shared__ uint32_t stage[PART_TILE];
   __shared__ uint32_t gpos[PART_TILE];
   const uint32_t slice = blockIdx.x, lw = blockIdx.y;
+  if (slice == 0u && lw == 0u) slice_plan(block_base, gridDim.y * nbins, nslices, slice_base, bigflag, big_bins, stage);
   uint32_t mycnt = 0;
   if (threadIdx.x < nbins) {
     const size_t idx = ((size_t)lw * nbins + threadIdx.x) * nslices + slice;
@@ -130,7 +165,6 @@
     for (uint32_t o = threadIdx.x; o < total; o += 256) part[gpos[o]] = stage[o];
   }
 }
-constexpr uint32_t BIN_STAGE = 12288;
 __global__ void __launch_bounds__(256) k_bin_sort(const uint32_t* __restrict__ part, const uint32_t* __restrict__ block_base,
                                                   uint32_t* __restrict__ hist, uint32_t* __restrict__ sorted,
                                                   uint32_t nbins_total, uint32_t nslices, uint32_t sub_bits, int use_stage,
@@ -176,37 +210,6 @@
     __syncthreads();
     for (uint32_t o = threadIdx.x; start + o < end; o += 256) sorted[start + o] = stage[o];
   }
-}
-
-constexpr uint32_t SLICE = BIN_STAGE;
-
-__global__ void __launch_bounds__(256) k_slice_plan(const uint32_t* __restrict__ block_base, uint32_t nbins_total, uint32_t nslices,
-                                                    uint32_t* __restrict__ slice_base ,
-                                                    uint8_t* __restrict__ bigflag, int enable) {
-  __shared__ uint32_t part_sum[256];
-  const uint32_t per = (nbins_total + 255u) / 256u, g0 = threadIdx.x * per;
-  uint32_t mine = 0;
-  for (uint32_t g = g0; g < g0 + per && g < nbins_total; ++g) {
-    const uint32_t size = block_base[(size_t)(g + 1) * nslices] - block_base[(size_t)g * nslices];
-    mine += (enable && size > BIN_STAGE) ? (size + SLICE - 1u) / SLICE : 0u;
-  }
-  part_sum[threadIdx.x] = mine;
-  __syncthreads();
-  for (int d = 1; d < 256; d <<= 1) {
-    uint32_t u = ((int)threadIdx.x >= d) ? part_sum[threadIdx.x - d] : 0u;
-    __syncthreads();
-    part_sum[threadIdx.x] += u;
-    __syncthreads();
-  }
-  uint32_t run = part_sum[threadIdx.x] - mine;
-  for (uint32_t g = g0; g < g0 + per && g < nbins_total; ++g) {
-    const uint32_t size = block_base[(size_t)(g + 1) * nslices] - block_base[(size_t)g * nslices];
-    const uint32_t ns = (enable && size > BIN_STAGE) ? (size + SLICE - 1u) / SLICE : 0u;
-    slice_base[g] = run;
-    bigflag[g] = ns ? 1 : 0;
-    run += ns;
-  }
-  if (threadIdx.x == 255) slice_base[nbins_total] = part_sum[255];
 }
 
 __device__ __forceinline__ bool slice_of_block(const uint32_t* __restrict__ slice_base, uint32_t nbins_total, uint32_t b,
@@ -315,8 +318,19 @@
   }
 }
 
-__global__ void __launch_bounds__(256) k_uscan1(uint32_t* __restrict__ a, uint32_t* __restrict__ block_tot, uint32_t n) {
+__device__ __forceinline__ bool last_block_ticket(uint32_t* ticket, uint32_t nblocks, uint32_t* s_ticket ) {
+  __threadfence();
+  __syncthreads();
+  if (threadIdx.x == 0) *s_ticket = atomicAdd(ticket, 1u);
+  __syncthreads();
+  if (*s_ticket != nblocks - 1u) return false;
+  __threadfence();
+  return true;
+}
+
+__global__ void __launch_bounds__(256) k_uscan1(uint32_t* __restrict__ a, uint32_t* block_tot, uint32_t n, uint32_t* ticket) {
   __shared__ uint32_t sh[256];
+  __shared__ uint32_t s_ticket;
   uint32_t base = blockIdx.x * SCAN_ITEMS + threadIdx.x * 4;
   uint32_t v[4], local = 0;
 #pragma unroll
@@ -333,14 +347,15 @@
 #pragma unroll
   for (int k = 0; k < 4; ++k) { if (base + k < n) a[base + k] = excl; excl += v[k]; }
   if (threadIdx.x == 255) block_tot[blockIdx.x] = sh[255];
-}
-__global__ void __launch_bounds__(256) k_uscan2(uint32_t* __restrict__ block_tot, uint32_t nblocks, uint32_t* __restrict__ a, uint32_t n) {
-  __shared__ uint32_t sh[256];
+  const uint32_t nblocks = gridDim.x;
+  if (!last_block_ticket(ticket, nblocks, &s_ticket)) return;
+  if (threadIdx.x == 0) *ticket = 0u;
   uint32_t carry = 0;
   for (uint32_t tile = 0; tile < nblocks; tile += 256) {
     uint32_t i = tile + threadIdx.x;
-    uint32_t v = (i < nblocks) ? block_tot[i] : 0u;
-    sh[threadIdx.x] = v;
+    uint32_t t = (i < nblocks) ? block_tot[i] : 0u;
+    __syncthreads();
+    sh[threadIdx.x] = t;
     __syncthreads();
     for (int d = 1; d < 256; d <<= 1) {
       uint32_t u = ((int)threadIdx.x >= d) ? sh[threadIdx.x - d] : 0u;
@@ -348,9 +363,8 @@
       sh[threadIdx.x] += u;
       __syncthreads();
     }
-    if (i < nblocks) block_tot[i] = carry + sh[threadIdx.x] - v;
+    if (i < nblocks) block_tot[i] = carry + sh[threadIdx.x] - t;
     uint32_t tot = sh[255];
-    __syncthreads();
     carry += tot;
   }
   if (threadIdx.x == 0) a[n] = carry;
@@ -464,9 +478,36 @@
   return (cnt + L - 1) / L;
 }
 
+constexpr uint32_t LEN_BINS = 256;
+__device__ __forceinline__ uint32_t len_key(uint32_t len) { return len < LEN_BINS - 1 ? len : LEN_BINS - 1; }
+
+__device__ __forceinline__ void len_hist_add(uint32_t* sh_hist, uint32_t cnt, uint32_t L0) {
+  if (cnt == 0u) return;
+  const uint32_t L = chunk_len(cnt, L0), nch = (cnt + L - 1) / L;
+  if (nch > 1u) atomicAdd(&sh_hist[len_key(L)], nch - 1u);
+  atomicAdd(&sh_hist[len_key(cnt - (nch - 1u) * L)], 1u);
+}
+
+__device__ __forceinline__ void len_cursor_scan(uint32_t v, uint32_t* __restrict__ len_cursor, uint32_t* sh ) {
+  __syncthreads();
+  sh[threadIdx.x] = v;
+  __syncthreads();
+  for (int d = 1; d < 256; d <<= 1) {
+    uint32_t u = ((int)threadIdx.x >= d) ? sh[threadIdx.x - d] : 0u;
+    __syncthreads();
+    sh[threadIdx.x] += u;
+    __syncthreads();
+  }
+  len_cursor[LEN_BINS - 1 - threadIdx.x] = sh[threadIdx.x] - v;
+}
+
 __global__ void __launch_bounds__(256) k_scan1(const uint32_t* __restrict__ hist, uint32_t* __restrict__ off, uint32_t* __restrict__ choff,
-                                               uint2* __restrict__ block_tot, uint32_t nb_total, uint32_t L0) {
+                                               uint2* block_tot, uint32_t nb_total, uint32_t L0,
+                                               uint32_t* len_hist, uint32_t* __restrict__ len_cursor, uint32_t* ticket, uint32_t* __restrict__ stats) {
   __shared__ uint2 sh[256];
+  __shared__ uint32_t shl[LEN_BINS];
+  __shared__ uint32_t s_ticket;
+  shl[threadIdx.x] = 0;
   uint32_t base = blockIdx.x * SCAN_ITEMS + threadIdx.x * 4;
   uint32_t cnt[4], ch[4];
   uint2 local = make_uint2(0, 0);
@@ -478,6 +519,8 @@
   }
   sh[threadIdx.x] = local;
   __syncthreads();
+#pragma unroll
+  for (int k = 0; k < 4; ++k) len_hist_add(shl, cnt[k], L0);
   for (int d = 1; d < 256; d <<= 1) {
     uint2 v = make_uint2(0, 0);
     if ((int)threadIdx.x >= d) v = sh[threadIdx.x - d];
@@ -492,14 +535,15 @@
     excl.x += cnt[k]; excl.y += ch[k];
   }
   if (threadIdx.x == 255) block_tot[blockIdx.x] = sh[255];
-}
-__global__ void __launch_bounds__(256) k_scan2(uint2* __restrict__ block_tot, uint32_t nblocks, uint32_t* __restrict__ off,
-                                               uint32_t* __restrict__ choff, uint32_t nb_total) {
-  __shared__ uint2 sh[256];
+  { const uint32_t v = shl[threadIdx.x]; if (v) atomicAdd(&len_hist[threadIdx.x], v); }
+  const uint32_t nblocks = gridDim.x;
+  if (!last_block_ticket(ticket, nblocks, &s_ticket)) return;
+  if (threadIdx.x == 0) *ticket = 0u;
   uint2 carry = make_uint2(0, 0);
   for (uint32_t tile = 0; tile < nblocks; tile += 256) {
     uint32_t i = tile + threadIdx.x;
     uint2 v = (i < nblocks) ? block_tot[i] : make_uint2(0, 0);
+    __syncthreads();
     sh[threadIdx.x] = v;
     __syncthreads();
     for (int d = 1; d < 256; d <<= 1) {
@@ -511,10 +555,10 @@
     }
     if (i < nblocks) block_tot[i] = make_uint2(carry.x + sh[threadIdx.x].x - v.x, carry.y + sh[threadIdx.x].y - v.y);
     uint2 tot = sh[255];
-    __syncthreads();
     carry.x += tot.x; carry.y += tot.y;
   }
-  if (threadIdx.x == 0) { off[nb_total] = carry.x; choff[nb_total] = carry.y; }
+  if (threadIdx.x == 0) { off[nb_total] = carry.x; choff[nb_total] = carry.y; stats[1] = carry.x; stats[2] = carry.y; }
+  len_cursor_scan(__hip_atomic_load(&len_hist[LEN_BINS - 1 - threadIdx.x], __ATOMIC_RELAXED, __HIP_MEMORY_SCOPE_AGENT), len_cursor, shl);
 }
 __global__ void __launch_bounds__(256) k_scan3(const uint2* __restrict__ block_tot, uint32_t* __restrict__ off,
                                                uint32_t* __restrict__ choff, uint32_t nb_total) {
@@ -524,16 +568,16 @@
   for (int k = 0; k < 4; ++k) if (base + k < nb_total) { off[base + k] += p.x; choff[base + k] += p.y; }
 }
 
-constexpr uint32_t LEN_BINS = 256;
-__device__ __forceinline__ uint32_t len_key(uint32_t len) { return len < LEN_BINS - 1 ? len : LEN_BINS - 1; }
-
 constexpr uint32_t SCAN1_MAX = 1u << 13;
 __global__ void __launch_bounds__(1024) k_scan_one(const uint32_t* __restrict__ hist, uint32_t* __restrict__ off, uint32_t* __restrict__ choff,
-                                                    uint32_t nb_total, uint32_t L0) {
+                                                    uint32_t nb_total, uint32_t L0, uint32_t* __restrict__ len_cursor, uint32_t* __restrict__ stats) {
   __shared__ uint2 sh[1024];
+  __shared__ uint32_t shl[LEN_BINS];
+  if (threadIdx.x < LEN_BINS) shl[threadIdx.x] = 0;
+  __syncthreads();
   const uint32_t per = (nb_total + 1023u) / 1024u, lo = threadIdx.x * per, hi = (lo + per < nb_total) ? lo + per : nb_total;
   uint2 local = make_uint2(0, 0);
-  for (uint32_t i = lo; i < hi; ++i) { const uint32_t c = hist[i]; local.x += c; local.y += chunk_count(c, L0); }
+  for (uint32_t i = lo; i < hi; ++i) { const uint32_t c = hist[i]; local.x += c; local.y += chunk_count(c, L0); len_hist_add(shl, c, L0); }
   sh[threadIdx.x] = local;
   __syncthreads();
   for (int d = 1; d < 1024; d <<= 1) {
@@ -549,15 +593,28 @@
     off[i] = excl.x; choff[i] = excl.y;
     excl.x += c; excl.y += chunk_count(c, L0);
   }
-  if (threadIdx.x == 1023) { off[nb_total] = sh[1023].x; choff[nb_total] = sh[1023].y; }
+  if (threadIdx.x == 1023) { off[nb_total] = sh[1023].x; choff[nb_total] = sh[1023].y; stats[1] = sh[1023].x; stats[2] = sh[1023].y; }
+  __shared__ uint32_t shs[LEN_BINS];
+  const bool mine = threadIdx.x < LEN_BINS;
+  const uint32_t v = mine ? shl[LEN_BINS - 1 - threadIdx.x] : 0u;
+  if (mine) shs[threadIdx.x] = v;
+  __syncthreads();
+  for (int d = 1; d < 256; d <<= 1) {
+    uint32_t u = (mine && (int)threadIdx.x >= d) ? shs[threadIdx.x - d] : 0u;
+    __syncthreads();
+    if (mine) shs[threadIdx.x] += u;
+    __syncthreads();
+  }
+  if (mine) len_cursor[LEN_BINS - 1 - threadIdx.x] = shs[threadIdx.x] - v;
 }
 
 constexpr uint32_t CHUNK_DESC_BLOCKS = 320;
 __global__ void __launch_bounds__(256) k_chunk_desc(const uint32_t* __restrict__ off, const uint32_t* __restrict__ choff,
-                                                    uint2* __restrict__ desc, uint32_t* __restrict__ len_hist,
+                                                    uint2* __restrict__ desc, uint32_t* __restrict__ len_cursor, uint32_t* __restrict__ order,
                                                     uint32_t* __restrict__ heavy ,
                                                     uint32_t heavy_cap, uint32_t nb_total, uint32_t L0, uint32_t* __restrict__ any_multi = nullptr) {
   __shared__ uint32_t sh[LEN_BINS];
+  __shared__ uint32_t pos[LEN_BINS];
   sh[threadIdx.x] = 0;
   __syncthreads();
 #pragma unroll 1
@@ -570,8 +627,7 @@
         uint32_t s = k * L, len = (cnt - s < L) ? (cnt - s) : L;
         desc[o + k] = make_uint2(start + s, len);
       }
-      if (nch > 1u) atomicAdd(&sh[len_key(L)], nch - 1u);
-      atomicAdd(&sh[len_key(cnt - (nch - 1u) * L)], 1u);
+      len_hist_add(sh, cnt, L0);
       if (nch >= HEAVY_MIN_CHUNKS) {
         uint32_t slot = atomicAdd(&heavy[0], 1u);
         if (slot < heavy_cap) heavy[1 + slot] = b;
@@ -582,62 +638,20 @@
   }
   }
   __syncthreads();
-  uint32_t v = sh[threadIdx.x];
-  if (v) atomicAdd(&len_hist[threadIdx.x], v);
-}
-
-__global__ void __launch_bounds__(256) k_len_scan(const uint32_t* __restrict__ len_hist, uint32_t* __restrict__ len_cursor,
-                                                  const uint32_t* __restrict__ total_entries, const uint32_t* __restrict__ total_chunks,
-                                                  uint32_t* __restrict__ stats) {
-  __shared__ uint32_t sh[LEN_BINS];
-  if (threadIdx.x == 0) { stats[1] = *total_entries; stats[2] = *total_chunks; }
-  uint32_t rev = LEN_BINS - 1 - threadIdx.x;
-  uint32_t v = len_hist[rev];
-  sh[threadIdx.x] = v;
-  __syncthreads();
-  for (int d = 1; d < 256; d <<= 1) {
-    uint32_t u = ((int)threadIdx.x >= d) ? sh[threadIdx.x - d] : 0u;
-    __syncthreads();
-    sh[threadIdx.x] += u;
-    __syncthreads();
-  }
-  len_cursor[rev] = sh[threadIdx.x] - v;
-}
-
-constexpr uint32_t ORDER_PER = 8;
-__global__ void __launch_bounds__(256) k_order(const uint2* __restrict__ desc, const uint32_t* __restrict__ total_chunks,
-                                               uint32_t* __restrict__ len_cursor, uint32_t* __restrict__ order) {
-  __shared__ uint32_t cnt[LEN_BINS];
-  __shared__ uint32_t base[LEN_BINS];
-  cnt[threadIdx.x] = 0;
-  __syncthreads();
-  const uint32_t total = *total_chunks;
-  uint32_t key[ORDER_PER], local[ORDER_PER];
-#pragma unroll
-  for (uint32_t rep = 0; rep < ORDER_PER; ++rep) {
-    const uint32_t t = (blockIdx.x * ORDER_PER + rep) * 256 + threadIdx.x;
-    const bool live = t < total;
-    key[rep] = live ? len_key(desc[t].y) : 0u;
-    local[rep] = 0;
-    const unsigned long long amask = __ballot(live);
-    if (amask) {
-      const int leader = __ffsll((long long)amask) - 1;
-      const uint32_t k0 = __shfl(key[rep], leader, 64);
-      const unsigned long long same = __ballot(live && key[rep] == k0);
-      const uint32_t lane = threadIdx.x & 63u;
-      uint32_t b0 = 0;
-      if ((int)lane == leader) b0 = atomicAdd(&cnt[k0], (uint32_t)__popcll(same));
-      b0 = __shfl(b0, leader, 64);
-      if (live) local[rep] = (key[rep] == k0) ? b0 + (uint32_t)__popcll(same & ((1ull << lane) - 1ull)) : atomicAdd(&cnt[key[rep]], 1u);
-    }
-  }
-  __syncthreads();
-  const uint32_t c = cnt[threadIdx.x];
-  if (c) base[threadIdx.x] = atomicAdd(&len_cursor[threadIdx.x], c);
-  __syncthreads();
-#pragma unroll
-  for (uint32_t rep = 0; rep < ORDER_PER; ++rep) {
-    const uint32_t t = (blockIdx.x * ORDER_PER + rep) * 256 + threadIdx.x;
-    if (t < total) order[base[key[rep]] + local[rep]] = t;
-  }
-}
+  { const uint32_t v = sh[threadIdx.x]; pos[threadIdx.x] = v ? atomicAdd(&len_cursor[threadIdx.x], v) : 0u; }
+  __syncthreads();
+#pragma unroll 1
+  for (uint32_t b = blockIdx.x * 256 + threadIdx.x; b - threadIdx.x < nb_total; b += gridDim.x * 256) {
+  if (b < nb_total) {
+    uint32_t start = off[b], cnt = off[b + 1] - start;
+    if (cnt) {
+      uint32_t L = chunk_len(cnt, L0), nch = (cnt + L - 1) / L, o = choff[b];
+      if (nch > 1u) {
+        const uint32_t p = atomicAdd(&pos[len_key(L)], nch - 1u);
+        for (uint32_t k = 0; k + 1u < nch; ++k) order[p + k] = o + k;
+      }
+      order[atomicAdd(&pos[len_key(cnt - (nch - 1u) * L)], 1u)] = o + nch - 1u;
+    }
+  }
+  }
+}
diff --git a/curdleproofs_pie_amd/csrc/msm_gpu.hip b/curdleproofs_pie_amd/csrc/msm_gpu.hip
--- a/curdleproofs_pie_amd/csrc/msm_gpu.hip
+++ b/curdleproofs_pie_amd/csrc/msm_gpu.hip
@@ -15,6 +15,7 @@
 #include "g1_xyzz.h"
 #include "g1_quad.h"
 #include "host_g1.h"
+#include "host_horner.h"
 #include "lazy_host.h"
 #include "pool.h"
 #include "../../include/curdle_g1.h"
```

Result: slower. 356.4 million (-4.0%).
